# althonos/pyskani

Hardware: AMD Instinct MI355X
Metric: genome-pairs/sec (sketch+ANI) (higher is better)
Workload: dtype u64; 1 GPU; all-vs-all 10000 x 10000 synthetic ~5 Mb genomes on one GPU (100 families x 100; single-contig genomes, substitutions only), c=125 marker_c=1000 k=15; device-resident ASCII; hits=999867, genomes=10000, parallelism=references sharded over 1 GPU(s)

## Files before the change

### pyskani_amd/csrc/chain.hip

```cpp
#include "chain_stages.h"
#include "query_parts.h"
#include <hipcub/hipcub.hpp>
#include <cmath>
#include <algorithm>
#include <unordered_map>


SketchDesc make_desc(const psk_sketch* s, bool unindexed_ok) {
    SketchDesc d{};
    const bool ix = s->idx != nullptr;
    d.key = ix ? s->idx->km32 + s->idx_off : nullptr; d.pms = ix ? s->idx->pms + s->idx_off : nullptr;
    d.perm = ix ? s->idx->perm + s->idx_off : nullptr; d.bucket = ix ? s->idx->bucket + s->idx_boff : nullptr;
    d.bshift = ix ? s->idx_bshift : 0; d.n = (ix || (unindexed_ok && s->store)) ? (uint32_t)s->n_seeds : 0;
    d.pos = s->store ? s->store->seed_pos + s->seed_off : nullptr; d.meta = s->store ? s->store->seed_meta + s->seed_off : nullptr;
    d.kmer = s->store ? s->store->seed_kmer + s->seed_off : nullptr;
    d.seed_pos_base = s->store ? s->store->seed_pos : nullptr;
    d.contig_start = s->store ? s->store->contig_seed_start + s->contig_off : nullptr;
    d.total_len = s->total_len; d.n_contigs = (uint32_t)s->contig_len.size();
    uint64_t rows = 0;
    if (d.n) for (uint32_t len : s->contig_len) rows += (uint64_t)len / (FRAGMENT_LENGTH + 1) + 1;
    d.rows = (uint32_t)std::min<uint64_t>(rows, 0xFFFFFFFFu);
    s->len_quantiles(d.lenq);
    d.tab = (ix && s->ptab) ? (const ProbeLine*)s->ptab->base + s->ptab_off : nullptr; d.tab_lines = (ix && s->ptab) ? s->ptab_lines : 0;
    return d;
// ... 25 lines not shown
    const int lane = threadIdx.x & 63, wave = threadIdx.x >> 6;
    uint32_t running = 0;
    for (uint32_t base = 0; base < n_refs && running < B.rank_hi; base += 256) {
        const uint32_t r = base + threadIdx.x;
        const bool f = r < n_refs && row[r];
        const unsigned long long bal = __ballot(f);
        if (lane == 0) s_w[wave] = (uint32_t)__popcll(bal);
        __syncthreads();
        uint32_t before = 0;
        for (int w = 0; w < wave; w++) before += s_w[w];
        const uint32_t tot = s_w[0] + s_w[1] + s_w[2] + s_w[3];
        const uint32_t rank = running + before + (uint32_t)__popcll(bal & ((1ull << lane) - 1));
        if (f && rank >= B.rank_lo && rank < B.rank_hi) {
            const uint32_t j = rank - B.rank_lo, slot = B.pair_off + j;
            pairs[slot] = combine_desc(Q, rd[r]);
            sbase[slot] = B.item_off + j * Q.n; cbase[slot] = B.row_off + j * Q.rows;
            pair_qr[slot] = make_uint2(B.q, r);
        }
        running += tot;
        __syncthreads();
    }
    if (blockIdx.x == gridDim.x - 1 && threadIdx.x == 0) { sbase[n_pairs] = n_items; cbase[n_pairs] = n_rows; }
}

__global__ __launch_bounds__(256) void pass_canon_kernel(uint8_t* __restrict__ pass, uint32_t n_refs, const uint32_t* __restrict__ canon) {
    uint8_t* row = pass + (size_t)blockIdx.x * n_refs;
    for (uint32_t r = threadIdx.x; r < n_refs; r += blockDim.x) if (row[r] && canon[r] != r) { row[canon[r]] = 1; row[r] = 0; }
}
static_assert((1 << BSI_BLOG) == 256, "pass_count_kernel: one sweep of its 256 threads = one block of references");
__global__ __launch_bounds__(256) void pass_count_kernel(const uint8_t* __restrict__ pass, uint32_t n_refs, uint32_t* __restrict__ row_count, uint8_t* __restrict__ col_flag, uint32_t* __restrict__ row_blocks) {
    __shared__ uint32_t s_c[4], s_any;
    const uint8_t* row = pass + (size_t)blockIdx.x * n_refs;
    uint32_t c = 0, blocks = 0;
    if (threadIdx.x == 0) s_any = 0;
    __syncthreads();
    for (uint32_t r0 = 0; r0 < n_refs; r0 += 256) {
        const uint32_t r = r0 + threadIdx.x;
        const bool f = r < n_refs && row[r];
        if (f) { c++; col_flag[r] = 1; s_any = 1; }
        __syncthreads();
        blocks += s_any;
        __syncthreads();
        if (threadIdx.x == 0) s_any = 0;
        __syncthreads();
    }
#pragma unroll
    for (int o = 32; o > 0; o >>= 1) c += __shfl_xor(c, o);
    if ((threadIdx.x & 63) == 0) s_c[threadIdx.x >> 6] = c;
    __syncthreads();
    if (threadIdx.x == 0) { row_count[blockIdx.x] = s_c[0] + s_c[1] + s_c[2] + s_c[3]; row_blocks[blockIdx.x] = blocks; }
}

__global__ __launch_bounds__(256) void gsi_room_kernel(const uint32_t* __restrict__ sbase, uint32_t n_pairs, uint32_t* __restrict__ pstart) {
    const uint32_t p = blockIdx.x * blockDim.x + threadIdx.x;
    if (p <= n_pairs) { const uint32_t a = sbase[p]; pstart[p] = a + (a >> 3) + 8u * p; }
}
__global__ void gsi_total_kernel(const unsigned long long* __restrict__ poff, uint32_t n_pairs, unsigned long long* __restrict__ total64) { *total64 = poff[n_pairs]; }

struct HitPasses { __host__ __device__ bool operator()(const psk_hit& h) const { return h.ani > 0.1f; } };

__global__ __launch_bounds__(256) void work_rows_kernel(const ChunkOut* __restrict__ cout, const uint32_t* __restrict__ n_chunks, const uint32_t* __restrict__ cbase,
                                                        const uint32_t* __restrict__ row_pair, uint32_t n_rows, unsigned long long* __restrict__ out) {
    __shared__ unsigned long long s_c[4], s_l[4];
    unsigned long long c = 0, live = 0;
    for (uint32_t r = blockIdx.x * blockDim.x + threadIdx.x; r < n_rows; r += gridDim.x * blockDim.x) {
        const uint32_t p = row_pair[r];
        if (r - cbase[p] < n_chunks[p]) { c += cout[r].n_cand; live++; }
    }
#pragma unroll
    for (int o = 32; o > 0; o >>= 1) { c += __shfl_xor(c, o); live += __shfl_xor(live, o); }
    if ((threadIdx.x & 63) == 0) { s_c[threadIdx.x >> 6] = c; s_l[threadIdx.x >> 6] = live; }
    __syncthreads();
    if (threadIdx.x == 0) {
        c = s_c[0] + s_c[1] + s_c[2] + s_c[3]; live = s_l[0] + s_l[1] + s_l[2] + s_l[3];
        if (live) { atomicAdd(&out[0], c); atomicAdd(&out[1], live); }
    }
}

psk_status chain_layout(Lane* ctx, size_t n_pairs, size_t n_items, size_t n_rows, size_t n_bq, ChainBufs* L) {
    const size_t gi = (n_items + 255) / 256, gi_sum = std::max(gi, (n_pairs + 3) / 4);
    size_t o_pairs = 0, o_sbase = al256(o_pairs + sizeof(PairDesc) * n_pairs), o_cbase = al256(o_sbase + 4 * (n_pairs + 1)),
           o_pstart = al256(o_cbase + 4 * (n_pairs + 1)), o_lb = al256(o_pstart + 4 * (n_pairs + 1)),
           o_aoff = al256(o_lb + 8 * (n_items + 1)), o_nch = al256(o_aoff + 4 * (n_items + 1)),
           o_chunks = al256(o_nch + 4 * n_pairs), o_cout = al256(o_chunks + sizeof(uint2) * n_rows),
           o_misc = al256(o_cout + sizeof(ChunkOut) * n_rows), o_hits = o_misc + 256, o_sel = al256(o_hits + sizeof(psk_hit) * n_pairs),
           o_ovf = al256(o_sel + sizeof(psk_hit) * n_pairs), o_bsum = al256(o_ovf + 4 * n_rows),
           o_qr = al256(o_bsum + 8 * (gi_sum + 1)), o_bq = al256(o_qr + 8 * n_pairs), o_bp = al256(o_bq + sizeof(BatchQ) * (n_bq + 1)),
           o_rp = al256(o_bp + 4 * (gi + 1)), o_live = al256(o_rp + 4 * (n_rows + 1)), o_big = al256(o_live + 4 * (n_pairs + 1)),
           o_huge = al256(o_big + 4 * (n_pairs + 1)), o_end = o_huge + 4 * (n_pairs + 1);
    PSK_TRY(ctx->q_b.reserve(o_end));
    char* B = (char*)ctx->q_b.p;
    L->pairs = (PairDesc*)(B + o_pairs); L->sbase = (uint32_t*)(B + o_sbase); L->cbase = (uint32_t*)(B + o_cbase); L->pstart = (uint32_t*)(B + o_pstart);
    L->lbcnt = (uint2*)(B + o_lb); L->aoff = (uint32_t*)(B + o_aoff); L->nch = (uint32_t*)(B + o_nch); L->chunks = (uint2*)(B + o_chunks);
    L->cout = (ChunkOut*)(B + o_cout); L->hits = (psk_hit*)(B + o_hits); L->hits_sel = (psk_hit*)(B + o_sel); L->misc = (uint32_t*)(B + o_misc);
    L->ovf = (uint32_t*)(B + o_ovf); L->bsum = (unsigned long long*)(B + o_bsum); L->pair_qr = (uint2*)(B + o_qr); L->bq = (BatchQ*)(B + o_bq);
    L->blk_pair = (uint32_t*)(B + o_bp); L->row_pair = (uint32_t*)(B + o_rp); L->live = (uint32_t*)(B + o_live); L->big_list = (uint32_t*)(B + o_big); L->huge_list = (uint32_t*)(B + o_huge);
    L->gi = (uint32_t)gi; L->gi_sum = (uint32_t)gi_sum;
    L->total = (unsigned long long*)(L->misc + 16);
    return PSK_OK;
}

psk_status chain_run(Lane* ctx, const ChainBufs& L, uint32_t n_pairs, size_t n_items, size_t n_rows, const psk_params& prm,
                     const psk_query_opts* o, const SketchDesc* d_qd, const SketchDesc* d_rd, uint64_t cap, bool wide, const Switches& sw, bool probe_ok) {
    hipStream_t st = ctx->stream;
    const int force_serial = sw.chain_serial.get() != nullptr;
    const uint32_t gi = L.gi;
    hipLaunchKernelGGL(pair_table_kernel, dim3((uint32_t)(((size_t)gi + n_rows + 255) / 256)), dim3(256), 0, st, L.sbase, L.cbase, n_pairs, gi, (uint32_t)n_items, (uint32_t)n_rows, L.blk_pair, L.row_pair,
                       L.misc, L.lbcnt + n_items);
    ctx->t_begin(K_ANCHOR);
    if (wide) hipLaunchKernelGGL(anchor_count_kernel, dim3(gi), dim3(256), 0, st, L.pairs, L.sbase, n_pairs, (uint32_t)n_items, L.lbcnt, L.bsum, L.blk_pair);
    const uint32_t gi4 = (gi + JT - 1) / JT;
    uint32_t n_sum = gi;
    const int jp_force = sw.join_pairs.force();
    const bool gsi_join = !wide && (L.g_key || L.b_key) && L.d_pass && L.n_bq;
    const bool join_pairs = !wide && (gsi_join || (jp_force >= 0 ? jp_force == 1 : (n_pairs >= 16384 && n_items / n_pairs < 2048)));
    const bool gsl = gsi_join && L.gsi_slice;
    const bool gsi_one = gsi_join && !gsl && L.gsi_onepass && cap >= n_items + n_items / 8 + 8 * ((size_t)n_pairs + 1);
    bool probe_local = false;
    GsiJoinArgs GA{};
    GslArgs GL{};
    const uint32_t gsi_nw = (L.g_key && !L.gsi_slice) ? std::max(4u, (L.n_refs + 63u) / 64u) : 4u;
    const size_t gsi_lds_row = 8 * (size_t)gsi_nw + 4 * (size_t)((gsi_nw + 1u) & ~1u), gsi_lds_count = gsi_lds_row + 4 * (size_t)L.p_cap, gsi_lds_emit = gsi_lds_row + 4 * (size_t)L.p_cap * 9;
    if (gsi_join) {
        GA.bq = L.bq; GA.pass = L.d_pass; GA.n_refs = L.n_refs; GA.qd = d_qd; GA.g_key = L.g_key; GA.g_val = L.g_val; GA.g_bucket = L.g_bucket; GA.g_shift = L.g_shift;
        GA.b_key = L.b_key; GA.b_val = L.b_val; GA.b_bucket = L.b_bucket; GA.b_shift = L.b_shift; GA.b_nb1 = L.b_nb1; GA.b_blocks = L.b_blocks; GA.b_max = L.b_max;
        GA.pair_cnt = L.big_list; GA.pstart = L.pstart; GA.cap = (uint32_t)cap; GA.err = L.misc; GA.p_cap = L.p_cap; GA.nw_lds = gsi_nw;
        const uint32_t t_blocks = gsl ? L.g_blocks : L.b_blocks;
        const unsigned long long* t_base = gsl ? L.g_base : L.b_base;
        const uint32_t bcap = std::max(1u, std::min<uint32_t>(t_blocks, std::min<uint32_t>(GSI_PMAX, std::max(1u, L.p_cap))));
        uint32_t* d_btab = nullptr; uint32_t* d_bcnt = nullptr;
        if (t_blocks) {
            const size_t o_bc = al256(4 * (size_t)L.n_bq * bcap * GSL_BT_WORDS);
            PSK_TRY(ctx->q_k.reserve(o_bc + 4 * (size_t)L.n_bq + 256));
            d_btab = (uint32_t*)ctx->q_k.p; d_bcnt = (uint32_t*)((char*)ctx->q_k.p + o_bc);
            PSK_TRY(gsl_blocks_launch(L.bq, L.n_bq, L.d_pass, L.n_refs, t_blocks, t_base, d_btab, d_bcnt, bcap, st));
        }
        GA.blk_tab = d_btab; GA.blk_cnt = d_bcnt; GA.blk_cap = bcap;
        if (gsl) {
            GL.bq = L.bq; GL.n_entries = L.n_bq; GL.tab = L.gsl_tab; GL.n_tab = L.gsl_n_tab; GL.ebase = L.gsl_ebase; GL.pass = L.d_pass; GL.n_refs = L.n_refs; GL.qd = d_qd;
            GL.g_key = L.g_key; GL.g_val = L.g_val; GL.g_bucket = L.g_bucket; GL.g_shift = L.g_shift; GL.g_nb1 = L.g_nb1; GL.g_blocks = L.g_blocks; GL.g_base = L.g_base; GL.blk_tab = d_btab; GL.blk_cnt = d_bcnt; GL.blk_cap = bcap; GL.cnt = L.gsl_cnt; GL.rec = L.gsl_rec; GL.bm = L.gsl_bm; GL.un = L.gsl_un; GL.n_slices = L.gsl_n_slices;
            GL.pair_cnt = L.big_list; GL.pstart = L.pstart; GL.cap = (uint32_t)cap; GL.err = L.misc; GL.p_cap = L.p_cap; GL.chunks = L.chunks; GL.n_chunks = L.nch;
            PSK_HIP(hipMemsetAsync(L.big_list, 0, 4 * ((size_t)n_pairs + 1), st));
            PSK_TRY(gsl_count_launch(GL, st));
        }
        else if (!gsi_one) hipLaunchKernelGGL(gsi_join_kernel<false>, dim3(L.n_bq), dim3(64), gsi_lds_count, st, GA);
        probe_local = true;
    }
    else if (join_pairs) {
        size_t ts = 0;
        uint32_t* keys_in = L.big_list;
        uint32_t* vals_in = L.live;
        uint32_t* keys_out = (uint32_t*)L.hits_sel;
        uint32_t* order = keys_out + n_pairs;
        hipLaunchKernelGGL(pair_ref_keys_kernel, dim3((n_pairs + 255) / 256), dim3(256), 0, st, L.pair_qr, n_pairs, keys_in, vals_in);
        PSK_HIP(hipcub::DeviceRadixSort::SortPairs(nullptr, ts, keys_in, keys_out, vals_in, order, (int)n_pairs, 0, 32, st));
        PSK_TRY(ctx->q_g.reserve(ts + 256));
        PSK_HIP(hipcub::DeviceRadixSort::SortPairs(ctx->q_g.p, ts, keys_in, keys_out, vals_in, order, (int)n_pairs, 0, 32, st));
        const uint32_t nb = (n_pairs + 3) / 4;
        probe_local = probe_ok;
        if (probe_ok) hipLaunchKernelGGL(anchor_join_probe_kernel, dim3(nb), dim3(256), 0, st, L.pairs, L.sbase, order, n_pairs, L.lbcnt, L.bsum, L.misc + 5, L.aoff, L.big_list);
        else hipLaunchKernelGGL(anchor_join_pairs_kernel, dim3(nb), dim3(256), 0, st, L.pairs, L.sbase, order, n_pairs, L.lbcnt, L.bsum, L.misc + 5);
        n_sum = nb;
    }
    const int ep_force = sw.emit_pairs.force();
    const bool emit_pairs = !wide && !join_pairs && n_items >= 2 * ((size_t)n_pairs + 1) &&
                            (ep_force >= 0 ? ep_force == 1 : (n_pairs >= 1024 && n_items / n_pairs >= 1024 && n_items / n_pairs <= (1u << 17)));
    uint32_t* pair_cnt = L.live;
    if (emit_pairs) PSK_HIP(hipMemsetAsync(pair_cnt, 0, 4 * ((size_t)n_pairs + 1), st));
    const int xg_env = (int)sw.xcd_group.num(-1);
    const uint32_t xcd_group = xg_env >= 0 ? (uint32_t)xg_env : (n_pairs >= 64 ? (uint32_t)std::min<size_t>(4096, std::max<size_t>(1, 4 * (n_items / n_pairs) / (JT * 256))) : 0u);
    if (!wide && !join_pairs) { hipLaunchKernelGGL(anchor_join4_kernel, dim3(gi4), dim3(256), 0, st, L.pairs, L.sbase, n_pairs, (uint32_t)n_items, gi, L.lbcnt, L.bsum, L.misc + 5, L.blk_pair, emit_pairs ? pair_cnt : (uint32_t*)nullptr, xcd_group); n_sum = gi4; }
    ctx->t_end();
    size_t tmp = 0, tmp2 = 0;
    hipcub::TransformInputIterator<uint32_t, CountOf, const uint2*> cnt_it(L.lbcnt, CountOf());
    hipcub::TransformInputIterator<uint32_t, PackedCount, const uint2*> pcnt_it(L.lbcnt, PackedCount());
    PSK_HIP(hipcub::DeviceScan::ExclusiveSum(nullptr, tmp, cnt_it, L.aoff, (int)(n_items + 1), st));
    PSK_HIP(hipcub::DeviceReduce::Sum(nullptr, tmp2, L.bsum, L.total, (int)L.gi_sum, st));
    size_t tmp3 = 0;
    PSK_HIP(hipcub::DeviceSelect::If(nullptr, tmp3, L.hits, L.hits_sel, L.misc + 12, (int)n_pairs, HitPasses(), st));
    PSK_TRY(ctx->q_c.reserve(std::max(tmp, std::max(tmp2, tmp3))));
    unsigned long long* poff = (unsigned long long*)L.aoff;
    hipcub::TransformInputIterator<unsigned long long, Widen, const uint32_t*> pc_it(pair_cnt, Widen());
    if (gsi_one) {
        hipLaunchKernelGGL(gsi_room_kernel, dim3((n_pairs + 1 + 255) / 256), dim3(256), 0, st, (const uint32_t*)L.sbase, n_pairs, L.pstart);
        PSK_HIP(hipMemsetAsync(L.total, 0, 8, st));
    }
    else if (emit_pairs) {
        size_t tmp4 = 0;
        PSK_HIP(hipcub::DeviceScan::ExclusiveSum(nullptr, tmp4, pc_it, poff, (int)(n_pairs + 1), st));
        PSK_TRY(ctx->q_c.reserve(std::max(tmp4, std::max(tmp, std::max(tmp2, tmp3)))));
        PSK_HIP(hipcub::DeviceScan::ExclusiveSum(ctx->q_c.p, tmp4, pc_it, poff, (int)(n_pairs + 1), st));
        hipLaunchKernelGGL(pair_start64_kernel, dim3((n_pairs + 1 + 255) / 256), dim3(256), 0, st, poff, n_pairs, L.pstart, (uint32_t)cap, (const uint32_t*)(L.misc + 5));
    }
    else if (probe_local) {
        hipcub::TransformInputIterator<unsigned long long, Widen, const uint32_t*> pl_it(L.big_list, Widen());
        size_t tmp5 = 0;
        PSK_HIP(hipcub::DeviceScan::ExclusiveSum(nullptr, tmp5, pl_it, (unsigned long long*)nullptr, (int)(n_pairs + 1), st));
        const size_t o_poff = al256(tmp5 + 256);
        PSK_TRY(ctx->q_g.reserve(o_poff + 8 * ((size_t)n_pairs + 2) + 256));
        unsigned long long* pl_off64 = (unsigned long long*)((char*)ctx->q_g.p + o_poff);
        PSK_HIP(hipMemsetAsync(L.big_list + n_pairs, 0, 4, st));
        PSK_HIP(hipcub::DeviceScan::ExclusiveSum(ctx->q_g.p, tmp5, pl_it, pl_off64, (int)(n_pairs + 1), st));
        hipLaunchKernelGGL(pair_start64_kernel, dim3((n_pairs + 1 + 255) / 256), dim3(256), 0, st, (const unsigned long long*)pl_off64, n_pairs, L.pstart, (uint32_t)cap, (const uint32_t*)(L.misc + 5));
        if (gsi_join) hipLaunchKernelGGL(gsi_total_kernel, dim3(1), dim3(1), 0, st, (const unsigned long long*)pl_off64, n_pairs, L.total);
    }
    else if (wide) PSK_HIP(hipcub::DeviceScan::ExclusiveSum(ctx->q_c.p, tmp, cnt_it, L.aoff, (int)(n_items + 1), st));
    else PSK_HIP(hipcub::DeviceScan::ExclusiveSum(ctx->q_c.p, tmp, pcnt_it, L.aoff, (int)(n_items + 1), st));
    const bool small_sum = !gsi_join && n_sum <= 16384;
    if (!small_sum && !gsi_join) PSK_HIP(hipcub::DeviceReduce::Sum(ctx->q_c.p, tmp2, L.bsum, L.total, (int)n_sum, st));
    if ((!emit_pairs && !probe_local) || small_sum)
        hipLaunchKernelGGL(pair_start_kernel, dim3((emit_pairs || probe_local) ? 1u : (n_pairs + 1 + 255) / 256), dim3(256), 0, st, (emit_pairs || probe_local) ? (const uint32_t*)nullptr : L.aoff, L.sbase, n_pairs, L.pstart, (uint32_t)cap,
                           L.bsum, small_sum ? n_sum : 0u, L.total, (const uint32_t*)(L.misc + 5));
    hipLaunchKernelGGL(pair_guard_kernel, dim3((n_pairs + 1 + 255) / 256), dim3(256), 0, st, (const uint32_t*)(L.misc + 5), (const unsigned long long*)L.total, (unsigned long long)cap, L.pstart, n_pairs);
    const size_t na = ((size_t)cap + 64 + 63) & ~(size_t)63;
    PSK_TRY(ctx->q_d.reserve(4 * na * CHAIN_ANCHOR_WORDS));
    PSK_TRY(ctx->q_e.reserve(na * (8 + 4 * 7 + 1) + 512 + 4 * 2 * BIG_GMAX * (BIG_GROUPS + 64) + 4 * BIG_GROUPS));
    uint32_t* D = (uint32_t*)ctx->q_d.p;
    uint32_t* E4 = (uint32_t*)ctx->q_e.p;
    uint4* anc = (uint4*)D;
    uint32_t* a_nxt = D + 4 * na;
    ChainArgs A{};
    A.anc = anc;
    A.sc_ptr = D + 5 * na;
    A.sc_f = (int32_t*)E4; A.sc_root = E4 + na; A.sc_depth = E4 + 2 * na; A.sc_best = E4 + 3 * na;
    uint32_t* CAND = D + 6 * na;
    A.c_score.p = (int32_t*)CAND; A.c_q0.p = CAND + 1; A.c_q1.p = CAND + 2; A.c_r0.p = CAND + 3; A.c_r1.p = CAND + 4; A.c_n.p = CAND + 5; A.c_rc.p = CAND + 6; A.c_state.p = CAND + 7;
    A.chunks = L.chunks; A.n_chunks = L.nch; A.cbase = L.cbase; A.n_pairs = n_pairs; A.n_rows = (uint32_t)n_rows;
    A.row_pair = L.row_pair;
    A.pairs = L.pairs;
    A.out = L.cout; A.two_c = 2u * (uint32_t)prm.c; A.force_serial = force_serial; A.stats = L.misc + 1;
    A.band = std::max(1, std::min(MAX_CHAIN_BAND, BP_CHAIN_BAND / (int)prm.c));
    A.cap = (uint32_t)cap;
    const bool use_hops = gsi_join ? false : sw.chunk_hops.get() ? !sw.chunk_hops.off() : ((n_pairs < 1024 && n_items / n_pairs > 4096) || n_items / n_pairs > (1u << 20));
    const bool emit_heads = emit_pairs && !use_hops && !sw.emit_heads.off();
    const int hi_force = sw.hops_items.force();
    const bool hops_items = use_hops && !gsl && !emit_pairs && !join_pairs && n_items <= 0x7FFFFFFFull && (hi_force >= 0 ? hi_force == 1 : n_items / n_pairs > (1u << 20));
    ctx->t_begin(K_ANCHOR_EMIT);
    if (hops_items) {
        const size_t o_scr = al256(4 * (size_t)n_pairs * HOP_SLICES + 256);
        PSK_TRY(ctx->q_g.reserve(o_scr + sizeof(uint2) * n_rows + 256));
        uint32_t* slice_cnt = (uint32_t*)ctx->q_g.p;
        uint2* scratch_rows = (uint2*)((char*)ctx->q_g.p + o_scr);
        hipStream_t sd = nullptr;
        PSK_TRY(ctx->side_lane(&sd));
        PSK_HIP(hipEventRecord(ctx->side_fork, st));
        PSK_HIP(hipStreamWaitEvent(sd, ctx->side_fork, 0));
        hipLaunchKernelGGL(chunk_hops_items_kernel, dim3(n_pairs, HOP_SLICES), dim3(64), 0, sd, L.pstart, (const uint32_t*)L.aoff, L.pairs, L.sbase, L.cbase, n_pairs, slice_cnt, scratch_rows, L.misc);
        hipLaunchKernelGGL(chunk_hops_sliced_kernel, dim3(n_pairs, HOP_SLICES), dim3(64), 0, sd, L.pstart, a_nxt, anc, L.pairs, L.cbase, n_pairs, slice_cnt, 1, scratch_rows, L.chunks, L.nch, L.misc);
        PSK_HIP(hipEventRecord(ctx->side_join, sd));
    }
    if (gsl) { GL.anc = anc; PSK_TRY(gsl_heads_launch(GL, st)); PSK_TRY(gsl_emit_launch(GL, st)); }
    else if (gsi_join) { GA.anc = anc; GA.chunks = L.chunks; GA.n_chunks = L.nch; GA.onepass = gsi_one ? 1 : 0; GA.total = L.total; if (gsi_one) GA.pair_cnt = L.aoff;
                    hipLaunchKernelGGL(gsi_join_kernel<true>, dim3(L.n_bq), dim3(64), gsi_lds_emit, st, GA); }
    else if (wide) hipLaunchKernelGGL(anchor_emit_kernel, dim3(gi), dim3(256), 0, st, L.pairs, L.sbase, n_pairs, (uint32_t)n_items, L.lbcnt, L.aoff, anc, (uint32_t)cap, L.misc, L.blk_pair);
    else if (emit_pairs) hipLaunchKernelGGL(anchor_emit_pairs_kernel, dim3(n_pairs), dim3(EP_T), 0, st, L.pairs, L.sbase, n_pairs, L.lbcnt, poff, anc, (uint32_t)cap, L.misc,
                                            L.cbase, emit_heads ? L.chunks : (uint2*)nullptr, L.nch);
    else {
        const int ex_force = sw.emit_expand.force();
        const bool expand = ex_force >= 0 ? ex_force == 1 : n_items / n_pairs > (1u << 20);
        if (expand) hipLaunchKernelGGL(anchor_emit_expand_kernel, dim3(gi), dim3(256), 0, st, L.pairs, L.sbase, n_pairs, (uint32_t)n_items, L.lbcnt, L.aoff, anc, (uint32_t)cap, L.misc, L.blk_pair);
        else hipLaunchKernelGGL(anchor_emit_packed4_kernel, dim3(gi4), dim3(256), 0, st, L.pairs, L.sbase, n_pairs, (uint32_t)n_items, gi, L.lbcnt, L.aoff, anc, (uint32_t)cap, L.misc, L.blk_pair,
                                probe_local ? (const uint32_t*)L.pstart : (const uint32_t*)nullptr);
    }
    if (hops_items) PSK_HIP(hipStreamWaitEvent(st, ctx->side_join, 0));
    else if (use_hops) {
        if (n_items / n_pairs > (1u << 20)) {
            uint32_t* coarse = E4;
            hipLaunchKernelGGL(anchor_next_kernel<1>, dim3((uint32_t)((cap / 64 + 1 + 255) / 256)), dim3(256), 0, st, anc, L.pstart, n_pairs, (const uint32_t*)nullptr, coarse);
            hipLaunchKernelGGL(anchor_next_kernel<2>, dim3((uint32_t)((cap + 255) / 256)), dim3(256), 0, st, anc, L.pstart, n_pairs, (const uint32_t*)coarse, a_nxt);
        } else
        hipLaunchKernelGGL(anchor_next_kernel<0>, dim3((uint32_t)((cap + 255) / 256)), dim3(256), 0, st, anc, L.pstart, n_pairs, (const uint32_t*)nullptr, a_nxt);
        if (n_items / n_pairs > (1u << 20)) {
            const size_t o_scr = al256(4 * (size_t)n_pairs * HOP_SLICES + 256);
            PSK_TRY(ctx->q_g.reserve(o_scr + sizeof(uint2) * n_rows + 256));
            uint32_t* slice_cnt = (uint32_t*)ctx->q_g.p;
            uint2* scratch_rows = (uint2*)((char*)ctx->q_g.p + o_scr);
            for (int pass = 0; pass < 2; pass++)
                hipLaunchKernelGGL(chunk_hops_sliced_kernel, dim3(n_pairs, HOP_SLICES), dim3(64), 0, st, L.pstart, a_nxt, anc, L.pairs, L.cbase, n_pairs, slice_cnt, pass, scratch_rows, L.chunks, L.nch, L.misc);
        } else
        hipLaunchKernelGGL(chunk_hops_kernel, dim3(n_pairs), dim3(64), 0, st, L.pstart, a_nxt, L.cbase, n_pairs, L.chunks, L.nch, L.misc);
    } else if (!emit_heads && !gsi_join)
        hipLaunchKernelGGL(chunk_heads_kernel, dim3(n_pairs), dim3(64), 0, st, L.pstart, anc, L.cbase, n_pairs, L.chunks, L.nch, L.misc);
    ctx->t_end();
    ctx->t_begin(K_CHAIN_CHUNK);
    auto order_rows = [&]() -> psk_status {
        if (n_rows < 4096) return PSK_OK;
        size_t ts = 0;
        PSK_HIP(hipcub::DeviceRadixSort::SortPairsDescending(nullptr, ts, (const uint32_t*)nullptr, (uint32_t*)nullptr, (const uint32_t*)nullptr, (uint32_t*)nullptr, (int)n_rows, 0, 8, st));
        const size_t ob = al256(4 * n_rows);
        PSK_TRY(ctx->q_g.reserve(4 * ob + ts + 256));
        uint32_t* k_in = (uint32_t*)ctx->q_g.p; uint32_t* v_in = (uint32_t*)((char*)ctx->q_g.p + ob); uint32_t* k_out = (uint32_t*)((char*)ctx->q_g.p + 2 * ob); uint32_t* v_out = (uint32_t*)((char*)ctx->q_g.p + 3 * ob);
        hipLaunchKernelGGL(row_len_kernel, dim3((uint32_t)((n_rows + 255) / 256)), dim3(256), 0, st, L.chunks, L.nch, L.cbase, L.row_pair, (uint32_t)n_rows, k_in, v_in);
        PSK_HIP(hipcub::DeviceRadixSort::SortPairsDescending((char*)ctx->q_g.p + 4 * ob, ts, (const uint32_t*)k_in, k_out, (const uint32_t*)v_in, v_out, (int)n_rows, 0, 8, st));
        A.row_order = v_out;
        return PSK_OK;
    };
    {
        const char* le = sw.chain_lane.get();
        A.lane_dp = !force_serial && A.band <= LANE_N && !sw.chain_lane.off();
        if (A.lane_dp) {
            PSK_TRY(order_rows());
            uint32_t rpw = 64;
            while (rpw > 16 && n_rows / rpw < 512) rpw >>= 1;
            const int le_rows = (int)sw.chain_lane.num(0);
            if (le_rows >= 8) rpw = (uint32_t)std::min(64, le_rows);
            const uint32_t waves = (uint32_t)((n_rows + rpw - 1) / rpw);
            A.ovf_list = L.ovf; A.ovf_count = L.misc + 8;
            const bool quad = le && le[0] == 'q' ? true : (le_rows >= 8 ? false : n_rows < 32 * 1024);
            if (quad) {
                const uint32_t qw = (uint32_t)((n_rows + 15) / 16);
                hipLaunchKernelGGL(chain_quad_kernel, dim3((qw + LANE_WAVES - 1) / LANE_WAVES), dim3(64 * LANE_WAVES), 0, st, A);
            } else {
                const int xt_force = sw.lane_xtrees.force();
                const bool xtrees = xt_force >= 0 ? xt_force == 1 : n_items / n_pairs > (1u << 20);
                if (A.band <= 20 && xtrees) hipLaunchKernelGGL(chain_lane20x_kernel, dim3((waves + LANE_WAVES - 1) / LANE_WAVES), dim3(64 * LANE_WAVES), 0, st, A, rpw);
                else if (A.band <= 20) hipLaunchKernelGGL(chain_lane20_kernel, dim3((waves + LANE_WAVES - 1) / LANE_WAVES), dim3(64 * LANE_WAVES), 0, st, A, rpw);
                else hipLaunchKernelGGL(chain_lane_kernel, dim3((waves + LANE_WAVES - 1) / LANE_WAVES), dim3(64 * LANE_WAVES), 0, st, A, rpw);
            }
            const uint32_t lw = (uint32_t)std::min<size_t>((n_rows + CHAIN_WAVES - 1) / CHAIN_WAVES, 2048);
            hipLaunchKernelGGL(chain_chunk_list_kernel, dim3(lw), dim3(64 * CHAIN_WAVES), 0, st, A);
        }
    }
    const int wr_force = sw.chain_wave_reg.force();
    const bool wave_reg = !A.lane_dp && !force_serial && A.band < 128 && (wr_force >= 0 ? wr_force == 1 : n_rows <= 2048);
    if (wave_reg) {
        const dim3 g((uint32_t)((n_rows + CHAIN_WAVES - 1) / CHAIN_WAVES)), b(64 * CHAIN_WAVES);
        if (A.band < 64) hipLaunchKernelGGL(chain_wave_reg_kernel<1>, g, b, 0, st, A);
        else hipLaunchKernelGGL(chain_wave_reg_kernel<2>, g, b, 0, st, A);
    }
    const bool quad_deep = !wave_reg && !A.lane_dp && !force_serial && !sw.chain_quad_deep.off() && A.band <= 4 * QD && !sw.chain_lane.off();
    if (quad_deep) {
        A.ovf_list = L.ovf; A.ovf_count = L.misc + 8;
        A.lane_dp = 1;
        PSK_TRY(order_rows());
        const uint32_t qw = (uint32_t)((n_rows + 15) / 16);
        hipLaunchKernelGGL(chain_quad_deep_kernel, dim3((qw + LANE_WAVES - 1) / LANE_WAVES), dim3(64 * LANE_WAVES), 0, st, A);
        const uint32_t lw = (uint32_t)std::min<size_t>((n_rows + CHAIN_WAVES - 1) / CHAIN_WAVES, 2048);
        hipLaunchKernelGGL(chain_chunk_list_kernel, dim3(lw), dim3(64 * CHAIN_WAVES), 0, st, A);
    }
    if (!A.lane_dp && !wave_reg)
    hipLaunchKernelGGL(chain_chunk_kernel, dim3((uint32_t)((n_rows + CHAIN_WAVES - 1) / CHAIN_WAVES)), dim3(64 * CHAIN_WAVES), 0, st, A);
    ctx->t_end();
    SelArgs SA{};
    SA.chunks = L.chunks; SA.n_chunks = L.nch; SA.cbase = L.cbase; SA.n_pairs = n_pairs;
    SA.c_score = A.c_score; SA.c_q0 = A.c_q0; SA.c_q1 = A.c_q1; SA.c_r0 = A.c_r0; SA.c_r1 = A.c_r1; SA.c_n = A.c_n; SA.c_rc = A.c_rc; SA.c_state = A.c_state;
    SA.out = L.cout; SA.two_c = A.two_c; SA.force_serial = force_serial; SA.stats = L.misc + 1;
    const bool use_live = n_pairs > 4096;
    SA.live = use_live ? L.live : nullptr; SA.n_live = L.misc + 9; SA.big_list = L.big_list; SA.big_count = L.misc + 10;
    if (use_live) {
        hipcub::CountingInputIterator<uint32_t> ids(0);
        size_t tl = 0;
        PSK_HIP(hipcub::DeviceSelect::If(nullptr, tl, ids, L.live, L.misc + 9, (int)n_pairs, IsLivePair{L.nch}, st));
        PSK_TRY(ctx->q_c.reserve(std::max(tl, std::max(tmp, std::max(tmp2, tmp3)))));
        PSK_HIP(hipcub::DeviceSelect::If(ctx->q_c.p, tl, ids, L.live, L.misc + 9, (int)n_pairs, IsLivePair{L.nch}, st));
    }
    ctx->t_begin(K_SELECT);
    {
        SA.tiny_done = use_live && !force_serial && !sw.select_tiny.off() && n_rows / n_pairs < 16;
        SA.rest_list = (uint32_t*)L.hits_sel; SA.rest_count = L.misc + 13;
        if (SA.tiny_done) hipLaunchKernelGGL(select_tiny_kernel, dim3((n_pairs + 255) / 256), dim3(256), 0, st, SA);
    }
    hipLaunchKernelGGL(select_kernel, dim3(std::min<uint32_t>(n_pairs, 16384u)), dim3(64), 0, st, SA, L.huge_list, L.misc + 14);
    hipLaunchKernelGGL(select_mid_kernel, dim3(std::min<uint32_t>(n_pairs, 768u)), dim3(64), 0, st, SA, (const uint32_t*)L.huge_list, (const uint32_t*)(L.misc + 14));
    {
        if (!force_serial) {
            BigArgs BA{};
            BA.S = SA; BA.pstart = L.pstart;
            char* E = (char*)ctx->q_e.p;
            BA.key = (unsigned long long*)E; uint32_t* U = (uint32_t*)(E + 8 * na);
            BA.slot = U; BA.crow = U + na; BA.idx = U + 2 * na; BA.pm = U + 3 * na; BA.pm2 = U + 4 * na; BA.ord = U + 5 * na; BA.clist = U + 6 * na;
            BA.conf = (uint8_t*)(U + 7 * na);
            BA.parts = (uint32_t*)(E + (((size_t)na * (8 + 4 * 7 + 1) + 255) & ~(size_t)255));
            BA.huge_list = L.huge_list; BA.huge_count = L.misc + 11; BA.ctr = L.misc + 32; BA.huge_c = BA.parts + (size_t)2 * BIG_GMAX * (BIG_GROUPS + 64);
            const uint32_t solo = sw.big_solo.get() ? (uint32_t)std::max((int)sw.big_solo.num(0), CMAX) : BIG_SOLO;
            BA.solo = solo;
            hipLaunchKernelGGL(select_big_kernel, dim3(std::min<uint32_t>(n_pairs, 64u)), dim3(BIG_T), 0, st, BA);
            if (na / 3 > solo) {
                static std::mutex slots_mu;
                static std::unordered_map<int, uint32_t> slots_of;
                uint32_t slots;
                {
                    std::lock_guard<std::mutex> lk(slots_mu);
                    auto it = slots_of.find(ctx->device);
                    if (it == slots_of.end()) {
                        int per_cu = 0, cus = 0;
                        PSK_HIP(hipOccupancyMaxActiveBlocksPerMultiprocessor(&per_cu, select_huge_kernel, BIG_T, 0));
                        PSK_HIP(hipDeviceGetAttribute(&cus, hipDeviceAttributeMultiprocessorCount, ctx->device));
                        if (sw.huge_slots.get()) { per_cu = 1; cus = std::max(0, (int)sw.huge_slots.num(0)); }
                        it = slots_of.emplace(ctx->device, (uint32_t)std::max(0, per_cu) * (uint32_t)std::max(0, cus)).first;
                    }
                    slots = it->second;
                }
                uint32_t nb = BIG_GMAX;
                if ((double)(n_items / n_pairs) > sw.huge_min_seeds.num((double)(1ull << 20))) {
                    ctx->huge_acquire();
                    while (nb > 1 && nb > slots) nb >>= 1;
                } else {
                    const uint32_t rest = slots > BIG_GMAX ? slots - BIG_GMAX : 0;
                    while (nb > 1 && (size_t)nb * ctx->dev->max_lanes > rest) nb >>= 1;
                }
                if (nb < 8) nb = 1;
                hipLaunchKernelGGL(select_huge_kernel, dim3(nb), dim3(BIG_T), 0, st, BA);
            }
        }
    }
    hipLaunchKernelGGL(chunk_seeds_kernel, dim3((uint32_t)((n_rows + 255) / 256)), dim3(256), 0, st, A);
    ctx->t_end();
    ReduceArgs R{};
    R.chunks = L.cout; R.n_chunks = L.nch; R.cbase = L.cbase; R.pstart = L.pstart; R.pcnt = gsi_one ? L.aoff : nullptr; R.pairs = L.pairs; R.pair_qr = L.pair_qr;
    R.k = prm.k; R.median = o->median; R.robust = o->robust;
    R.min_af = o->min_aligned_frac > 0 ? o->min_aligned_frac : 0.15; R.hits = L.hits;
    if (o->median || o->robust) {
        PSK_TRY(ctx->q_f.reserve(sizeof(double) * (2 * n_rows + 1024 * (size_t)n_pairs + 1024)));
        R.big_vals = (double*)ctx->q_f.p;
    }
    ctx->t_begin(K_PAIR_REDUCE);
    R.live = use_live ? L.live : nullptr; R.n_live = L.misc + 9;
    if (use_live) hipLaunchKernelGGL(pair_empty_kernel, dim3((n_pairs + 255) / 256), dim3(256), 0, st, R, n_pairs);
    const bool no_small = sw.reduce_small.off();
    const bool no_wave = sw.reduce_wave.off();
    R.wave_done = !no_wave && !no_small && L.rows_pair_max > 64u && n_rows / n_pairs <= 64u * RW_PER;
    R.small_done = !no_small && (n_rows / n_pairs < 16 || R.wave_done);
    const bool no_tiny = sw.reduce_tiny.off();
    R.tiny_done = R.small_done && !no_tiny && !o->median && !o->robust && n_rows / n_pairs < 16;
// ... 144 lines not shown
```

### pyskani_amd/csrc/chain_dev.h

```cpp
#pragma once
#include "common.h"

struct MarkerSet { const uint64_t* p; uint32_t n; uint32_t pad; };

__device__ __forceinline__ void lds_wave_sync() {
    __builtin_amdgcn_fence(__ATOMIC_RELEASE, "workgroup");
    __builtin_amdgcn_wave_barrier();
    __builtin_amdgcn_fence(__ATOMIC_ACQUIRE, "workgroup");
}

struct LaneAnchor { uint32_t q, u, m; int32_t f; };
__device__ __forceinline__ uint32_t lane_diag(uint32_t qx, uint32_t rx, uint32_t sg) { return qx - ((rx ^ sg) - sg); }

struct LanePred { uint32_t q1, u, m; int32_t f1; };
__device__ __forceinline__ int32_t lane_eval2(uint32_t qx, uint32_t ux, uint32_t mx, const LanePred& y, int d) {
    const int32_t a = (int32_t)(qx - y.q1);
    const int32_t t = (int32_t)(ux - y.u), nt = (int32_t)(y.u - ux);
    const int32_t gap = t > nt ? t : nt;
    const int32_t b = a - t;
    const int32_t s1 = y.f1 - gap;
    const uint32_t z = y.m ^ mx;
    const uint32_t bad = (uint32_t)a | (uint32_t)(BP_CHAIN_BAND - 1 - a) | (uint32_t)b | (uint32_t)(MAX_GAP_LENGTH - gap) | (uint32_t)s1 | z | (0u - z);
    const uint32_t key = ((uint32_t)s1 << 7) + ((((uint32_t)ANCHOR_SCORE2 + 1u) << 7) | (127u - (uint32_t)d));
    return (int32_t)(key | (bad & 0x80000000u));
}
```

### pyskani_amd/csrc/chain_stages.h

```cpp
#pragma once
#include "common.h"
#include "chain_dev.h"
#include "slice_join.h"

struct PairDesc {
    const uint32_t* r_key; const uint64_t* r_pms;
    const uint32_t* q_key; const uint32_t* q_perm;
    const uint32_t* q_pos; const uint32_t* q_meta;
    const uint32_t* q_kmer;
    uint32_t q_nc, pad_;
    const uint32_t* q_seed_pos_base;
    const uint32_t* q_contig_start;
    uint64_t q_total_len, r_total_len;
    uint32_t r_n, q_n;
    const uint32_t* r_bucket; uint32_t r_bshift;
    uint32_t r_tab_lines; const ProbeLine* r_tab;
};


__device__ __forceinline__ uint32_t find_le(const uint32_t* __restrict__ base, uint32_t n, uint32_t x) {
    uint32_t lo = 0, hi = n - 1;
    while (lo < hi) { uint32_t mid = (lo + hi + 1) >> 1; if (base[mid] <= x) lo = mid; else hi = mid - 1; }
    return lo;
}

__device__ __forceinline__ uint32_t pair_from_hint(const uint32_t* __restrict__ base, uint32_t n, uint32_t x, uint32_t p) {
    while (p + 1 < n && base[p + 1] <= x) p++;
    return p;
}

struct CountOf { __host__ __device__ uint32_t operator()(const uint2& v) const { return v.y; } };

constexpr int JOIN_WIN = 256;

struct PackedCount { __host__ __device__ uint32_t operator()(const uint2& v) const { return v.y >> 24; } };

constexpr int JT = 4;

struct Widen { __host__ __device__ unsigned long long operator()(const uint32_t& v) const { return v; } };

constexpr int EP_W = 1;

constexpr int EP_T = 64 * EP_W;

constexpr int HEAD_WIN = 2048;

constexpr int HOP_WIN = 4096;

constexpr int HOP_SLICES = 32;

struct ChunkOut { uint32_t anchors, seeds, n_intervals, n_cand; uint32_t left, right; uint64_t cov_q; };

template <class T> struct Strided {
    T* p;
    __host__ __device__ __forceinline__ T& operator[](size_t i) const { return p[i * 8]; }
};

struct ChainArgs {
    const uint4* anc;
    const uint2* chunks; const uint32_t* n_chunks; const uint32_t* cbase; uint32_t n_pairs, n_rows;
    const uint32_t* row_pair;
    const uint32_t* row_order;
    const PairDesc* pairs;
    ChunkOut* out;
    int32_t* sc_f; uint32_t *sc_ptr, *sc_root, *sc_depth, *sc_best;
    Strided<int32_t> c_score; Strided<uint32_t> c_q0, c_q1, c_r0, c_r1, c_n, c_state, c_rc;
    uint32_t two_c; int band; int force_serial; int lane_dp;
    uint32_t cap;
    uint32_t* ovf_list; uint32_t* ovf_count;
    uint32_t* stats;
};

constexpr int RING = 128;

constexpr int RMAX = 256;

constexpr int CHAIN_WAVES = 4;

constexpr int LANE_N = 24;

constexpr int LANE_WAVES = 2;

constexpr int LANE_TREES = 4;

constexpr int LANE_XTREES = 12;

constexpr int QUAD_N = LANE_N / 4;

constexpr int QD = 21;

constexpr int QD_NEAR = 2;

constexpr int QD_RING = 128;

constexpr int CMAX = 1024;

struct SelArgs {
    const uint2* chunks; const uint32_t* n_chunks; const uint32_t* cbase; uint32_t n_pairs;
    Strided<int32_t> c_score; Strided<uint32_t> c_q0, c_q1, c_r0, c_r1, c_n, c_rc, c_state;
    ChunkOut* out; uint32_t two_c; int force_serial; uint32_t* stats;
    const uint32_t* live; const uint32_t* n_live;
    uint32_t* rest_list; uint32_t* rest_count;
    uint32_t* big_list; uint32_t* big_count;
    int tiny_done;
};

constexpr uint32_t TINY_ROWS = 4, TINY_CANDS = 8;

constexpr int CSMALL = 512;

struct BigArgs {
    SelArgs S; const uint32_t* pstart;
    unsigned long long* key;
    uint32_t *slot, *crow;
    uint32_t *idx, *pm, *pm2;
    uint32_t *ord, *clist;
    uint8_t* conf;
    uint32_t *huge_list, *huge_count;
    uint32_t* huge_c;
    uint32_t *ctr, *parts;
    uint32_t solo;
};

constexpr int BIG_T = 1024;

constexpr uint32_t BIG_TILE = 4096;

constexpr uint32_t BIG_SOLO = 32768;

#ifndef BIG_GMAX_N
#define BIG_GMAX_N 256
#endif
constexpr uint32_t BIG_GMAX = BIG_GMAX_N;

constexpr uint32_t BIG_GROUPS = 16;

struct ReduceArgs {
    const ChunkOut* chunks; const uint32_t* n_chunks; const uint32_t* cbase;
    const uint32_t* pstart; const PairDesc* pairs;
    const uint32_t* pcnt;
    const uint2* pair_qr;
    const uint32_t* live; const uint32_t* n_live;
// ... 14 lines not shown
struct IsLivePair { const uint32_t* nch; __host__ __device__ bool operator()(const uint32_t& p) const { return nch[p] != 0; } };

struct GsiJoinArgs {
    const BatchQ* bq; const uint8_t* pass; uint32_t n_refs; const SketchDesc* qd;
    const uint32_t* g_key; const unsigned long long* g_val; const uint32_t* g_bucket; int g_shift;
    const uint32_t* b_key; const unsigned long long* b_val; const uint32_t* b_bucket; int b_shift; uint32_t b_nb1, b_blocks, b_max;
    const uint32_t* blk_tab; const uint32_t* blk_cnt; uint32_t blk_cap;
    uint32_t nw_lds;
    uint32_t* pair_cnt; const uint32_t* pstart; uint4* anc; uint32_t cap; uint32_t* err;
    uint32_t p_cap;
    uint2* chunks; uint32_t* n_chunks;
    int onepass; unsigned long long* total;
};

#ifndef LANE_NEAR_N
#define LANE_NEAR_N 3
#endif
constexpr int LANE_NEAR = LANE_NEAR_N;

__global__ __launch_bounds__(256) void pair_table_kernel(const uint32_t* __restrict__ sbase, const uint32_t* __restrict__ cbase, uint32_t n,
                                                         uint32_t n_tiles, uint32_t n_items, uint32_t n_rows,
                                                         uint32_t* __restrict__ blk_pair, uint32_t* __restrict__ row_pair, uint32_t* __restrict__ misc, uint2* __restrict__ lb_tail);
__global__ __launch_bounds__(256) void anchor_count_kernel(const PairDesc* __restrict__ pairs, const uint32_t* __restrict__ sbase,
                                                           uint32_t n_pairs, uint32_t n_items,
                                                           uint2* __restrict__ lbcnt_out, unsigned long long* __restrict__ block_sum,
                                                           const uint32_t* __restrict__ blk_pair);
__global__ __launch_bounds__(256) void anchor_join4_kernel(const PairDesc* __restrict__ pairs, const uint32_t* __restrict__ sbase,
                                                           uint32_t n_pairs, uint32_t n_items, uint32_t n_tiles,
                                                           uint2* __restrict__ item_out, unsigned long long* __restrict__ block_sum,
                                                           uint32_t* __restrict__ need_wide, const uint32_t* __restrict__ blk_pair,
                                                           uint32_t* __restrict__ pair_cnt, uint32_t xcd_group);
__global__ __launch_bounds__(256) void anchor_join_pairs_kernel(const PairDesc* __restrict__ pairs, const uint32_t* __restrict__ sbase,
                                                                const uint32_t* __restrict__ order, uint32_t n_pairs,
                                                                uint2* __restrict__ item_out, unsigned long long* __restrict__ block_sum,
                                                                uint32_t* __restrict__ need_wide);
__global__ __launch_bounds__(256) void anchor_join_probe_kernel(const PairDesc* __restrict__ pairs, const uint32_t* __restrict__ sbase,
                                                                const uint32_t* __restrict__ order, uint32_t n_pairs,
                                                                uint2* __restrict__ item_out, unsigned long long* __restrict__ block_sum,
                                                                uint32_t* __restrict__ need_wide, uint32_t* __restrict__ aoff_local, uint32_t* __restrict__ pair_cnt);
__global__ __launch_bounds__(256) void anchor_emit_packed4_kernel(const PairDesc* __restrict__ pairs, const uint32_t* __restrict__ sbase,
                                                                  uint32_t n_pairs, uint32_t n_items, uint32_t n_tiles,
                                                                  const uint2* __restrict__ item, const uint32_t* __restrict__ aoff,
                                                                  uint4* __restrict__ anc, uint32_t cap, uint32_t* __restrict__ err,
                                                                  const uint32_t* __restrict__ blk_pair, const uint32_t* __restrict__ pstart_local);
__global__ __launch_bounds__(256) void anchor_emit_expand_kernel(const PairDesc* __restrict__ pairs, const uint32_t* __restrict__ sbase,
                                                                 uint32_t n_pairs, uint32_t n_items,
                                                                 const uint2* __restrict__ item, const uint32_t* __restrict__ aoff,
                                                                 uint4* __restrict__ anc, uint32_t cap, uint32_t* __restrict__ err,
                                                                 const uint32_t* __restrict__ blk_pair);
__global__ __launch_bounds__(256) void anchor_emit_kernel(const PairDesc* __restrict__ pairs, const uint32_t* __restrict__ sbase,
                                                          uint32_t n_pairs, uint32_t n_items,
                                                          const uint2* __restrict__ lbcnt,
                                                          const uint32_t* __restrict__ aoff,
                                                          uint4* __restrict__ anc, uint32_t cap, uint32_t* __restrict__ err,
                                                          const uint32_t* __restrict__ blk_pair);
__global__ __launch_bounds__(EP_T) __attribute__((amdgpu_waves_per_eu(5, 8))) void anchor_emit_pairs_kernel(const PairDesc* __restrict__ pairs, const uint32_t* __restrict__ sbase, uint32_t n_pairs,
                                                                const uint2* __restrict__ item, const unsigned long long* __restrict__ poff,
                                                                uint4* __restrict__ anc, uint32_t cap, uint32_t* __restrict__ err,
                                                                const uint32_t* __restrict__ cbase, uint2* __restrict__ chunks, uint32_t* __restrict__ n_chunks);
__global__ __launch_bounds__(256) void pair_start64_kernel(const unsigned long long* __restrict__ poff, uint32_t n_pairs, uint32_t* __restrict__ pstart, uint32_t cap,
                                                           const uint32_t* __restrict__ need_wide);
__global__ __launch_bounds__(256) void pair_guard_kernel(const uint32_t* __restrict__ need_wide, const unsigned long long* __restrict__ total64, unsigned long long cap,
                                                         uint32_t* __restrict__ pstart, uint32_t n_pairs);
__global__ __launch_bounds__(256) void pair_start_kernel(const uint32_t* __restrict__ aoff, const uint32_t* __restrict__ sbase, uint32_t n_pairs, uint32_t* __restrict__ pstart, uint32_t cap,
                                                         const unsigned long long* __restrict__ bsum, uint32_t n_sum, unsigned long long* __restrict__ total64,
                                                         const uint32_t* __restrict__ need_wide);
__global__ __launch_bounds__(64) void chunk_heads_kernel(const uint32_t* __restrict__ pstart, const uint4* __restrict__ anc,
                                                         const uint32_t* __restrict__ cbase, uint32_t n_pairs, uint2* __restrict__ chunks,
                                                         uint32_t* __restrict__ n_chunks, uint32_t* __restrict__ err);
template <int COARSE>
__global__ __launch_bounds__(256) void anchor_next_kernel(const uint4* __restrict__ anc,
                                                          const uint32_t* __restrict__ pstart, uint32_t n_pairs,
                                                          const uint32_t* __restrict__ coarse, uint32_t* __restrict__ nxt);
__global__ __launch_bounds__(64) void chunk_hops_kernel(const uint32_t* __restrict__ pstart, const uint32_t* __restrict__ nxt, const uint32_t* __restrict__ cbase,
                                                         uint32_t n_pairs, uint2* __restrict__ chunks, uint32_t* __restrict__ n_chunks,
                                                         uint32_t* __restrict__ err);
__global__ __launch_bounds__(64) void chunk_hops_sliced_kernel(const uint32_t* __restrict__ pstart, const uint32_t* __restrict__ nxt, const uint4* __restrict__ anc,
                                                                const PairDesc* __restrict__ pairs, const uint32_t* __restrict__ cbase, uint32_t n_pairs,
                                                                uint32_t* __restrict__ slice_cnt, int pass, uint2* __restrict__ scratch, uint2* __restrict__ chunks, uint32_t* __restrict__ n_chunks,
                                                                uint32_t* __restrict__ err);
__global__ __launch_bounds__(64) void chunk_hops_items_kernel(const uint32_t* __restrict__ pstart, const uint32_t* __restrict__ aoff,
                                                               const PairDesc* __restrict__ pairs, const uint32_t* __restrict__ sbase, const uint32_t* __restrict__ cbase,
                                                               uint32_t n_pairs, uint32_t* __restrict__ slice_cnt, uint2* __restrict__ scratch, uint32_t* __restrict__ err);
__global__ __launch_bounds__(64 * LANE_WAVES) __attribute__((amdgpu_waves_per_eu(3, 8))) void chain_lane20_kernel(ChainArgs A, uint32_t rows_per_wave);
__global__ __launch_bounds__(64 * LANE_WAVES) void chain_lane20x_kernel(ChainArgs A, uint32_t rows_per_wave);
__global__ __launch_bounds__(64 * LANE_WAVES) void chain_lane_kernel(ChainArgs A, uint32_t rows_per_wave);
__global__ __launch_bounds__(64 * LANE_WAVES) void chain_quad_kernel(ChainArgs A);
__global__ __launch_bounds__(64 * LANE_WAVES) void chain_quad_deep_kernel(ChainArgs A);
__global__ __launch_bounds__(64 * CHAIN_WAVES) void chain_chunk_kernel(ChainArgs A);
__global__ __launch_bounds__(64 * CHAIN_WAVES) void chain_chunk_list_kernel(ChainArgs A);
__global__ __launch_bounds__(256) void row_len_kernel(const uint2* __restrict__ chunks, const uint32_t* __restrict__ n_chunks, const uint32_t* __restrict__ cbase,
                                                      const uint32_t* __restrict__ row_pair, uint32_t n_rows, uint32_t* __restrict__ key, uint32_t* __restrict__ val);
template <int S>
__global__ __launch_bounds__(64 * CHAIN_WAVES) void chain_wave_reg_kernel(ChainArgs A);
__global__ __launch_bounds__(256) void select_tiny_kernel(SelArgs S);
__global__ __launch_bounds__(64) void select_kernel(SelArgs S, uint32_t* __restrict__ mid_list, uint32_t* __restrict__ mid_count);
__global__ __launch_bounds__(64) void select_mid_kernel(SelArgs S, const uint32_t* __restrict__ mid_list, const uint32_t* __restrict__ mid_count);
__global__ __launch_bounds__(BIG_T) void select_big_kernel(BigArgs B);
__global__ __launch_bounds__(BIG_T) void select_huge_kernel(BigArgs B);
__global__ __launch_bounds__(256) void chunk_seeds_kernel(ChainArgs A);
__global__ __launch_bounds__(256) void pair_empty_kernel(ReduceArgs R, uint32_t n_pairs);
__global__ __launch_bounds__(256) void pair_reduce_small_kernel(ReduceArgs R, uint32_t n_pairs);
__global__ __launch_bounds__(256) void pair_reduce_tiny_kernel(ReduceArgs R, uint32_t n_pairs);
__global__ __launch_bounds__(256) void pair_reduce_wave_kernel(ReduceArgs R, uint32_t n_pairs);
__global__ __launch_bounds__(256) void pair_reduce_kernel(ReduceArgs R, uint32_t n_pairs);
__global__ __launch_bounds__(256) void pair_reduce_large_kernel(ReduceArgs R, uint32_t n_pairs);
__global__ __launch_bounds__(256) void pair_ref_keys_kernel(const uint2* __restrict__ pair_qr, uint32_t n_pairs, uint32_t* __restrict__ keys, uint32_t* __restrict__ ids);
template <bool EMIT>
__global__ __launch_bounds__(64) void gsi_join_kernel(GsiJoinArgs A);
```

### pyskani_amd/csrc/common.h

```cpp
#pragma once
#include <hip/hip_runtime.h>
#include <cstdint>
#include <cstdio>
#include <cstdlib>
#include <cstring>
#include <ctime>
#include <sys/mman.h>
#include <algorithm>
#include <atomic>
#include <memory>
#include <mutex>
#include <shared_mutex>
#include <condition_variable>
#include <deque>
#include <string>
#include <unordered_map>
#include <vector>
#include "../../include/pyskani_amd.h"

struct EnvVal {
    const char* text;
    bool off() const { return text && text[0] == '0'; }
    int force() const { return text ? text[0] == '1' : -1; }
    double num(double dflt) const { return text ? atof(text) : dflt; }
// ... 372 lines not shown
    mutable std::shared_ptr<IndexStore> idx;
    mutable uint64_t idx_off = 0;
    mutable uint64_t idx_boff = 0;
    mutable uint32_t idx_bshift = 0;
    mutable std::shared_ptr<ProbeStore> ptab;
    mutable uint64_t ptab_off = 0;
    mutable uint32_t ptab_lines = 0;
};

struct psk_db {
    psk_ctx* ctx = nullptr;
    mutable std::shared_mutex rw;
    psk_params params{};
    std::vector<psk_sketch*> refs;
    std::deque<std::string> names;
    std::vector<uint32_t> name_slot;
    std::vector<uint32_t> canon;
    bool has_dups = false, canon_dirty = false;
    static uint32_t name_hash(const std::string& s) { uint32_t h = 2166136261u; for (unsigned char c : s) h = (h ^ c) * 16777619u; return h; }
    void note_added(uint32_t i) {
        canon_dirty = true;
        if (name_slot.size() < 2 * (size_t)(i + 1) + 2) {
            size_t cap = 64; while (cap < 4 * (size_t)(i + 1)) cap <<= 1;
            std::vector<uint32_t> grown(cap, 0);
            for (uint32_t v : name_slot) if (v) { size_t k = name_hash(names[v - 1]) & (cap - 1); while (grown[k]) k = (k + 1) & (cap - 1); grown[k] = v; }
            name_slot.swap(grown);
        }
        const size_t mask = name_slot.size() - 1;
        size_t k = name_hash(names[i]) & mask;
        while (name_slot[k] && names[name_slot[k] - 1] != names[i]) k = (k + 1) & mask;
        if (name_slot[k]) { has_dups = true; const uint32_t prev = name_slot[k] - 1; for (uint32_t j = 0; j < i; j++) if (canon[j] == prev) canon[j] = i; }
        name_slot[k] = i + 1;
        canon.push_back(i);
    }
    bool tables_dirty = true;
    PoolScratch d_marker_ptr, d_marker_n;
    bool inv_dirty = true;
    PoolScratch inv_key, inv_ref, inv_tmp, inv_bucket;
    uint64_t inv_n = 0; int inv_bits = 0;
    bool desc_dirty = true;
    uint64_t desc_indexed = 0; uint32_t desc_n = 0;
    PoolScratch d_refdesc, d_canon;
    std::vector<SketchDesc> h_refdesc;
    int gsi_state = 0;
    PoolScratch gsi_key, gsi_val, gsi_bucket;
    uint64_t gsi_n = 0; int gsi_shift = 0;
    int bsi_state = 0;
    PoolScratch bsi_key, bsi_val, bsi_bucket, bsi_base;
    uint64_t bsi_n = 0; int bsi_shift = 0; uint32_t bsi_nb1 = 0, bsi_blocks = 0;
    std::atomic<int> small_state{0};
};

struct ModelNode { int32_t feature; float threshold; int32_t left, right; float value; int32_t missing, is_leaf, menu; };
struct ModelDev { const ModelNode* nodes; const uint32_t* first; uint32_t n_trees; uint32_t n_features; float bias, shrinkage; };
struct psk_model {
    psk_ctx* ctx = nullptr;
    void* base = nullptr;
    ModelDev dev{};
    uint64_t n_nodes = 0;
    std::vector<int32_t> features;
    ~psk_model() { if (base) (void)hipFree(base); }
};
void learned_apply_launch(const psk_model* m, psk_hit* d_hits, const uint2* pair_qr, const SketchDesc* qd, const SketchDesc* rd,
                          uint32_t n_pairs, hipStream_t st);

struct ContigDesc {
    uint64_t byte_off;
    uint32_t len;
    uint32_t first_tile;
    uint32_t genome;
    uint32_t contig_index;
    uint32_t pad0, pad1;
};

struct SketchConsts {
    uint64_t thr, thr_marker;
    uint32_t kmask;
    int k, d, rshift;
    int delta;
};


constexpr int BSI_BLOG = 8;
constexpr uint32_t SQ_MAX_TILES = 64, SQ_MAX_DESC = 64;
constexpr uint32_t SQ_SEEDS = 3072;
constexpr uint32_t SQ_MARKERS = 2048;
constexpr uint32_t SQ_ROWS = 64;
constexpr uint32_t SQ_CANDS = 256;
constexpr uint32_t SQ_HITS_FIRST = 256;
constexpr uint32_t SQ_F_SEEDS = 1u, SQ_F_MARKERS = 2u, SQ_F_PAIR = 4u;
struct SmallQHead {
    uint32_t n_seeds, n_markers_raw, n_markers, n_short;
    uint32_t flags, n_hits;
    unsigned long long n_anchors;
    uint32_t coff[SQ_MAX_DESC + 1];
    uint32_t done;
    uint32_t pad1[128 - 9 - (SQ_MAX_DESC + 1)];
};
static_assert(sizeof(SmallQHead) == 512, "the status block is 512 bytes, the hits follow it");
struct SmallQSketch {
    const uint8_t* d_bases; const ContigDesc* d_desc; const uint32_t* d_tci; const uint4* d_tinfo; const uint32_t* d_cft;
    uint32_t n_desc, n_tiles;
    uint32_t *d_packed; uint64_t* d_mask; uint32_t *d_cnt, *d_toff, *d_tmc;
    uint32_t *seed_kmer, *seed_pos, *seed_meta; uint64_t* seed_pm; uint64_t* mstage;
    SmallQHead* head;
};
psk_status small_query_sketch_enqueue(Lane* ctx, const psk_params* p, const SmallQSketch& A, hipStream_t st);

__device__ __forceinline__ uint64_t mm_hash64(uint64_t key) {
    key = ~(key + (key << 21));
    key = key ^ key >> 24;
    key = (key + (key << 3)) + (key << 8);
    key = key ^ key >> 14;
    key = (key + (key << 2)) + (key << 4);
    key = key ^ key >> 28;
    key = key + (key << 31);
    return key;
}

__device__ __forceinline__ uint64_t mm_hash64_u32(uint32_t key) {
    const uint64_t P = (uint64_t)key * 0x200001u;
    uint32_t lo = (uint32_t)P, hi = (uint32_t)(P >> 32);
    lo ^= __builtin_amdgcn_alignbit(hi, lo, 24);
    hi ^= 0xFFFFFF00u;
    uint64_t r = (uint64_t)lo * 265u;
    hi = hi * 265u + (uint32_t)(r >> 32);
    uint64_t x = ((uint64_t)hi << 32) | (uint32_t)r;
    x ^= x >> 14;
    lo = (uint32_t)x; hi = (uint32_t)(x >> 32);
    r = (uint64_t)lo * 21u;
    hi = hi * 21u + (uint32_t)(r >> 32);
    x = ((uint64_t)hi << 32) | (uint32_t)r;
    x ^= x >> 28;
    lo = (uint32_t)x; hi = (uint32_t)(x >> 32);
    r = (uint64_t)lo * 0x80000001u;
    hi = (hi << 31) + (uint32_t)(r >> 32) + hi;
    return ((uint64_t)hi << 32) | (uint32_t)r;
}

psk_status sketch_batch_impl(Lane* ctx, const psk_params* p, const uint8_t* d_bases,
                             const uint64_t* contig_off, const uint64_t* contig_len,
                             const uint32_t* genome_first_contig, uint32_t n_genomes,
                             int want_seeds, psk_sketch** out, const uint32_t* d_packed_in = nullptr);
extern "C" void psk_pack2bit_host(const uint8_t* src, uint64_t n, uint32_t* dst, int mode);
psk_status ensure_index(Lane* ctx, const psk_sketch* const* refs, uint32_t n, bool lazy = false);
psk_status ensure_probe(Lane* ctx, const psk_sketch* const* refs, uint32_t n);
__device__ __forceinline__ uint32_t probe_line(uint32_t km, uint32_t lines) { return __umulhi(km * 2654435761u, lines); }
psk_status screen_impl(Lane* ctx, psk_db* db, const psk_sketch* query, double screen_val, int rescue_small,
                       uint8_t* pass, uint32_t* shared);
psk_status chain_pairs_impl(Lane* ctx, const psk_sketch* const* refs, const psk_sketch* const* queries, uint32_t n,
                            const psk_query_opts* o, psk_hit* out);
void* hit_block_alloc(size_t bytes);
bool hit_block_free(void* p);
void hit_block_trim();
template <class H>
struct HitListT {
    H* p = nullptr; size_t n = 0, cap = 0;
    HitListT() = default;
    HitListT(const HitListT&) = delete; HitListT& operator=(const HitListT&) = delete;
    ~HitListT() { drop(p); }
    static void drop(void* q) { if (q && !hit_block_free(q)) free(q); }
    bool reserve(size_t want) {
        if (want <= cap) return true;
        if (n && want < 2 * cap) want = 2 * cap;
        const size_t bytes = sizeof(H) * want;
        H* q = (H*)(bytes >= ((size_t)8 << 20) ? hit_block_alloc(bytes) : malloc(bytes));
// ... 28 lines not shown
```

### pyskani_amd/csrc/dp.hip

```cpp
#include "chain_stages.h"






__device__ uint32_t chain_chunk_serial(const ChainArgs& A, uint32_t s, uint32_t e) {
    for (uint32_t x = s; x < e; x++) {
        int32_t bs = ANCHOR_SCORE2; uint32_t bp = x;
        uint32_t qx = A.anc[x].x, rx = A.anc[x].y, mx = A.anc[x].z;
        for (uint32_t y = x; y-- > s && x - y <= (uint32_t)A.band;) {
            if (A.anc[y].z != mx) continue;
            int64_t dq = (int64_t)qx - (int64_t)A.anc[y].x;
            if (dq > BP_CHAIN_BAND) break;
            int64_t dr = (mx & 1) ? (int64_t)A.anc[y].y - (int64_t)rx : (int64_t)rx - (int64_t)A.anc[y].y;
            if (dq <= 0 || dr <= 0) continue;
            int64_t gap = dq > dr ? dq - dr : dr - dq;
            if (gap > MAX_GAP_LENGTH) continue;
            int32_t sc = A.sc_f[y] + ANCHOR_SCORE2 - (int32_t)gap;
            if (sc > bs) { bs = sc; bp = y; }
        }
        A.sc_f[x] = bs;
        if (bp == x) { A.sc_root[x] = x; A.sc_depth[x] = 1; }
        else { A.sc_root[x] = A.sc_root[bp]; A.sc_depth[x] = A.sc_depth[bp] + 1; }
        A.sc_best[x] = 0xFFFFFFFFu;
    }
    for (uint32_t x = s; x < e; x++) { uint32_t rt = A.sc_root[x]; uint32_t b = A.sc_best[rt]; if (b == 0xFFFFFFFFu || A.sc_f[x] > A.sc_f[b]) A.sc_best[rt] = x; }
    uint32_t nc = 0;
    for (uint32_t x = s; x < e; x++) {
        if (A.sc_root[x] != x) continue;
        uint32_t b = A.sc_best[x];
        if (A.sc_depth[b] < MIN_ANCHORS || A.sc_f[b] < MIN_SCORE2) continue;
        uint32_t ra = A.anc[x].y, rb = A.anc[b].y;
        A.c_score[s + nc] = A.sc_f[b]; A.c_q0[s + nc] = A.anc[x].x; A.c_q1[s + nc] = A.anc[b].x;
        A.c_r0[s + nc] = ra < rb ? ra : rb; A.c_r1[s + nc] = ra < rb ? rb : ra; A.c_n[s + nc] = A.sc_depth[b];
        A.c_rc[s + nc] = A.anc[x].z >> 1;
        nc++;
    }
    return nc;
}



template <int W, int XT>
__device__ __forceinline__ void chain_lane_body(const ChainArgs& A, const uint32_t rows_per_wave) {
    __shared__ uint32_t s_rd[LANE_WAVES][32][64];
    __shared__ unsigned long long s_xk[LANE_WAVES][XT ? XT : 1][XT ? 64 : 1];
    __shared__ uint32_t s_xr[LANE_WAVES][XT ? XT : 1][XT ? 64 : 1];
    const int wave = threadIdx.x >> 6, lane = threadIdx.x & 63;
    const uint32_t slot_i = (blockIdx.x * LANE_WAVES + wave) * rows_per_wave + lane;
    const uint32_t slot = A.row_order && (uint32_t)lane < rows_per_wave && slot_i < A.n_rows ? A.row_order[slot_i] : slot_i;
    uint32_t s = 0, e = 0;
    bool mine = false, real = false;
    const uint32_t pair = A.row_pair[slot < A.n_rows ? slot : A.n_rows - 1];
    if ((uint32_t)lane < rows_per_wave && slot_i < A.n_rows) {
        if (slot - A.cbase[pair] < A.n_chunks[pair]) {
            const uint2 se = A.chunks[slot];
            s = se.x; e = se.y;
            real = true;
            mine = e > s && e - s < 16384;
        }
    }
    constexpr int LD = XT ? 1 : 2;
    const uint32_t s_al = s & ~(4u * LD - 1u);
    const uint32_t len = mine ? e - s_al : 0;
    LanePred P[W];
#pragma unroll
    for (int i = 0; i < W; i++) { P[i].q1 = 0; P[i].u = 0; P[i].m = 0xFFFFFFFFu; P[i].f1 = -1; }
    unsigned long long bk[LANE_TREES];
    uint32_t sroot[LANE_TREES];
#pragma unroll
    for (int j = 0; j < LANE_TREES; j++) { bk[j] = 0; sroot[j] = 0xFFFFFFFFu; }
    uint32_t S = 0;
    bool ovf = false;
    uint32_t (*rd)[64] = s_rd[wave];
    const int band = A.band;
    constexpr bool prune = XT == 0;
    constexpr int NR = LANE_NEAR;
    uint32_t far_diag = 0;
    for (uint32_t tb = 0; __any(tb < len); tb += 4 * LD) {
      uint4 an[4 * LD];
#pragma unroll
      for (int i = 0; i < 4 * LD; i++) an[i] = make_uint4(0, 0, 0, 0);
      if (tb < len) {
#pragma unroll
          for (int i = 0; i < 4 * LD; i++) an[i] = A.anc[s_al + tb + i];
      }
#pragma unroll
      for (int h = 0; h < LD; h++) {
        const uint32_t t0 = tb + 4u * h, x0 = s_al + t0;
        const uint32_t qs[4] = {an[4 * h].x, an[4 * h + 1].x, an[4 * h + 2].x, an[4 * h + 3].x}, rs[4] = {an[4 * h].y, an[4 * h + 1].y, an[4 * h + 2].y, an[4 * h + 3].y},
                       ms[4] = {an[4 * h].z, an[4 * h + 1].z, an[4 * h + 2].z, an[4 * h + 3].z};
        LanePred nw[4];
        int32_t ftop[4] = {-1, -1, -1, -1};
        if (prune) {
            if ((t0 & 63u) == 0) {
                far_diag = 0;
#pragma unroll
                for (int i = NR - 3; i < W; i++) far_diag |= __builtin_amdgcn_alignbit(3u, 3u, 32u - (((P[i].u - (uint32_t)MAX_GAP_LENGTH) >> 10) & 31u));
            } else {
#pragma unroll
                for (int i = NR - 3; i <= NR; i++) far_diag |= __builtin_amdgcn_alignbit(3u, 3u, 32u - (((P[i].u - (uint32_t)MAX_GAP_LENGTH) >> 10) & 31u));
            }
            const uint32_t q0 = qs[0] + 1u;
            int32_t m = -1;
#pragma unroll
            for (int i = NR; i < W; i++) { const int32_t f = q0 - P[i].q1 <= (uint32_t)BP_CHAIN_BAND ? P[i].f1 : -1; m = f > m ? f : m; }
            ftop[0] = m;
#pragma unroll
            for (int u = 1; u < 4; u++) { const int32_t f = q0 - P[NR - u].q1 <= (uint32_t)BP_CHAIN_BAND ? P[NR - u].f1 : -1; m = f > m ? f : m; ftop[u] = m; }
        }
#pragma unroll
        for (int u = 0; u < 4; u++) {
            const uint32_t x = x0 + u, t = t0 + u;
            const bool act = x >= s && x < e && mine;
            const uint32_t qx = qs[u], rx = rs[u], mx = ms[u];
            const uint32_t ux = lane_diag(qx, rx, 0u - (mx & 1u));
            int32_t best = 0;
#pragma unroll
            for (int d = 1; d <= NR; d++) {
                if (d <= band) {
                    const int32_t k = d <= u ? lane_eval2(qx, ux, mx, nw[u - d], d) : lane_eval2(qx, ux, mx, P[d - 1 - u], d);
                    best = k > best ? k : best;
                }
            }
            if (!prune || __any(act && ftop[u] >= 0 && (best >> 7) < ftop[u] + 1 + ANCHOR_SCORE2 && ((far_diag >> ((ux >> 10) & 31u)) & 1u) && qx + 1u - P[NR - u].q1 <= (uint32_t)BP_CHAIN_BAND)) {
#pragma unroll
                for (int d = NR + 1; d <= W; d++) {
                    if (d <= band) {
                        const int32_t k = lane_eval2(qx, ux, mx, P[d - 1 - u], d);
                        best = k > best ? k : best;
                    }
                }
            }
            int32_t f = ANCHOR_SCORE2; uint32_t ridx = x - s, dep = 1;
            if (best > 0) {
                f = best >> 7;
                const uint32_t v = rd[(t - (127u - ((uint32_t)best & 127u))) & 31u][lane];
                ridx = v >> 14; dep = (v & 16383u) + 1;
            }
            rd[t & 31u][lane] = (ridx << 14) | dep;
            nw[u].q1 = qx + 1u; nw[u].u = ux; nw[u].m = act ? mx : 0xFFFFFFFFu; nw[u].f1 = act ? f - 1 : -1;
            if (act && f >= MIN_SCORE2) {
                const unsigned long long k64 = ((unsigned long long)(uint32_t)f << 28) | ((unsigned long long)(16383u - (x - s)) << 14) | dep;
                bool found = false;
#pragma unroll
                for (int j = 0; j < LANE_TREES; j++) {
                    const bool hit = sroot[j] == ridx;
                    found = found || hit;
                    if (hit && k64 > bk[j]) bk[j] = k64;
                }
                if (XT && !found && S > (uint32_t)LANE_TREES) {
                    const uint32_t nx = S - LANE_TREES < (uint32_t)XT ? S - LANE_TREES : (uint32_t)XT;
                    for (uint32_t j = 0; j < nx; j++)
                        if (s_xr[wave][j][lane] == ridx) { found = true; if (k64 > s_xk[wave][j][lane]) s_xk[wave][j][lane] = k64; break; }
                }
                if (!found) {
                    if (S >= (uint32_t)(LANE_TREES + XT)) ovf = true;
                    else if (XT && S >= (uint32_t)LANE_TREES) { s_xr[wave][S - LANE_TREES][lane] = ridx; s_xk[wave][S - LANE_TREES][lane] = k64; }
#pragma unroll
                    for (int j = 0; j < LANE_TREES; j++) if (S == (uint32_t)j) { sroot[j] = ridx; bk[j] = k64; }
                    S++;
                }
            }
        }
#pragma unroll
        for (int i = W - 1; i >= 4; i--) P[i] = P[i - 4];
        P[0] = nw[3]; P[1] = nw[2]; P[2] = nw[1]; P[3] = nw[0];
      }
    }
    if ((uint32_t)lane < rows_per_wave && slot < A.n_rows && real) {
        if (mine && !ovf) {
            uint32_t nc = 0, last = 0;
            for (uint32_t c = 0; c < S; c++) {
                uint32_t pick = 0xFFFFFFFFu; unsigned long long k = 0;
#pragma unroll
                for (int j = 0; j < LANE_TREES; j++)
                    if (sroot[j] != 0xFFFFFFFFu && (c == 0 || sroot[j] > last) && sroot[j] < pick) { pick = sroot[j]; k = bk[j]; }
                if (XT && S > (uint32_t)LANE_TREES)
                    for (uint32_t j = 0; j < S - LANE_TREES; j++) {
                        const uint32_t rt = s_xr[wave][j][lane];
                        if ((c == 0 || rt > last) && rt < pick) { pick = rt; k = s_xk[wave][j][lane]; }
                    }
                last = pick;
                const uint32_t xb = s + (16383u - (uint32_t)((k >> 14) & 16383u));
                const uint32_t q1 = A.anc[xb].x, rb = A.anc[xb].y;
                const uint32_t xr = s + pick, ra = A.anc[xr].y, o = s + nc;
                A.c_score[o] = (int32_t)(uint32_t)(k >> 28); A.c_q0[o] = A.anc[xr].x; A.c_q1[o] = q1;
                A.c_r0[o] = ra < rb ? ra : rb; A.c_r1[o] = ra < rb ? rb : ra;
                A.c_n[o] = (uint32_t)(k & 16383u); A.c_rc[o] = A.anc[xr].z >> 1;
                nc++;
            }
            ChunkOut o{};
            o.n_cand = nc; o.left = 0xFFFFFFFFu; o.right = 0;
            A.out[slot] = o;
        } else {
            A.ovf_list[atomicAdd(A.ovf_count, 1u)] = slot;
        }
    }
}

__global__ __launch_bounds__(64 * LANE_WAVES) __attribute__((amdgpu_waves_per_eu(3, 8))) void chain_lane20_kernel(ChainArgs A, uint32_t rows_per_wave) { chain_lane_body<20, 0>(A, rows_per_wave); }
__global__ __launch_bounds__(64 * LANE_WAVES) void chain_lane20x_kernel(ChainArgs A, uint32_t rows_per_wave) { chain_lane_body<20, LANE_XTREES>(A, rows_per_wave); }
__global__ __launch_bounds__(64 * LANE_WAVES) void chain_lane_kernel(ChainArgs A, uint32_t rows_per_wave) { chain_lane_body<LANE_N, 0>(A, rows_per_wave); }

__device__ __forceinline__ uint32_t lane_eval_d(uint32_t qx, uint32_t ux, uint32_t mx, const LaneAnchor& y, uint32_t d, int band) {
    const int32_t dq = (int32_t)(qx - y.q);
    const int32_t t = (int32_t)(ux - y.u), nt = (int32_t)(y.u - ux);
    const int32_t dr = dq - t;
    const int32_t gap = t > nt ? t : nt;
    const int32_t scp = y.f - gap;
    const uint32_t z = y.m ^ mx;
    const uint32_t bad = (uint32_t)(dq - 1) | (uint32_t)(BP_CHAIN_BAND - dq) | (uint32_t)(dr - 1) | (uint32_t)(MAX_GAP_LENGTH - gap) |
                         (uint32_t)(scp - 1) | z | (0u - z) | (uint32_t)(band - (int32_t)d);
    const uint32_t ok = (uint32_t)((int32_t)~bad >> 31);
    return ((((uint32_t)scp << 7) + (((uint32_t)ANCHOR_SCORE2 << 7) | 127u) - d)) & ok;
}

__global__ __launch_bounds__(64 * LANE_WAVES) void chain_quad_kernel(ChainArgs A) {
    __shared__ uint32_t s_rd[LANE_WAVES][32][16];
    const int wave = threadIdx.x >> 6, lane = threadIdx.x & 63, quad = lane >> 2;
    const uint32_t j = lane & 3;
    const uint32_t slot_i = (blockIdx.x * LANE_WAVES + wave) * 16 + quad;
    const uint32_t slot = A.row_order && slot_i < A.n_rows ? A.row_order[slot_i] : slot_i;
    uint32_t s = 0, e = 0;
    bool mine = false, real = false;
    const uint32_t pair = A.row_pair[slot < A.n_rows ? slot : A.n_rows - 1];
    if (slot < A.n_rows && slot - A.cbase[pair] < A.n_chunks[pair]) {
        const uint2 se = A.chunks[slot];
        s = se.x; e = se.y;
        real = true;
        mine = e > s && e - s < 16384;
    }
    const uint32_t s_al = s & ~3u;
    const uint32_t len = mine ? e - s_al : 0;
    uint32_t Wq[QUAD_N], Wr[QUAD_N], Wm[QUAD_N]; int32_t Wf[QUAD_N];
#pragma unroll
    for (int i = 0; i < QUAD_N; i++) { Wq[i] = 0; Wr[i] = 0; Wm[i] = 0xFFFFFFFFu; Wf[i] = 0; }
    unsigned long long bk[LANE_TREES];
    uint32_t sroot[LANE_TREES], bq[LANE_TREES], br[LANE_TREES];
#pragma unroll
    for (int k = 0; k < LANE_TREES; k++) { bk[k] = 0; sroot[k] = 0xFFFFFFFFu; bq[k] = br[k] = 0; }
    uint32_t S = 0;
    bool ovf = false;
    uint32_t (*rd)[16] = s_rd[wave];
    const int band = A.band;
    for (uint32_t t0 = 0; __any(t0 < len); t0 += 4) {
        const uint32_t x0 = s_al + t0;
        uint4 an0 = make_uint4(0, 0, 0, 0), an1 = an0, an2 = an0, an3 = an0;
        if (t0 < len) { an0 = A.anc[x0]; an1 = A.anc[x0 + 1]; an2 = A.anc[x0 + 2]; an3 = A.anc[x0 + 3]; }
        const uint32_t qs[4] = {an0.x, an1.x, an2.x, an3.x}, rs[4] = {an0.y, an1.y, an2.y, an3.y}, ms[4] = {an0.z, an1.z, an2.z, an3.z};
#pragma unroll
        for (int u = 0; u < 4; u++) {
            const uint32_t x = x0 + u, t = t0 + u;
            const bool act = x >= s && x < e && mine;
            const uint32_t qx = qs[u], rx = rs[u], mx = ms[u];
            const uint32_t ux = lane_diag(qx, rx, 0u - (mx & 1u));
            const uint32_t d0 = ((((uint32_t)u - j) - 1u) & 3u) + 1u;
            uint32_t best = 0;
#pragma unroll
            for (int i = 0; i < QUAD_N; i++) {
                LaneAnchor y; y.q = Wq[i]; y.u = Wr[i]; y.m = Wm[i]; y.f = Wf[i];
                const uint32_t k = lane_eval_d(qx, ux, mx, y, d0 + 4u * i, band);
                best = k > best ? k : best;
            }
            {
                uint32_t o = (uint32_t)__builtin_amdgcn_mov_dpp((int)best, 0xB1, 0xF, 0xF, true);
                best = o > best ? o : best;
                o = (uint32_t)__builtin_amdgcn_mov_dpp((int)best, 0x4E, 0xF, 0xF, true);
                best = o > best ? o : best;
            }
            int32_t f = ANCHOR_SCORE2; uint32_t ridx = x - s, dep = 1;
            if (best) {
                f = (int32_t)(best >> 7);
                const uint32_t v = rd[(t - (127u - (best & 127u))) & 31u][quad];
                ridx = v >> 14; dep = (v & 16383u) + 1;
            }
            rd[t & 31u][quad] = (ridx << 14) | dep;
            const bool own = j == (uint32_t)u;
#pragma unroll
            for (int i = QUAD_N - 1; i >= 1; i--) { Wq[i] = own ? Wq[i - 1] : Wq[i]; Wr[i] = own ? Wr[i - 1] : Wr[i]; Wm[i] = own ? Wm[i - 1] : Wm[i]; Wf[i] = own ? Wf[i - 1] : Wf[i]; }
            Wq[0] = own ? qx : Wq[0]; Wr[0] = own ? ux : Wr[0]; Wm[0] = own ? (act ? mx : 0xFFFFFFFFu) : Wm[0]; Wf[0] = own ? f : Wf[0];
            if (act && f >= MIN_SCORE2) {
                const unsigned long long k64 = ((unsigned long long)(uint32_t)f << 28) | ((unsigned long long)(16383u - (x - s)) << 14) | dep;
                bool found = false;
#pragma unroll
                for (int k = 0; k < LANE_TREES; k++) {
                    const bool hit = sroot[k] == ridx;
                    found = found || hit;
                    if (hit && k64 > bk[k]) { bk[k] = k64; bq[k] = qx; br[k] = rx; }
                }
                if (!found) {
                    if (S >= (uint32_t)LANE_TREES) ovf = true;
#pragma unroll
                    for (int k = 0; k < LANE_TREES; k++) if (S == (uint32_t)k) { sroot[k] = ridx; bk[k] = k64; bq[k] = qx; br[k] = rx; }
                    S++;
                }
            }
        }
    }
    if (j == 0 && slot < A.n_rows && real) {
        if (mine && !ovf) {
            uint32_t nc = 0, last = 0;
            for (uint32_t c = 0; c < S; c++) {
                uint32_t pick = 0xFFFFFFFFu; unsigned long long k = 0; uint32_t q1 = 0, rb = 0;
#pragma unroll
                for (int i = 0; i < LANE_TREES; i++)
                    if (sroot[i] != 0xFFFFFFFFu && (c == 0 || sroot[i] > last) && sroot[i] < pick) { pick = sroot[i]; k = bk[i]; q1 = bq[i]; rb = br[i]; }
                last = pick;
                const uint32_t xr = s + pick, ra = A.anc[xr].y, o = s + nc;
                A.c_score[o] = (int32_t)(uint32_t)(k >> 28); A.c_q0[o] = A.anc[xr].x; A.c_q1[o] = q1;
                A.c_r0[o] = ra < rb ? ra : rb; A.c_r1[o] = ra < rb ? rb : ra;
                A.c_n[o] = (uint32_t)(k & 16383u); A.c_rc[o] = A.anc[xr].z >> 1;
                nc++;
            }
            ChunkOut o{};
            o.n_cand = nc; o.left = 0xFFFFFFFFu; o.right = 0;
            A.out[slot] = o;
        } else {
            A.ovf_list[atomicAdd(A.ovf_count, 1u)] = slot;
        }
    }
}

__device__ __forceinline__ int32_t quad_eval(uint32_t qx, uint32_t ux, uint32_t mx, uint32_t yq1, uint32_t yu, uint32_t ym, int32_t yf1, int32_t dpj, int32_t bj) {
    const int32_t a = (int32_t)(qx - yq1);
    const int32_t t = (int32_t)(ux - yu), nt = (int32_t)(yu - ux);
    const int32_t gap = t > nt ? t : nt;
    const int32_t b = a - t;
    const int32_t s1 = yf1 - gap;
    const uint32_t z = ym ^ mx;
    const uint32_t bad = (uint32_t)a | (uint32_t)(BP_CHAIN_BAND - 1 - a) | (uint32_t)b | (uint32_t)(MAX_GAP_LENGTH - gap) | (uint32_t)s1 | z | (0u - z) | (uint32_t)(bj - dpj);
    const uint32_t key = ((uint32_t)s1 << 7) + (((((uint32_t)ANCHOR_SCORE2 + 1u) << 7) | 127u) - (uint32_t)dpj);
    return (int32_t)(key | (bad & 0x80000000u));
}
__global__ __launch_bounds__(64 * LANE_WAVES) void chain_quad_deep_kernel(ChainArgs A) {
    __shared__ uint32_t s_rd[LANE_WAVES][QD_RING][16];
    const int wave = threadIdx.x >> 6, lane = threadIdx.x & 63, quad = lane >> 2;
    const int32_t j = lane & 3;
    const uint32_t slot_i = (blockIdx.x * LANE_WAVES + wave) * 16 + quad;
    const uint32_t slot = A.row_order && slot_i < A.n_rows ? A.row_order[slot_i] : slot_i;
    uint32_t s = 0, e = 0;
    bool mine = false, real = false;
    const uint32_t pair = A.row_pair[slot < A.n_rows ? slot : A.n_rows - 1];
    if (slot < A.n_rows && slot - A.cbase[pair] < A.n_chunks[pair]) {
        const uint2 se = A.chunks[slot];
        s = se.x; e = se.y;
        real = true;
        mine = e > s && e - s < 16384;
    }
    const uint32_t s_al = s & ~3u;
    const uint32_t len = mine ? e - s_al : 0;
    uint32_t Wq[QD], Wu[QD], Wm[QD]; int32_t Wf[QD];
#pragma unroll
    for (int i = 0; i < QD; i++) { Wq[i] = 0; Wu[i] = 0; Wm[i] = 0xFFFFFFFFu; Wf[i] = -1; }
    static_assert(LANE_TREES == 4, "one tree slot per lane of the quad");
    unsigned long long my_bk = 0;
    uint32_t my_root = 0xFFFFFFFFu, my_bq = 0, my_br = 0;
    uint32_t S = 0;
    bool ovf = false;
    uint32_t (*rd)[16] = s_rd[wave];
    const int32_t bj = A.band + j;
    uint32_t far_diag = 0;
    for (uint32_t t0 = 0; __any(t0 < len); t0 += 4) {
        const uint32_t x0 = s_al + t0;
        uint4 an0 = make_uint4(0, 0, 0, 0), an1 = an0, an2 = an0, an3 = an0;
        if (t0 < len) { an0 = A.anc[x0]; an1 = A.anc[x0 + 1]; an2 = A.anc[x0 + 2]; an3 = A.anc[x0 + 3]; }
        const uint32_t qs[4] = {an0.x, an1.x, an2.x, an3.x}, rs[4] = {an0.y, an1.y, an2.y, an3.y}, ms[4] = {an0.z, an1.z, an2.z, an3.z};
        uint32_t nq = 0, nu = 0, nm = 0xFFFFFFFFu; int32_t nf = -1;
        int32_t far_top = -1;
        {
            if ((t0 & 63u) == 0) {
                far_diag = 0;
#pragma unroll
                for (int i = QD_NEAR; i < QD; i++) far_diag |= __builtin_amdgcn_alignbit(3u, 3u, 32u - (((Wu[i] - (uint32_t)MAX_GAP_LENGTH) >> 10) & 31u));
            } else far_diag |= __builtin_amdgcn_alignbit(3u, 3u, 32u - (((Wu[QD_NEAR] - (uint32_t)MAX_GAP_LENGTH) >> 10) & 31u));
#pragma unroll
            for (int i = QD_NEAR; i < QD; i++) far_top = Wf[i] > far_top ? Wf[i] : far_top;
            int32_t o = __builtin_amdgcn_mov_dpp(far_top, 0xB1, 0xF, 0xF, true); far_top = o > far_top ? o : far_top;
            o = __builtin_amdgcn_mov_dpp(far_top, 0x4E, 0xF, 0xF, true); far_top = o > far_top ? o : far_top;
        }
        uint32_t fd = far_diag;
        fd |= (uint32_t)__builtin_amdgcn_mov_dpp((int)fd, 0xB1, 0xF, 0xF, true); fd |= (uint32_t)__builtin_amdgcn_mov_dpp((int)fd, 0x4E, 0xF, 0xF, true);
#pragma unroll
        for (int u = 0; u < 4; u++) {
            const uint32_t x = x0 + u, t = t0 + u;
            const bool act = x >= s && x < e && mine;
            const uint32_t qx = qs[u], rx = rs[u], mx = ms[u];
            const uint32_t ux = lane_diag(qx, rx, 0u - (mx & 1u));
            int32_t best = 0;
#pragma unroll
            for (int i = 0; i < QD_NEAR; i++) {
                const int32_t k = quad_eval(qx, ux, mx, Wq[i], Wu[i], Wm[i], Wf[i], u + 4 * (i + 1), bj);
                best = k > best ? k : best;
            }
            {
                const bool late = u > j;
                const int32_t k = quad_eval(qx, ux, mx, late ? nq : Wq[QD - 1], late ? nu : Wu[QD - 1], late ? nm : Wm[QD - 1], late ? nf : Wf[QD - 1], late ? u : u + 4 * QD, bj);
                best = k > best ? k : best;
            }
            bool far;
            {
                int32_t nb = best;
                int32_t o = __builtin_amdgcn_mov_dpp(nb, 0xB1, 0xF, 0xF, true); nb = o > nb ? o : nb;
                o = __builtin_amdgcn_mov_dpp(nb, 0x4E, 0xF, 0xF, true); nb = o > nb ? o : nb;
                far = __any(act && far_top >= 0 && (nb >> 7) < far_top + 1 + ANCHOR_SCORE2 && ((fd >> ((ux >> 10) & 31u)) & 1u) && qx + 1u - Wq[QD_NEAR] <= (uint32_t)BP_CHAIN_BAND);
            }
            if (far) {
#pragma unroll
                for (int i = QD_NEAR; i < QD - 1; i++) {
                    const int32_t k = quad_eval(qx, ux, mx, Wq[i], Wu[i], Wm[i], Wf[i], u + 4 * (i + 1), bj);
                    best = k > best ? k : best;
                }
            }
            if (best > 0) best += j;
            {
                int32_t o = __builtin_amdgcn_mov_dpp(best, 0xB1, 0xF, 0xF, true);
                best = o > best ? o : best;
                o = __builtin_amdgcn_mov_dpp(best, 0x4E, 0xF, 0xF, true);
                best = o > best ? o : best;
            }
            int32_t f = ANCHOR_SCORE2; uint32_t ridx = x - s, dep = 1;
            if (best > 0) {
                f = best >> 7;
                const uint32_t v = rd[(t - (127u - ((uint32_t)best & 127u))) & (uint32_t)(QD_RING - 1)][quad];
                ridx = v >> 14; dep = (v & 16383u) + 1;
            }
            rd[t & (uint32_t)(QD_RING - 1)][quad] = (ridx << 14) | dep;
            if (j == u) { nq = qx + 1u; nu = ux; nm = act ? mx : 0xFFFFFFFFu; nf = act ? f - 1 : -1; }
            if (act && f >= MIN_SCORE2) {
                const unsigned long long k64 = ((unsigned long long)(uint32_t)f << 28) | ((unsigned long long)(16383u - (x - s)) << 14) | dep;
                const bool hit = my_root == ridx;
                if (hit && k64 > my_bk) { my_bk = k64; my_bq = qx; my_br = rx; }
                int fnd = hit ? 1 : 0;
                fnd |= __builtin_amdgcn_mov_dpp(fnd, 0xB1, 0xF, 0xF, true); fnd |= __builtin_amdgcn_mov_dpp(fnd, 0x4E, 0xF, 0xF, true);
                if (!fnd) {
                    if (S >= (uint32_t)LANE_TREES) ovf = true;
                    if (S == (uint32_t)j) { my_root = ridx; my_bk = k64; my_bq = qx; my_br = rx; }
                    S++;
                }
            }
        }
#pragma unroll
        for (int i = QD - 1; i >= 1; i--) { Wq[i] = Wq[i - 1]; Wu[i] = Wu[i - 1]; Wm[i] = Wm[i - 1]; Wf[i] = Wf[i - 1]; }
        Wq[0] = nq; Wu[0] = nu; Wm[0] = nm; Wf[0] = nf;
    }
    unsigned long long bk[LANE_TREES];
    uint32_t sroot[LANE_TREES], bq[LANE_TREES], br[LANE_TREES];
#pragma unroll
    for (int k = 0; k < LANE_TREES; k++) {
        const int src = (lane & ~3) + k;
        sroot[k] = (uint32_t)__shfl((int)my_root, src); bq[k] = (uint32_t)__shfl((int)my_bq, src); br[k] = (uint32_t)__shfl((int)my_br, src);
        bk[k] = ((unsigned long long)(uint32_t)__shfl((int)(uint32_t)(my_bk >> 32), src) << 32) | (uint32_t)__shfl((int)(uint32_t)my_bk, src);
    }
    if (j == 0 && slot < A.n_rows && real) {
        if (mine && !ovf) {
            uint32_t nc = 0, last = 0;
            for (uint32_t c = 0; c < S; c++) {
                uint32_t pick = 0xFFFFFFFFu; unsigned long long k = 0; uint32_t q1 = 0, rb = 0;
#pragma unroll
                for (int i = 0; i < LANE_TREES; i++)
                    if (sroot[i] != 0xFFFFFFFFu && (c == 0 || sroot[i] > last) && sroot[i] < pick) { pick = sroot[i]; k = bk[i]; q1 = bq[i]; rb = br[i]; }
                last = pick;
                const uint32_t xr = s + pick, ra = A.anc[xr].y, o = s + nc;
                A.c_score[o] = (int32_t)(uint32_t)(k >> 28); A.c_q0[o] = A.anc[xr].x; A.c_q1[o] = q1;
                A.c_r0[o] = ra < rb ? ra : rb; A.c_r1[o] = ra < rb ? rb : ra;
                A.c_n[o] = (uint32_t)(k & 16383u); A.c_rc[o] = A.anc[xr].z >> 1;
                nc++;
            }
            ChunkOut o{};
            o.n_cand = nc; o.left = 0xFFFFFFFFu; o.right = 0;
            A.out[slot] = o;
        } else {
            A.ovf_list[atomicAdd(A.ovf_count, 1u)] = slot;
        }
    }
}

__device__ __forceinline__ uint32_t wave_max_u32(uint32_t v) {
    uint32_t o = (uint32_t)__builtin_amdgcn_mov_dpp((int)v, 0xB1, 0xF, 0xF, true); v = o > v ? o : v;
    o = (uint32_t)__builtin_amdgcn_mov_dpp((int)v, 0x4E, 0xF, 0xF, true); v = o > v ? o : v;
    o = (uint32_t)__builtin_amdgcn_mov_dpp((int)v, 0x124, 0xF, 0xF, true); v = o > v ? o : v;
    o = (uint32_t)__builtin_amdgcn_mov_dpp((int)v, 0x128, 0xF, 0xF, true); v = o > v ? o : v;
    const uint32_t a = __builtin_amdgcn_readlane(v, 0), b = __builtin_amdgcn_readlane(v, 16), c = __builtin_amdgcn_readlane(v, 32), d = __builtin_amdgcn_readlane(v, 48);
    const uint32_t ab = a > b ? a : b, cd = c > d ? c : d;
    return ab > cd ? ab : cd;
}

struct ChainWaveLds {
    union {
        uint32_t ring[6][RING];
        uint32_t cand[7][64];
    };
    unsigned long long best[RMAX];
};
static_assert(sizeof(uint32_t) * 7 * 64 <= sizeof(uint32_t) * 6 * RING, "candidate staging fits the ring");

__device__ void chain_row_candidates(const ChainArgs& A, uint32_t s, uint32_t e, ChunkOut* op, ChainWaveLds& L, int lane, uint32_t R, bool fast);

__device__ void chain_chunk_row(const ChainArgs& A, uint32_t slot, ChainWaveLds& L, int lane) {
    const uint2 se = A.chunks[slot];
    const uint32_t s = se.x, e = se.y, n = e - s;
    ChunkOut* op = &A.out[slot];
    uint32_t (*ring)[RING] = L.ring;
    unsigned long long* s_best_w = L.best;
    bool fast = !A.force_serial && n < 16384;
    uint32_t R = 0;
    if (fast) {
        for (uint32_t base = s; base < e && fast; base += 64) {
            const uint32_t idx = base + lane;
            const bool have = idx < e;
            const uint4 my_a = have ? A.anc[idx] : make_uint4(0, 0, 0, 0);
            const uint32_t my_qp = my_a.x, my_rp = my_a.y, my_rm = my_a.z;
            const uint32_t cnt = e - base < 64 ? e - base : 64;
            for (uint32_t j = 0; j < cnt; j++) {
                const uint32_t x = base + j;
                const uint32_t qx = __builtin_amdgcn_readlane(my_qp, j), rx = __builtin_amdgcn_readlane(my_rp, j),
                               mx = __builtin_amdgcn_readlane(my_rm, j);
                const uint32_t avail = x - s;
                uint32_t key = 0;
                int sweeps = 1;
                if (avail > 64 && A.band > 64 && qx - ring[0][(x - 65) & (RING - 1)] <= (uint32_t)BP_CHAIN_BAND) sweeps = 2;
                for (int sw = 0; sw < sweeps; sw++) {
                    const uint32_t dist = lane + 1 + 64 * sw;
                    if (dist <= avail && dist <= (uint32_t)A.band) {
                        const uint32_t sl = (x - dist) & (RING - 1);
                        const uint32_t qy = ring[0][sl], ry = ring[1][sl], my = ring[2][sl];
                        const int32_t fy = (int32_t)ring[3][sl];
                        const int32_t dq = (int32_t)(qx - qy);
                        const int32_t dr = (mx & 1) ? (int32_t)(ry - rx) : (int32_t)(rx - ry);
                        const int32_t gap = dq > dr ? dq - dr : dr - dq;
                        const int32_t sc = fy + ANCHOR_SCORE2 - gap;
                        if (my == mx && dq > 0 && dq <= BP_CHAIN_BAND && dr > 0 && gap <= MAX_GAP_LENGTH && sc > ANCHOR_SCORE2) {
                            uint32_t k2 = ((uint32_t)sc << 7) | (127u - dist);
                            key = k2 > key ? k2 : key;
                        }
                    }
                }
                uint32_t best = wave_max_u32(key);
                int32_t f = ANCHOR_SCORE2; uint32_t rid, dep;
                if (best) {
                    f = (int32_t)(best >> 7);
                    const uint32_t sl = (x - (127u - (best & 127u))) & (RING - 1);
                    rid = ring[4][sl]; dep = ring[5][sl] + 1;
                } else {
                    rid = R++; dep = 1;
                    if (rid >= RMAX) { fast = false; break; }
                    if (lane == 0) s_best_w[rid] = (unsigned long long)avail << 49;
                }
                if (lane == 0) {
                    const uint32_t sl = x & (RING - 1);
                    ring[0][sl] = qx; ring[1][sl] = rx; ring[2][sl] = mx; ring[3][sl] = (uint32_t)f; ring[4][sl] = rid; ring[5][sl] = dep;
                    const unsigned long long old = s_best_w[rid];
                    const unsigned long long k64 = (old & ~((1ull << 49) - 1)) | ((unsigned long long)(uint32_t)f << 28) | ((unsigned long long)(16383u - avail) << 14) | dep;
                    if (k64 > old) s_best_w[rid] = k64;
                }
                lds_wave_sync();
            }
        }
    }
    chain_row_candidates(A, s, e, op, L, lane, R, fast);
}

__device__ void chain_row_candidates(const ChainArgs& A, uint32_t s, uint32_t e, ChunkOut* op, ChainWaveLds& L, int lane, uint32_t R, bool fast) {
    unsigned long long* s_best_w = L.best; uint32_t (*s_cand_w)[64] = L.cand;
    uint32_t C = 0;
    if (fast) {
        for (uint32_t r0 = 0; r0 < R && fast; r0 += 64) {
            const uint32_t r = r0 + lane;
            bool qual = false; uint32_t f = 0, lx = 0, dep = 0, rootx = 0;
            if (r < R) {
                unsigned long long bk = s_best_w[r];
                rootx = (uint32_t)(bk >> 49); bk &= (1ull << 49) - 1;
                f = (uint32_t)(bk >> 28); lx = 16383u - (uint32_t)((bk >> 14) & 16383u); dep = (uint32_t)(bk & 16383u);
                qual = dep >= MIN_ANCHORS && (int32_t)f >= MIN_SCORE2;
            }
            unsigned long long bal = __ballot(qual);
            uint32_t ci = C + __popcll(bal & ((1ull << lane) - 1));
            C += __popcll(bal);
            if (C > 64) { fast = false; break; }
            if (qual) {
                uint32_t xr = s + rootx, xb = s + lx;
                uint32_t ra = A.anc[xr].y, rb = A.anc[xb].y;
                s_cand_w[0][ci] = f; s_cand_w[1][ci] = A.anc[xr].x; s_cand_w[2][ci] = A.anc[xb].x;
                s_cand_w[3][ci] = ra < rb ? ra : rb; s_cand_w[4][ci] = ra < rb ? rb : ra; s_cand_w[5][ci] = dep;
                s_cand_w[6][ci] = A.anc[xr].z >> 1;
            }
        }
    }
    if (!fast) {
        if (lane == 0) {
            C = chain_chunk_serial(A, s, e);
            atomicAdd(&A.stats[1], 1u);
        }
    } else {
        lds_wave_sync();
        if ((uint32_t)lane < C) {
            A.c_score[s + lane] = (int32_t)s_cand_w[0][lane]; A.c_q0[s + lane] = s_cand_w[1][lane]; A.c_q1[s + lane] = s_cand_w[2][lane];
            A.c_r0[s + lane] = s_cand_w[3][lane]; A.c_r1[s + lane] = s_cand_w[4][lane]; A.c_n[s + lane] = s_cand_w[5][lane];
            A.c_rc[s + lane] = s_cand_w[6][lane];
        }
    }
    if (lane == 0) {
        ChunkOut o{};
        o.n_cand = C; o.left = 0xFFFFFFFFu; o.right = 0;
        *op = o;
    }
}

__global__ __launch_bounds__(64 * CHAIN_WAVES) void chain_chunk_kernel(ChainArgs A) {
    __shared__ ChainWaveLds s_lds[CHAIN_WAVES];
    const int wave = threadIdx.x >> 6, lane = threadIdx.x & 63;
    const uint32_t slot = blockIdx.x * CHAIN_WAVES + wave;
    const uint32_t pair = A.row_pair[slot < A.n_rows ? slot : A.n_rows - 1];
    if (slot >= A.n_rows) return;
    if (slot - A.cbase[pair] >= A.n_chunks[pair]) return;
    chain_chunk_row(A, slot, s_lds[wave], lane);
}

__global__ __launch_bounds__(64 * CHAIN_WAVES) void chain_chunk_list_kernel(ChainArgs A) {
    __shared__ ChainWaveLds s_lds[CHAIN_WAVES];
    const int wave = threadIdx.x >> 6, lane = threadIdx.x & 63;
    const uint32_t n_list = *A.ovf_count, n_waves = gridDim.x * CHAIN_WAVES;
    for (uint32_t k = blockIdx.x * CHAIN_WAVES + wave; k < n_list; k += n_waves) {
        chain_chunk_row(A, A.ovf_list[k], s_lds[wave], lane);
        lds_wave_sync();
    }
}

__global__ __launch_bounds__(256) void row_len_kernel(const uint2* __restrict__ chunks, const uint32_t* __restrict__ n_chunks, const uint32_t* __restrict__ cbase,
                                                      const uint32_t* __restrict__ row_pair, uint32_t n_rows, uint32_t* __restrict__ key, uint32_t* __restrict__ val) {
    const uint32_t r = blockIdx.x * 256u + threadIdx.x;
    if (r >= n_rows) return;
    const uint32_t p = row_pair[r];
    uint32_t len = 0;
    if (r - cbase[p] < n_chunks[p]) { const uint2 se = chunks[r]; len = se.y - se.x; len = (len + 7u) >> 3; len = len < 255u ? len : 255u; }
    key[r] = len; val[r] = r;
}

__device__ __forceinline__ void write_lane6(uint32_t lane, uint32_t& v0, uint32_t a0, uint32_t& v1, uint32_t a1, uint32_t& v2, uint32_t a2, uint32_t& v3, uint32_t a3,
                                            uint32_t& v4, uint32_t a4, uint32_t& v5, uint32_t a5) {
    uint32_t keep;
    asm volatile("s_mov_b32 %6, m0\n\ts_mov_b32 m0, %7\n\ts_nop 0\n\tv_writelane_b32 %0, %8, m0\n\tv_writelane_b32 %1, %9, m0\n\tv_writelane_b32 %2, %10, m0\n\t"
                 "v_writelane_b32 %3, %11, m0\n\tv_writelane_b32 %4, %12, m0\n\tv_writelane_b32 %5, %13, m0\n\ts_mov_b32 m0, %6"
                 : "+v"(v0), "+v"(v1), "+v"(v2), "+v"(v3), "+v"(v4), "+v"(v5), "=&s"(keep)
                 : "s"(lane), "s"(a0), "s"(a1), "s"(a2), "s"(a3), "s"(a4), "s"(a5));
}
struct RegWin { uint32_t q1, u, m; int32_t f1; uint32_t id, dp; };
__device__ __forceinline__ uint32_t wave_max_scalar(uint32_t v) {
    uint32_t o = (uint32_t)__builtin_amdgcn_mov_dpp((int)v, 0xB1, 0xF, 0xF, true); v = o > v ? o : v;
    o = (uint32_t)__builtin_amdgcn_mov_dpp((int)v, 0x4E, 0xF, 0xF, true); v = o > v ? o : v;
    o = (uint32_t)__builtin_amdgcn_mov_dpp((int)v, 0x124, 0xF, 0xF, true); v = o > v ? o : v;
    o = (uint32_t)__builtin_amdgcn_mov_dpp((int)v, 0x128, 0xF, 0xF, true); v = o > v ? o : v;
    asm volatile("s_nop 1\n\tv_max_u32_dpp %0, %0, %0 row_bcast:15 row_mask:0xa bank_mask:0xf\n\ts_nop 1\n\t"
                 "v_max_u32_dpp %0, %0, %0 row_bcast:31 row_mask:0xc bank_mask:0xf\n\ts_nop 1" : "+v"(v));
    return __builtin_amdgcn_readlane(v, 63);
}

template <int S, int T>
__device__ __forceinline__ void chain_reg_block(const ChainArgs& A, ChainWaveLds& L, uint32_t* s_root, const int lane, const uint32_t s, const uint32_t e, const uint32_t base,
                                                const uint32_t band, RegWin& w0, RegWin& w1, uint32_t& R, bool& over) {
    constexpr uint32_t WMASK = 64u * S - 1u;
    RegWin& wt = T ? w1 : w0;
    const uint32_t idx = base + lane;
    const uint4 my_a = idx < e ? A.anc[idx] : make_uint4(0, 0, 0, 0);
    const uint32_t cnt = e - base < 64 ? e - base : 64;
    for (uint32_t j = 0; j < cnt; j++) {
        const uint32_t qx = __builtin_amdgcn_readlane(my_a.x, j), rx = __builtin_amdgcn_readlane(my_a.y, j), mx = __builtin_amdgcn_readlane(my_a.z, j);
        const uint32_t avail = base + j - s;
        const uint32_t ux = lane_diag(qx, rx, 0u - (mx & 1u));
        const uint32_t d0 = (avail - (uint32_t)lane) & WMASK;
        int32_t key = lane_eval2(qx, ux, mx, LanePred{w0.q1, w0.u, w0.m, w0.f1}, (int)d0) | (int32_t)(((band - d0) | (d0 - 1u)) & 0x80000000u);
        key = key > 0 ? key : 0;
        if (S > 1) {
            const uint32_t d1 = (d0 - 64u) & WMASK;
            const int32_t k1 = lane_eval2(qx, ux, mx, LanePred{w1.q1, w1.u, w1.m, w1.f1}, (int)d1) | (int32_t)(((band - d1) | (d1 - 1u)) & 0x80000000u);
            key = k1 > key ? k1 : key;
        }
        const uint32_t best = wave_max_scalar((uint32_t)key);
        int32_t f = ANCHOR_SCORE2; uint32_t rid, dep;
        if (best) {
            f = (int32_t)(best >> 7);
            const uint32_t ps = (avail - (127u - (best & 127u))) & WMASK;
            rid = __builtin_amdgcn_readlane(w0.id, ps & 63u); dep = __builtin_amdgcn_readlane(w0.dp, ps & 63u);
            if (S > 1) {
                const uint32_t rid1 = __builtin_amdgcn_readlane(w1.id, ps & 63u), dep1 = __builtin_amdgcn_readlane(w1.dp, ps & 63u);
                if (ps >> 6) { rid = rid1; dep = dep1; }
            }
            dep++;
        } else {
            rid = R++; dep = 1;
            if (rid >= RMAX) { over = true; rid = 0; }
            else if (lane == 0) s_root[rid] = avail;
        }
        uint32_t f1 = (uint32_t)wt.f1;
        write_lane6(j, wt.q1, qx + 1u, wt.u, ux, wt.m, mx, f1, (uint32_t)(f - 1), wt.id, rid, wt.dp, dep);
        wt.f1 = (int32_t)f1;
    }
    if (!over && (uint32_t)lane < cnt)
        atomicMax(&L.best[wt.id], ((unsigned long long)(uint32_t)(wt.f1 + 1) << 28) | ((unsigned long long)(16383u - (base - s + (uint32_t)lane)) << 14) | wt.dp);
}

template <int S>
__device__ void chain_chunk_row_reg(const ChainArgs& A, uint32_t slot, ChainWaveLds& L, int lane) {
    static_assert(S == 1 || S == 2, "one or two window slots per lane");
    const uint2 se = A.chunks[slot];
    const uint32_t s = se.x, e = se.y, n = e - s;
    ChunkOut* op = &A.out[slot];
    bool fast = !A.force_serial && n < 16384;
    uint32_t R = 0;
    RegWin w0{0, 0, 0xFFFFFFFFu, 0, 0, 0}, w1 = w0;
    uint32_t* s_root = &L.ring[0][0];
    static_assert(RMAX <= 6 * RING, "root table fits the ring's space");
    const uint32_t band = (uint32_t)A.band;
    if (fast) {
#pragma unroll
        for (int u = 0; u < RMAX / 64; u++) L.best[lane + 64 * u] = 0;
        lds_wave_sync();
        bool over = false;
        for (uint32_t base = s; base < e && !over; base += 64u * S) {
            chain_reg_block<S, 0>(A, L, s_root, lane, s, e, base, band, w0, w1, R, over);
            if (S > 1 && base + 64u < e && !over) chain_reg_block<S, 1>(A, L, s_root, lane, s, e, base + 64u, band, w0, w1, R, over);
        }
        fast = !over;
    }
    if (fast) {
        lds_wave_sync();
#pragma unroll
        for (int u = 0; u < RMAX / 64; u++) if ((uint32_t)lane + 64u * u < R) L.best[lane + 64 * u] |= (unsigned long long)s_root[lane + 64 * u] << 49;
        lds_wave_sync();
    }
    chain_row_candidates(A, s, e, op, L, lane, R, fast);
}

template <int S>
__global__ __launch_bounds__(64 * CHAIN_WAVES) void chain_wave_reg_kernel(ChainArgs A) {
    __shared__ ChainWaveLds s_lds[CHAIN_WAVES];
    const int wave = __builtin_amdgcn_readfirstlane(threadIdx.x >> 6), lane = threadIdx.x & 63;
    const uint32_t slot = blockIdx.x * CHAIN_WAVES + wave;
    const uint32_t pair = A.row_pair[slot < A.n_rows ? slot : A.n_rows - 1];
    if (slot >= A.n_rows) return;
    if (slot - A.cbase[pair] >= A.n_chunks[pair]) return;
    chain_chunk_row_reg<S>(A, slot, s_lds[wave], lane);
}


template __global__ void chain_wave_reg_kernel<1>(ChainArgs A);
template __global__ void chain_wave_reg_kernel<2>(ChainArgs A);
```

### pyskani_amd/csrc/query_parts.h

```cpp
#pragma once
#include "chain_stages.h"
#include <deque>
#include <vector>
#include <cstring>

static inline size_t al256(size_t x) { return (x + 255) & ~(size_t)255; }

struct SwitchVal {
    char text[24]; bool set;
    const char* get() const { return set ? text : nullptr; }
    bool off() const { return EnvVal{get()}.off(); }
    int force() const { return EnvVal{get()}.force(); }
    double num(double dflt) const { return EnvVal{get()}.num(dflt); }
};
#define PSK_SWITCHES(X) \
    X(chain_serial, "PSK_CHAIN_SERIAL") \
    X(join_pairs, "PSK_JOIN_PAIRS") \
    X(emit_pairs, "PSK_EMIT_PAIRS") \
    X(xcd_group, "PSK_XCD_GROUP") \
    X(chunk_hops, "PSK_CHUNK_HOPS") \
    X(emit_heads, "PSK_EMIT_HEADS") \
    X(hops_items, "PSK_HOPS_ITEMS") \
    X(emit_expand, "PSK_EMIT_EXPAND") \
    X(chain_lane, "PSK_CHAIN_LANE") \
    X(lane_xtrees, "PSK_LANE_XTREES") \
    X(chain_quad_deep, "PSK_CHAIN_QUAD_DEEP") \
    X(chain_wave_reg, "PSK_CHAIN_WAVE_REG") \
    X(select_tiny, "PSK_SELECT_TINY") \
    X(big_solo, "PSK_BIG_SOLO") \
    X(huge_slots, "PSK_HUGE_SLOTS") \
    X(huge_min_seeds, "PSK_HUGE_MIN_SEEDS") \
    X(reduce_small, "PSK_REDUCE_SMALL") \
    X(reduce_wave, "PSK_REDUCE_WAVE") \
    X(reduce_tiny, "PSK_REDUCE_TINY") \
    X(join, "PSK_JOIN") \
    X(round_queries, "PSK_ROUND_QUERIES") \
    X(screen, "PSK_SCREEN") \
    X(prefilter, "PSK_PREFILTER") \
    X(gsi_join, "PSK_GSI_JOIN") \
    X(gsl_max_blocks, "PSK_GSL_MAX_BLOCKS") \
    X(probe, "PSK_PROBE") \
    X(gsi_slice, "PSK_GSI_SLICE") \
    X(bsi_small, "PSK_BSI_SMALL") \
    X(batch_items_log2, "PSK_BATCH_ITEMS_LOG2") \
    X(batch_pairs_log2, "PSK_BATCH_PAIRS_LOG2") \
    X(gsi_onepass, "PSK_GSI_ONEPASS") \
    X(pipeline, "PSK_PIPELINE") \
    X(screen_global, "PSK_SCREEN_GLOBAL") \
    X(screen_wave, "PSK_SCREEN_WAVE")
struct Switches {
#define X(field, name) SwitchVal field;
    PSK_SWITCHES(X)
#undef X
    static Switches read();
    bool join_wide() const { const char* e = join.get(); return e && !strcmp(e, "wide"); }
};

struct ScreenStaging { std::deque<std::vector<MarkerSet>> hq; std::deque<std::vector<uint32_t>> qoff; };
psk_status upload_marker_table(Lane* ctx, psk_db* db);
psk_status build_inverted(Lane* ctx, psk_db* db);
psk_status screen_many_device(Lane* ctx, psk_db* db, const psk_sketch* const* queries, uint32_t nq, double screen_val, int rescue_small, uint8_t* d_pass, ScreenStaging& keep, const Switches& sw);

SketchDesc make_desc(const psk_sketch* s, bool unindexed_ok = false);
__global__ __launch_bounds__(256) void pair_build_rows_kernel(const BatchQ* __restrict__ bq, const uint8_t* __restrict__ pass, uint32_t n_refs,
                                                              const SketchDesc* __restrict__ qd, const SketchDesc* __restrict__ rd,
                                                              PairDesc* __restrict__ pairs, uint32_t* __restrict__ sbase, uint32_t* __restrict__ cbase,
                                                              uint2* __restrict__ pair_qr, uint32_t n_pairs, uint32_t n_items, uint32_t n_rows);
__global__ __launch_bounds__(256) void pass_canon_kernel(uint8_t* __restrict__ pass, uint32_t n_refs, const uint32_t* __restrict__ canon);
__global__ __launch_bounds__(256) void pass_count_kernel(const uint8_t* __restrict__ pass, uint32_t n_refs, uint32_t* __restrict__ row_count, uint8_t* __restrict__ col_flag, uint32_t* __restrict__ row_blocks);
constexpr size_t CHAIN_ANCHOR_WORDS = 14;
struct ChainBufs {
    PairDesc* pairs; uint32_t *sbase, *cbase, *pstart; uint2* lbcnt; uint32_t* aoff; uint32_t* nch; uint2* chunks; ChunkOut* cout;
    psk_hit* hits; psk_hit* hits_sel; uint32_t* misc; uint32_t* ovf; unsigned long long* bsum; uint2* pair_qr; BatchQ* bq;
    uint32_t *blk_pair, *row_pair, *live, *big_list, *huge_list;
    uint32_t gi, gi_sum;
    unsigned long long* total;
    uint32_t rows_pair_max = 0xFFFFFFFFu;
    const uint32_t* g_key = nullptr; const unsigned long long* g_val = nullptr; const uint32_t* g_bucket = nullptr; int g_shift = 0;
    uint32_t g_nb1 = 0, g_blocks = 0; const unsigned long long* g_base = nullptr;
    const uint32_t* b_key = nullptr; const unsigned long long* b_val = nullptr; const uint32_t* b_bucket = nullptr; int b_shift = 0; uint32_t b_nb1 = 0, b_blocks = 0, b_max = 0; const unsigned long long* b_base = nullptr;
    const uint8_t* d_pass = nullptr; uint32_t n_refs = 0, n_bq = 0, p_cap = 0;
    bool gsi_slice = false; const uint2* gsl_tab = nullptr; uint32_t gsl_n_tab = 0; const uint2* gsl_ebase = nullptr; uint32_t *gsl_cnt = nullptr, *gsl_bm = nullptr, *gsl_un = nullptr, gsl_n_slices = 0; uint4* gsl_rec = nullptr;
    bool gsi_onepass = false;
};
psk_status chain_layout(Lane* ctx, size_t n_pairs, size_t n_items, size_t n_rows, size_t n_bq, ChainBufs* L);
psk_status chain_run(Lane* ctx, const ChainBufs& L, uint32_t n_pairs, size_t n_items, size_t n_rows, const psk_params& prm,
                     const psk_query_opts* o, const SketchDesc* d_qd, const SketchDesc* d_rd, uint64_t cap, bool wide, const Switches& sw, bool probe_ok = false);
uint64_t anchor_cap_for(Lane* ctx, size_t n_items, bool sparse = false, bool gb_scale = false);
struct ChainTail { uint32_t misc[16]; unsigned long long total64, visited, cands, rows; };
psk_status chain_check(const ChainTail& T, uint32_t n_pairs, uint64_t* cap, bool* wide, bool* retry);
struct HostPair { const psk_sketch* r; const psk_sketch* q; };
psk_status chain_batch(Lane* ctx, const HostPair* hp, uint32_t n_pairs, const psk_query_opts* o, psk_hit* out, const Switches& sw);

uint64_t index_stamp(const psk_db* db);
psk_status refresh_ref_descs(Lane* ctx, psk_db* db);

psk_status build_gsi(Lane* ctx, psk_db* db);
psk_status build_bsi(Lane* ctx, psk_db* db);
```

### pyskani_amd/csrc/seed_index.hip

```cpp
#include "query_parts.h"
#include <hipcub/hipcub.hpp>
#include <algorithm>

struct GsiSeg { const uint32_t* kmer; const uint64_t* pm; uint32_t n, off; };
__global__ __launch_bounds__(256) void gsi_gather_kernel(const GsiSeg* __restrict__ segs, uint32_t* __restrict__ key, unsigned long long* __restrict__ val) {
    const GsiSeg sg = segs[blockIdx.y];
    const unsigned long long ref = (unsigned long long)blockIdx.y << 48;
    for (uint32_t i = blockIdx.x * blockDim.x + threadIdx.x; i < sg.n; i += gridDim.x * blockDim.x) {
        const unsigned long long pm = sg.pm[i];
        const uint32_t meta = (uint32_t)pm;
        key[sg.off + i] = sg.kmer[i];
        val[sg.off + i] = ref | ((unsigned long long)(meta >> 1) << 33) | ((pm >> 32) << 1) | (meta & 1u);
    }
}
__global__ __launch_bounds__(256) void gsi_bucket_kernel(const uint32_t* __restrict__ key, uint32_t n, int shift, uint32_t nb, uint32_t* __restrict__ bucket) {
    const uint32_t i = blockIdx.x * 256u + threadIdx.x;
    if (i >= n) return;
    const uint32_t b = key[i] >> shift;
    const uint32_t from = i ? (key[i - 1] >> shift) + 1u : 0u;
    for (uint32_t x = from; x <= b; x++) bucket[x] = i;
    if (i == n - 1) for (uint32_t x = b + 1; x <= nb; x++) bucket[x] = n;
}
psk_status build_gsi(Lane* ctx, psk_db* db) {
    if (db->gsi_state) return PSK_OK;
    static const bool off = env_val("PSK_GSI").off();
    hipStream_t st = ctx->stream;
    const uint32_t n = (uint32_t)db->refs.size();
    db->gsi_state = 2;
    if (off || n == 0 || n > 65536u || db->params.k > 16) return PSK_OK;
    std::vector<GsiSeg> segs(n);
    uint64_t N = 0; uint32_t maxn = 0;
    for (uint32_t i = 0; i < n; i++) {
        const psk_sketch* r = db->refs[i];
        if (!r->has_seeds || r->contig_len.size() > 32768u || r->params.k != db->params.k || r->params.c != db->params.c) return PSK_OK;
        const uint32_t ns = r->store ? (uint32_t)r->n_seeds : 0u;
        segs[i] = GsiSeg{ns ? r->store->seed_kmer + r->seed_off : nullptr, ns ? r->store->seed_pm + r->seed_off : nullptr, ns, (uint32_t)N};
        N += ns; maxn = std::max(maxn, ns);
        if (N >= 0x7FFFFF00ull) return PSK_OK;
    }
    if (N == 0) return PSK_OK;
    const int kbits = 2 * db->params.k;
    int bits = 4; while (bits < 26 && (8ull << bits) < N) bits++;
    if (bits > kbits) bits = kbits;
    const uint32_t nb = 1u << bits;
    size_t ts = 0;
    PSK_HIP(hipcub::DeviceRadixSort::SortPairs(nullptr, ts, (const uint32_t*)nullptr, (uint32_t*)nullptr, (const unsigned long long*)nullptr, (unsigned long long*)nullptr, (int)N, 0, kbits, st));
    PoolScratch tmp;
    const size_t o_k = 0, o_v = al256(4 * (size_t)N), o_t = al256(o_v + 8 * (size_t)N), o_s = al256(o_t + ts), o_end = o_s + sizeof(GsiSeg) * (size_t)n;
    psk_status rc = tmp.reserve(ctx->dev, o_end + 256);
    if (rc == PSK_OK) rc = db->gsi_key.reserve(ctx->dev, 4 * (size_t)N + 256);
    if (rc == PSK_OK) rc = db->gsi_val.reserve(ctx->dev, 8 * (size_t)N + 256);
    if (rc == PSK_OK) rc = db->gsi_bucket.reserve(ctx->dev, 4 * ((size_t)nb + 2));
    if (rc != PSK_OK) { db->gsi_key.release(); db->gsi_val.release(); db->gsi_bucket.release(); return rc == PSK_ENOMEM ? PSK_OK : rc; }
    char* T = (char*)tmp.p;
    auto fail = [&](hipError_t e, const char* what) -> psk_status {
        (void)hipStreamSynchronize(st);
        db->gsi_key.release(); db->gsi_val.release(); db->gsi_bucket.release();
        psk_set_error("%s: %s", what, hipGetErrorString(e));
        return PSK_OK;
    };
    hipError_t e = hipMemcpyAsync(T + o_s, segs.data(), sizeof(GsiSeg) * (size_t)n, hipMemcpyHostToDevice, st);
    if (e != hipSuccess) return fail(e, "gsi: upload");
    hipLaunchKernelGGL(gsi_gather_kernel, dim3(std::max(1u, std::min(64u, (maxn + 4095u) / 4096u)), n), dim3(256), 0, st, (const GsiSeg*)(T + o_s), (uint32_t*)(T + o_k), (unsigned long long*)(T + o_v));
    e = hipcub::DeviceRadixSort::SortPairs(T + o_t, ts, (const uint32_t*)(T + o_k), (uint32_t*)db->gsi_key.p, (const unsigned long long*)(T + o_v), (unsigned long long*)db->gsi_val.p, (int)N, 0, kbits, st);
    if (e != hipSuccess) return fail(e, "gsi: sort");
    hipLaunchKernelGGL(gsi_bucket_kernel, dim3((uint32_t)((N + 255) / 256)), dim3(256), 0, st, (const uint32_t*)db->gsi_key.p, (uint32_t)N, kbits - bits, nb, (uint32_t*)db->gsi_bucket.p);
    e = hipStreamSynchronize(st);
    if (e != hipSuccess) return fail(e, "gsi: build");
    db->gsi_n = N; db->gsi_shift = kbits - bits;
    db->gsi_state = 1;
    return PSK_OK;
}

__global__ __launch_bounds__(256) void bsi_bucket_kernel(const uint32_t* __restrict__ key, uint32_t n, int shift, uint32_t nb, uint32_t* __restrict__ bucket, uint32_t base) {
    const uint32_t i = blockIdx.x * 256u + threadIdx.x;
    if (n == 0) { for (uint32_t x = i; x <= nb; x += gridDim.x * 256u) bucket[x] = base; return; }
    if (i >= n) return;
    const uint32_t b = key[i] >> shift;
    const uint32_t from = i ? (key[i - 1] >> shift) + 1u : 0u;
    for (uint32_t x = from; x <= b; x++) bucket[x] = base + i;
    if (i == n - 1) for (uint32_t x = b + 1; x <= nb; x++) bucket[x] = base + n;
}
psk_status build_bsi(Lane* ctx, psk_db* db) {
    if (db->bsi_state) return PSK_OK;
    static const bool off = env_val("PSK_GSI").off();
    hipStream_t st = ctx->stream;
    const uint32_t n = (uint32_t)db->refs.size();
    db->bsi_state = 2;
    if (off || n == 0 || db->params.k > 16) return PSK_OK;
    const uint32_t n_blocks = (n + (1u << BSI_BLOG) - 1) >> BSI_BLOG;
    std::vector<GsiSeg> segs(n);
    std::vector<uint64_t> base(n_blocks + 1, 0);
    uint64_t N = 0, max_block = 0; uint32_t maxn = 0;
    for (uint32_t b = 0; b < n_blocks; b++) {
        const uint32_t r0 = b << BSI_BLOG, r1 = std::min<uint32_t>(n, (b + 1) << BSI_BLOG);
        uint64_t in_block = 0;
        for (uint32_t i = r0; i < r1; i++) {
            const psk_sketch* r = db->refs[i];
            if (!r->has_seeds || r->contig_len.size() > 32768u || r->params.k != db->params.k || r->params.c != db->params.c) return PSK_OK;
            const uint32_t ns = r->store ? (uint32_t)r->n_seeds : 0u;
            if (in_block + ns >= 0x7FFFFF00ull) return PSK_OK;
            segs[i] = GsiSeg{ns ? r->store->seed_kmer + r->seed_off : nullptr, ns ? r->store->seed_pm + r->seed_off : nullptr, ns, (uint32_t)in_block};
            in_block += ns; maxn = std::max(maxn, ns);
        }
        base[b] = N; N += in_block; max_block = std::max(max_block, in_block);
    }
    base[n_blocks] = N;
    if (N == 0) return PSK_OK;
    const int kbits = 2 * db->params.k;
    int bits = 4; while (bits < 24 && (8ull << bits) < max_block) bits++;
    if (bits > kbits) bits = kbits;
    const uint32_t nb = 1u << bits;
    size_t ts = 0;
    PSK_HIP(hipcub::DeviceRadixSort::SortPairs(nullptr, ts, (const uint32_t*)nullptr, (uint32_t*)nullptr, (const unsigned long long*)nullptr, (unsigned long long*)nullptr, (int)max_block, 0, kbits, st));
    PoolScratch tmp;
    const size_t o_k = 0, o_v = al256(4 * (size_t)max_block), o_t = al256(o_v + 8 * (size_t)max_block), o_s = al256(o_t + ts), o_end = o_s + sizeof(GsiSeg) * (size_t)n;
    psk_status rc = tmp.reserve(ctx->dev, o_end + 256);
    if (rc == PSK_OK) rc = db->bsi_key.reserve(ctx->dev, 4 * (size_t)N + 256);
    if (rc == PSK_OK) rc = db->bsi_val.reserve(ctx->dev, 8 * (size_t)N + 256);
    if (rc == PSK_OK) rc = db->bsi_bucket.reserve(ctx->dev, 4 * ((size_t)n_blocks * (nb + 1) + 2));
    if (rc == PSK_OK) rc = db->bsi_base.reserve(ctx->dev, 8 * ((size_t)n_blocks + 1) + 256);
    auto drop = [&]() { db->bsi_key.release(); db->bsi_val.release(); db->bsi_bucket.release(); db->bsi_base.release(); };
    if (rc != PSK_OK) { drop(); if (rc == PSK_ENOMEM) return PSK_OK; return rc; }
    char* T = (char*)tmp.p;
    auto fail = [&](hipError_t e, const char* what) -> psk_status {
        (void)hipStreamSynchronize(st);
        drop();
        psk_set_error("%s: %s", what, hipGetErrorString(e));
        return PSK_OK;
    };
    hipError_t e = hipMemcpyAsync(T + o_s, segs.data(), sizeof(GsiSeg) * (size_t)n, hipMemcpyHostToDevice, st);
    if (e == hipSuccess) e = hipMemcpyAsync(db->bsi_base.p, base.data(), 8 * ((size_t)n_blocks + 1), hipMemcpyHostToDevice, st);
    if (e != hipSuccess) return fail(e, "bsi: upload");
    for (uint32_t b = 0; b < n_blocks; b++) {
        const uint32_t r0 = b << BSI_BLOG, r1 = std::min<uint32_t>(n, (b + 1) << BSI_BLOG);
        const size_t o = (size_t)base[b]; const uint32_t cnt = (uint32_t)(base[b + 1] - base[b]);
        if (cnt) {
            hipLaunchKernelGGL(gsi_gather_kernel, dim3(std::max(1u, std::min(64u, (maxn + 4095u) / 4096u)), r1 - r0), dim3(256), 0, st, (const GsiSeg*)(T + o_s) + r0, (uint32_t*)(T + o_k), (unsigned long long*)(T + o_v));
            size_t ts_b = ts;
            e = hipcub::DeviceRadixSort::SortPairs(T + o_t, ts_b, (const uint32_t*)(T + o_k), (uint32_t*)db->bsi_key.p + o, (const unsigned long long*)(T + o_v), (unsigned long long*)db->bsi_val.p + o, (int)cnt, 0, kbits, st);
            if (e != hipSuccess) return fail(e, "bsi: sort");
        }
        hipLaunchKernelGGL(bsi_bucket_kernel, dim3(std::max(1u, (cnt + 255u) / 256u)), dim3(256), 0, st, (const uint32_t*)db->bsi_key.p + o, cnt, kbits - bits, nb, (uint32_t*)db->bsi_bucket.p + (size_t)b * (nb + 1), 0u);
    }
    e = hipStreamSynchronize(st);
    if (e != hipSuccess) return fail(e, "bsi: build");
    db->bsi_n = N; db->bsi_shift = kbits - bits; db->bsi_nb1 = nb + 1; db->bsi_blocks = n_blocks;
    db->bsi_state = 1;
    return PSK_OK;
}

psk_status small_query_prepare(Lane* ctx, psk_db* db, std::shared_lock<std::shared_mutex>& sh, bool* ok) {
    *ok = false;
    const int state = db->small_state.load(std::memory_order_acquire);
    if (state == 1) { *ok = true; return PSK_OK; }
    if (state == 2) return PSK_OK;
    const uint32_t n = (uint32_t)db->refs.size();
    if (n == 0 || n > SQ_MAX_REFS) return PSK_OK;
    for (const psk_sketch* r : db->refs)
        if (!r->has_seeds || !r->store || r->params.k != db->params.k || r->params.c != db->params.c) { db->small_state = 2; return PSK_OK; }
    sh.unlock();
    psk_status rc = PSK_OK;
    {
        std::unique_lock<std::shared_mutex> ex(db->rw);
        if (db->refs.size() == n && db->small_state.load() == 0) {
            auto build = [&]() -> psk_status {
                PSK_TRY(upload_marker_table(ctx, db));
                PSK_TRY(build_inverted(ctx, db));
                if (db->has_dups && db->canon_dirty) {
                    PSK_TRY(db->d_canon.reserve(ctx->dev, 4 * (size_t)n));
                    PSK_HIP(hipMemcpyAsync(db->d_canon.p, db->canon.data(), 4 * (size_t)n, hipMemcpyHostToDevice, ctx->stream));
                    db->canon_dirty = false;
                }
                std::vector<const psk_sketch*> all_refs(db->refs.begin(), db->refs.end());
                PSK_TRY(ensure_index(ctx, all_refs.data(), (uint32_t)all_refs.size()));
                PSK_TRY(refresh_ref_descs(ctx, db));
                PSK_HIP(hipStreamSynchronize(ctx->stream));
                PSK_TRY(build_gsi(ctx, db));
                return PSK_OK;
            };
            rc = build();
            if (rc == PSK_OK) db->small_state.store(1, std::memory_order_release);
// ... 8 lines not shown
```

### pyskani_amd/csrc/select.hip

```cpp
#include "chain_stages.h"



__device__ __forceinline__ void sel_commit(const SelArgs& S, uint32_t row, uint32_t q0, uint32_t q1, uint32_t n) {
    ChunkOut* o = &S.out[row];
    atomicAdd(&o->anchors, n); atomicAdd(&o->n_intervals, 1u);
    atomicMin(&o->left, q0); atomicMax(&o->right, q1);
    atomicAdd((unsigned long long*)&o->cov_q, (unsigned long long)(q1 - q0) + 1 + S.two_c);
}

__device__ void select_serial(const SelArgs& S, uint32_t row0, uint32_t nrows) {
    for (uint32_t r = 0; r < nrows; r++) { uint32_t s = S.chunks[row0 + r].x, nc = S.out[row0 + r].n_cand; for (uint32_t i = 0; i < nc; i++) S.c_state[s + i] = 0; }
    for (;;) {
        int32_t best = -1; uint32_t brow = 0, bslot = 0;
        for (uint32_t r = 0; r < nrows; r++) {
            uint32_t s = S.chunks[row0 + r].x, nc = S.out[row0 + r].n_cand;
            for (uint32_t i = 0; i < nc; i++) if (S.c_state[s + i] == 0 && S.c_score[s + i] > best) { best = S.c_score[s + i]; brow = r; bslot = s + i; }
        }
        if (best < 0) break;
        bool ok = true;
        for (uint32_t r = 0; r < nrows && ok; r++) {
            uint32_t s = S.chunks[row0 + r].x, nc = S.out[row0 + r].n_cand;
            for (uint32_t i = 0; i < nc && ok; i++) if (S.c_state[s + i] == 1) {
                uint32_t j = s + i;
// ... 489 lines not shown
    SEL_STAMP();
#ifdef SEL_TRACE
    if (tid == 0 && G > 1) printf("SEL_TRACE pair %u C %u ncf %u G %u us: list %.0f sort %.0f max %.0f commit %.0f greedy %.0f\n", p, C, ncf, G, (t_ph[1] - t_ph[0]) * 0.01, (t_ph[2] - t_ph[1]) * 0.01, (t_ph[3] - t_ph[2]) * 0.01, (t_ph[4] - t_ph[3]) * 0.01, (t_ph[5] - t_ph[4]) * 0.01);
#endif
    if (tid == 0) atomicAdd(&S.stats[3], 1u);
}

__global__ __launch_bounds__(BIG_T) void select_big_kernel(BigArgs B) {
    __shared__ __attribute__((aligned(16))) unsigned char s_raw[12 * BIG_TILE];
    __shared__ uint32_t s_scan[BIG_T / 64 + 1];
    if (B.S.force_serial) return;
    const uint32_t n = *B.S.big_count;
    for (uint32_t k = blockIdx.x; k < n; k += gridDim.x) {
        const uint32_t p = B.S.big_list[k];
        const uint32_t n_cand = big_count_candidates(B.S, p, s_scan);
        if (n_cand > B.solo) { if (threadIdx.x == 0) { const uint32_t at = atomicAdd(B.huge_count, 1u); B.huge_list[at] = p; if (at < BIG_GROUPS) B.huge_c[at] = n_cand; } continue; }
        BigGrp g{1, 0, 0, nullptr, B.parts, B.parts + BIG_GMAX};
        g.part_a = B.parts + (size_t)(BIG_GROUPS + blockIdx.x) * 2 * BIG_GMAX; g.part_b = g.part_a + BIG_GMAX;
        select_big_pair(B, p, g, s_raw, s_scan);
        __syncthreads();
    }
}

__global__ __launch_bounds__(BIG_T) void select_huge_kernel(BigArgs B) {
    __shared__ __attribute__((aligned(16))) unsigned char s_raw[12 * BIG_TILE];
    __shared__ uint32_t s_scan[BIG_T / 64 + 1];
    const uint32_t n = *B.huge_count;
    if (n == 0) return;
    const uint32_t NB = gridDim.x;
    if (n <= BIG_GROUPS && NB >= 8 && NB >= 2 * n) {
        const uint32_t l = (blockIdx.x & 7u) * (NB >> 3) + (blockIdx.x >> 3);
        unsigned long long total = 0;
        for (uint32_t k = 0; k < n; k++) total += B.huge_c[k];
        uint32_t start = 0, gid = 0, G = 1; unsigned long long cum = 0;
        for (uint32_t k = 0; k < n; k++) {
            cum += B.huge_c[k];
            uint32_t end = k + 1 == n ? NB : (uint32_t)((unsigned long long)NB * cum / (total ? total : 1ull));
            if (end < start + 1u) end = start + 1u;
            if (end > NB - (n - 1u - k)) end = NB - (n - 1u - k);
            if (l >= start && l < end) { gid = k; G = end - start; break; }
            start = end;
        }
        BigGrp g{G, l - start, 0, B.ctr + gid, B.parts + (size_t)gid * 2 * BIG_GMAX, B.parts + (size_t)gid * 2 * BIG_GMAX + BIG_GMAX};
        select_big_pair(B, B.huge_list[gid], g, s_raw, s_scan);
        return;
    }
    uint32_t groups = 1; while (groups < n && groups < BIG_GROUPS && groups < NB) groups <<= 1;
    const uint32_t G = NB / groups;
    uint32_t gid, gr;
    if (NB < 8) { gid = blockIdx.x / G; gr = blockIdx.x % G; }
    else {
        const uint32_t xcd = blockIdx.x & 7, sl = blockIdx.x >> 3, per_xcd = NB >> 3;
        if (groups >= 8) { const uint32_t gpx = groups >> 3; gid = xcd * gpx + sl / G; gr = sl % G; }
        else { gid = xcd % groups; gr = (xcd / groups) * per_xcd + sl; }
    }
    BigGrp g{G, gr, 0, B.ctr + gid, B.parts + (size_t)gid * 2 * BIG_GMAX, B.parts + (size_t)gid * 2 * BIG_GMAX + BIG_GMAX};
    for (uint32_t k = gid; k < n; k += groups) {
        select_big_pair(B, B.huge_list[k], g, s_raw, s_scan);
        __syncthreads();
    }
}

__device__ uint32_t seeds_between(const PairDesc& P, uint32_t qc, uint32_t lo, uint32_t hi) {
    const uint32_t* __restrict__ pos = P.q_seed_pos_base;
    uint32_t a = P.q_contig_start[qc], b = P.q_contig_start[qc + 1];
    uint32_t l = a, r = b;
    while (l < r) { uint32_t m = (l + r) >> 1; if (pos[m] < lo) l = m + 1; else r = m; }
    uint32_t first = l; r = b;
    if (first + 256u < b && pos[first + 256u] > hi) r = first + 256u;
    while (l < r) { uint32_t m = (l + r) >> 1; if (pos[m] <= hi) l = m + 1; else r = m; }
    return l - first;
}

__global__ __launch_bounds__(256) void chunk_seeds_kernel(ChainArgs A) {
    uint32_t row = blockIdx.x * blockDim.x + threadIdx.x;
    const uint32_t pair = A.row_pair[row < A.n_rows ? row : A.n_rows - 1];
    if (row >= A.n_rows) return;
    if (row - A.cbase[pair] >= A.n_chunks[pair]) return;
    ChunkOut* o = &A.out[row];
    if (!o->n_intervals) return;
    const uint2 ch0 = A.chunks[row];
    if (ch0.x > ch0.y || ch0.y > A.cap) return;
    const uint32_t nc = A.pairs[pair].q_nc;
    const uint32_t qc = nc == 1u ? 0u : A.anc[ch0.x].w;
    if (qc < nc) o->seeds = seeds_between(A.pairs[pair], qc, o->left, o->right);
}
```

### pyskani_amd/csrc/slice_join.h

```cpp
#pragma once
#include "common.h"

struct BatchQ { uint32_t q, rank_lo, rank_hi, pair_off, item_off, row_off; };
constexpr uint32_t GSI_PMAX = 256;

#ifndef GSL_SEEDS_N
#define GSL_SEEDS_N 256
#endif
constexpr uint32_t GSL_SEEDS = GSL_SEEDS_N;
constexpr uint32_t GSL_WORDS = GSL_SEEDS / 32;
constexpr uint32_t GSL_BT_WORDS = 12;
struct GslArgs {
    const BatchQ* bq; uint32_t n_entries;
    const uint2* tab; uint32_t n_tab;
    const uint2* ebase;
    uint32_t* un; uint32_t n_slices;
    const uint8_t* pass; uint32_t n_refs; const SketchDesc* qd;
    const uint32_t* g_key; const unsigned long long* g_val; const uint32_t* g_bucket; int g_shift;
    const unsigned long long* g_base;
    uint32_t g_nb1, g_blocks;
    uint32_t* blk_tab; uint32_t* blk_cnt; uint32_t blk_cap;
    uint32_t* cnt;
    uint4* rec;
    uint32_t* bm;
    uint32_t* pair_cnt;
    const uint32_t* pstart; uint4* anc; uint32_t cap; uint32_t* err;
    uint32_t p_cap;
    uint2* chunks; uint32_t* n_chunks;
};

void gsl_make_tab(const BatchQ* bq, size_t n_entries, const uint32_t* q_seeds , std::vector<uint2>& tab, std::vector<uint2>& ebase, uint64_t* n_records, uint64_t* n_slices);
psk_status gsl_blocks_launch(const BatchQ* bq, uint32_t n_entries, const uint8_t* pass, uint32_t n_refs, uint32_t g_blocks, const unsigned long long* g_base,
                             uint32_t* blk_tab, uint32_t* blk_cnt, uint32_t blk_cap, hipStream_t st);
psk_status gsl_count_launch(const GslArgs& A, hipStream_t st);
psk_status gsl_heads_launch(const GslArgs& A, hipStream_t st);
psk_status gsl_emit_launch(const GslArgs& A, hipStream_t st);
```

### pyskani_amd/csrc/slice_join.hip

```cpp
#include "slice_join.h"
#include "chain_dev.h"

void gsl_make_tab(const BatchQ* bq, size_t n_entries, const uint32_t* q_seeds, std::vector<uint2>& tab, std::vector<uint2>& ebase, uint64_t* n_records, uint64_t* n_slices) {
    tab.clear(); ebase.resize(n_entries);
    uint64_t rec = 0, nsl_all = 0; uint32_t max_sl = 0;
    for (size_t e = 0; e < n_entries; e++) {
        const uint32_t nsl = (q_seeds[e] + GSL_SEEDS - 1) / GSL_SEEDS;
        ebase[e] = make_uint2((uint32_t)rec, (uint32_t)nsl_all);
        rec += (uint64_t)nsl * (bq[e].rank_hi - bq[e].rank_lo);
        nsl_all += nsl;
        max_sl = std::max(max_sl, nsl);
    }
    *n_records = rec; *n_slices = nsl_all;
    (void)max_sl;
    for (size_t e = 0; e < n_entries; e++) for (uint32_t sl = 0; sl < (q_seeds[e] + GSL_SEEDS - 1) / GSL_SEEDS; sl++) tab.push_back(make_uint2((uint32_t)e, sl));
}

#ifndef GSL_LINE_N
#define GSL_LINE_N 4
#endif
constexpr uint32_t GSL_LW = GSL_LINE_N, GSL_LM = GSL_LW - 1u, GSL_LS = GSL_LW == 8 ? 3u : GSL_LW == 4 ? 2u : 1u;
static_assert(GSL_LW == 8 || GSL_LW == 4 || GSL_LW == 2, "a staged line holds eight, four or two anchors");
static size_t gsl_walk_lds(const GslArgs& A, bool emit) {
    const size_t nw = (A.n_refs + 63) / 64;
    (void)nw;
    return (emit ? (16 * GSL_LW + 8 + 8) * (size_t)A.p_cap + 8 * 64 : 0) + 64 + 4 * (size_t)A.p_cap + (emit ? 0 : 4 * (size_t)GSL_WORDS * (A.p_cap + 1));
}

template <bool EMIT>
__global__ __launch_bounds__(64) void gsl_walk_kernel(GslArgs A) {
    extern __shared__ uint4 s_gsl[];
    const int lane = threadIdx.x;
    const uint2 te = A.tab[blockIdx.x];
    if (te.x == 0xFFFFFFFFu) return;
    if (EMIT && (A.err[5] || *(const unsigned long long*)(A.err + 16) > A.cap)) return;
    const BatchQ B = A.bq[te.x];
    const SketchDesc Q = A.qd[B.q];
    const uint32_t sb = te.y * GSL_SEEDS;
    if (sb >= Q.n) return;
    const uint32_t se = Q.n - sb > GSL_SEEDS ? sb + GSL_SEEDS : Q.n;
    const uint32_t P = B.rank_hi - B.rank_lo, pc = A.p_cap;
    const uint2 eb = A.ebase[te.x];
    const uint32_t rec0 = eb.x + te.y * P;
    uint4* s_line = s_gsl;
    unsigned long long* s_lim = (unsigned long long*)(s_gsl + (EMIT ? GSL_LW * pc : 0u));
    uint2* s_cs = (uint2*)(s_lim + (EMIT ? pc : 0u));
    uint2* s_fl = s_cs + (EMIT ? pc : 0u);
    uint2* s_bp = s_fl + (EMIT ? 64u : 0u);
    uint32_t* s_cur = (uint32_t*)(s_bp + 8u);
    uint32_t* s_rows = s_cur;
    uint32_t* s_bm = s_cur + pc;
    {
        if (EMIT) for (uint32_t j = lane; j < P; j += 64) { const uint4 v = A.rec[rec0 + j]; s_cs[j] = make_uint2(v.x, v.x); s_rows[j] = v.y; s_lim[j] = ((unsigned long long)v.w << 32) | v.z; }
        else {
            for (uint32_t j = lane; j < P; j += 64) s_cur[j] = 0;
            for (uint32_t x = lane; x < GSL_WORDS * (pc + 1u); x += 64) s_bm[x] = 0;
        }
    }
    uint32_t unw = 0;
    if (EMIT && lane < (int)GSL_WORDS) unw = A.un[(size_t)(eb.y + te.y) * GSL_WORDS + lane];
    lds_wave_sync();
    constexpr uint32_t GSL_AHEAD = 4;
    unsigned long long visited = 0;
    const uint32_t n_blk = A.blk_cnt[te.x];
    const uint32_t* __restrict__ brow = A.blk_tab + (size_t)te.x * A.blk_cap * GSL_BT_WORDS;
#pragma unroll 1
    for (uint32_t bi = 0; bi < n_blk; bi++, brow += GSL_BT_WORDS) {
    {
    const uint32_t blk = brow[8];
    const unsigned long long x_base = ((unsigned long long)brow[11] << 32) | brow[10];
    const uint32_t* __restrict__ x_key = A.g_key + x_base; const unsigned long long* __restrict__ x_val = A.g_val + x_base;
    {
        lds_wave_sync();
        if (lane < 8) {
            uint32_t run = brow[9];
#pragma unroll
            for (int u = 0; u < 7; u++) { const uint32_t w = brow[u]; if (u < lane) run += (uint32_t)__popc(w); }
            s_bp[lane] = make_uint2(brow[lane], run);
        }
        lds_wave_sync();
    }
    const uint32_t* __restrict__ bkt = A.g_bucket + (size_t)blk * A.g_nb1;
    uint32_t km1 = sb + (uint32_t)lane < se ? Q.kmer[sb + lane] : 0u, km2 = sb + 64u + (uint32_t)lane < se ? Q.kmer[sb + 64u + lane] : 0u;
    uint32_t lo1 = 0, hi1 = 0;
    if (sb + (uint32_t)lane < se) { const uint32_t b = km1 >> A.g_shift; lo1 = bkt[b]; hi1 = bkt[b + 1]; }
    for (uint32_t c0 = sb; c0 < se; c0 += 64) {
        const uint32_t i = c0 + (uint32_t)lane;
        const uint32_t km = km1, lo = lo1, hi = hi1;
        km1 = km2; lo1 = 0; hi1 = 0;
        if (i + 64u < se) { const uint32_t b = km1 >> A.g_shift; lo1 = bkt[b]; hi1 = bkt[b + 1]; }
        km2 = i + 128u < se ? Q.kmer[i + 128u] : 0u;
        uint32_t qp = 0, qm = 0;
        if (EMIT && i < se) { qp = Q.pos[i]; qm = Q.meta[i]; }
        const uint32_t nst = (hi - lo + 63u) >> 6;
        if (!EMIT) visited += hi - lo;
        uint32_t pre = nst;
#pragma unroll
        for (int o = 1; o < 64; o <<= 1) { const uint32_t y = __shfl_up(pre, o); if (lane >= o) pre += y; }
        const uint32_t T = (uint32_t)__builtin_amdgcn_readlane((int)pre, 63);
        pre -= nst;
        uint32_t ns[GSL_AHEAD], nx[GSL_AHEAD], nh[GSL_AHEAD], nk[GSL_AHEAD]; unsigned long long nv[GSL_AHEAD];
#define GSL_FETCH(t, u) do { \
            ns[u] = 0; nx[u] = 0; nh[u] = 0; nk[u] = 0xFFFFFFFFu; nv[u] = 0ull; \
            if ((t) < T) { \
                const unsigned long long own = __ballot(nst != 0 && pre <= (t)); \
                ns[u] = 63u - (uint32_t)__clzll((long long)own); \
                nx[u] = (uint32_t)__builtin_amdgcn_readlane((int)lo, (int)ns[u]) + 64u * ((t) - (uint32_t)__builtin_amdgcn_readlane((int)pre, (int)ns[u])); \
                nh[u] = (uint32_t)__builtin_amdgcn_readlane((int)hi, (int)ns[u]); \
                if (nx[u] + (uint32_t)lane < nh[u]) { nk[u] = x_key[nx[u] + lane]; nv[u] = x_val[nx[u] + lane]; } \
            } } while (0)
#pragma unroll
        for (uint32_t u = 0; u < GSL_AHEAD; u++) GSL_FETCH(u, u);
        for (uint32_t t0 = 0; t0 < T; t0 += GSL_AHEAD) {
            uint32_t cs[GSL_AHEAD], cx[GSL_AHEAD], ch[GSL_AHEAD], ck[GSL_AHEAD]; unsigned long long cv[GSL_AHEAD];
#pragma unroll
            for (uint32_t u = 0; u < GSL_AHEAD; u++) { cs[u] = ns[u]; cx[u] = nx[u]; ch[u] = nh[u]; ck[u] = nk[u]; cv[u] = nv[u]; }
#pragma unroll
            for (uint32_t u = 0; u < GSL_AHEAD; u++) GSL_FETCH(t0 + GSL_AHEAD + u, u);
            uint32_t slots[GSL_AHEAD]; uint2 bps[GSL_AHEAD];
#pragma unroll
            for (uint32_t u = 0; u < GSL_AHEAD; u++) bps[u] = s_bp[(uint32_t)(cv[u] >> 53) & 7u];
#pragma unroll
            for (uint32_t u = 0; u < GSL_AHEAD; u++) {
                const uint32_t skm = (uint32_t)__builtin_amdgcn_readlane((int)km, (int)cs[u]);
                const uint32_t b = (uint32_t)(cv[u] >> 48) & 31u, rk = bps[u].y + (uint32_t)__popc(bps[u].x & ~(~0u << b)) - B.rank_lo;
                const bool ok = cx[u] + (uint32_t)lane < ch[u] && ck[u] == skm && ((bps[u].x >> b) & 1u) && rk < P;
                slots[u] = ok ? rk : 0xFFFFFFFFu;
            }
#pragma unroll
            for (uint32_t u = 0; u < GSL_AHEAD; u++) {
                if (t0 + u >= T) break;
                const uint32_t s = cs[u]; const unsigned long long v = cv[u];
                const uint32_t slot = slots[u];
                const bool valid = slot != 0xFFFFFFFFu;
                if (!__any(valid)) continue;
                const uint32_t jl = c0 - sb + s;
                if (!EMIT) {
                    if (valid) { atomicAdd(&s_cur[slot], 1u); atomicOr(&s_bm[(jl >> 5) * (pc + 1u) + slot], 1u << (jl & 31u)); }
                    continue;
                }
                const uint32_t sqp = (uint32_t)__builtin_amdgcn_readlane((int)qp, (int)s), sqm = (uint32_t)__builtin_amdgcn_readlane((int)qm, (int)s);
                const uint32_t rmeta = (uint32_t)((((v >> 33) & 0x7FFFull) << 1) | (v & 1ull));
                const uint4 av = make_uint4(sqp, (uint32_t)(v >> 1), (rmeta & ~1u) | ((rmeta ^ sqm) & 1u), sqm >> 1);
                const uint32_t prev = (uint32_t)__builtin_amdgcn_update_dpp(-1, (int)slot, 0x138 , 0xf, 0xf, false);
                const bool same = valid && prev == slot;
                const bool dup = __ballot(same) != 0;
                const uint2 cs = s_cs[valid ? slot : 0u];
                const uint32_t base = cs.x;
                if (((uint32_t)__builtin_amdgcn_readlane((int)unw, (int)(jl >> 5)) >> (jl & 31u)) & 1u) {
                    if (valid && !same) {
                        const unsigned long long key1 = (((unsigned long long)(sqm >> 1) << 32) | sqp) + 1ull;
                        if (key1 > s_lim[slot]) {
                            const uint32_t row = s_rows[slot], idxc = base < A.cap ? base : A.cap;
                            if (row < Q.rows) {
                                uint2* r = A.chunks + ((size_t)B.row_off + (size_t)slot * Q.rows + row);
                                r->x = idxc;
                                if (row > 0) r[-1].y = idxc;
                            } else atomicOr(A.err, 1u);
                            s_rows[slot] = row + 1u; s_lim[slot] = key1 + FRAGMENT_LENGTH;
                        }
                    }
                }
                if (!dup) {
                    const uint32_t t3 = base & GSL_LM;
                    if (valid) { s_cs[slot].x = base + 1u; s_line[t3 * pc + slot] = av; }
                    const bool fl = valid && t3 == GSL_LM;
                    const unsigned long long fm = __ballot(fl);
                    if (fm) {
                        if (fl) {
                            const uint32_t st0 = cs.y, lb = base & ~GSL_LM, ft = lb >= st0 ? 0u : st0 - lb;
                            s_fl[__popcll(fm & ((1ull << lane) - 1ull))] = make_uint2(slot | (ft << 16), lb);
                        }
                        lds_wave_sync();
                        const uint32_t nf = (uint32_t)__popcll(fm), t = (uint32_t)lane & GSL_LM;
                        for (uint32_t g0 = 0; g0 < nf; g0 += 64u / GSL_LW) {
                            const uint32_t r2 = g0 + ((uint32_t)lane >> GSL_LS);
                            if (r2 < nf) { const uint2 f = s_fl[r2]; if (t >= (f.x >> 16)) A.anc[f.y + t] = s_line[t * pc + (f.x & 0xFFFFu)]; }
                        }
                    }
                    continue;
                }
                const uint32_t st0 = cs.y;
                const uint32_t next = (uint32_t)__builtin_amdgcn_update_dpp(-1, (int)slot, 0x130 , 0xf, 0xf, false);
                const bool last = valid && next != slot;
                const unsigned long long starts = __ballot(valid && !same);
                const unsigned long long upto = starts & (lane == 63 ? ~0ull : ((2ull << lane) - 1ull));
                const uint32_t jj = valid ? (uint32_t)lane - (63u - (uint32_t)__clzll((long long)upto)) : 0u;
                const unsigned long long ends = __ballot(last);
                const uint32_t tail = valid ? (uint32_t)__ffsll((long long)(ends >> lane)) - 1u : 0u;
                const uint32_t d = base + jj, e = d + tail, lastline = e >> GSL_LS;
                if (valid && jj == 0 && (base >> GSL_LS) != lastline && e < A.cap) {
                    const uint32_t f0 = (base & ~GSL_LM) > st0 ? (base & ~GSL_LM) : st0;
                    for (uint32_t t = f0; t < base; t++) A.anc[t] = s_line[(t & GSL_LM) * pc + slot];
                }
                lds_wave_sync();
                if (valid) {
                    if ((d >> GSL_LS) == lastline) s_line[(d & GSL_LM) * pc + slot] = av;
                    else if (e < A.cap) A.anc[d] = av;
                }
                lds_wave_sync();
                if (last) {
                    if (e >= A.cap) atomicOr(A.err, 2u);
                    else if ((e & GSL_LM) == GSL_LM) {
                        const uint32_t f0 = (e & ~GSL_LM) > st0 ? (e & ~GSL_LM) : st0;
                        for (uint32_t t = f0; t <= e; t++) A.anc[t] = s_line[(t & GSL_LM) * pc + slot];
                    }
                    s_cs[slot].x = e + 1u;
                }
                lds_wave_sync();
            }
        }
#undef GSL_FETCH
    }
    }
    }
    lds_wave_sync();
    if (!EMIT) {
#pragma unroll
        for (int o = 32; o > 0; o >>= 1) visited += __shfl_xor(visited, o);
        if (lane == 0 && visited) atomicAdd((unsigned long long*)(A.err + 18), visited);
        for (uint32_t j = lane; j < P; j += 64) {
            const uint32_t c = s_cur[j];
            A.cnt[rec0 + j] = c;
            if (c) atomicAdd(&A.pair_cnt[B.pair_off + j], c);
        }
        for (uint32_t x = lane; x < P * GSL_WORDS; x += 64) { const uint32_t j = x / GSL_WORDS, w = x % GSL_WORDS; A.bm[(size_t)(rec0 + j) * GSL_WORDS + w] = s_bm[w * (pc + 1u) + j]; }
    } else {
        for (uint32_t j = lane; j < P; j += 64) {
            const uint32_t c = s_cs[j].x, st0 = s_cs[j].y;
            if (c > st0 && (c & GSL_LM) && c <= A.cap) {
                const uint32_t f0 = ((c - 1u) & ~GSL_LM) > st0 ? ((c - 1u) & ~GSL_LM) : st0;
                for (uint32_t t = f0; t < c; t++) A.anc[t] = s_line[(t & GSL_LM) * pc + j];
            }
        }
    }
}

constexpr uint32_t GSL_HK = GSL_SEEDS / 64;
__global__ __launch_bounds__(64) void gsl_heads_kernel(GslArgs A) {
    __shared__ unsigned long long s_key[GSL_SEEDS];
    __shared__ uint32_t s_bm[64 * (GSL_WORDS + 1)];
    __shared__ uint32_t s_un[GSL_WORDS];
    const int lane = threadIdx.x;
    const uint32_t e = blockIdx.x;
    const BatchQ B = A.bq[e];
// ... 137 lines not shown
```

Measured before the change: 190.6 million genome-pairs/s.

## Pack chain anchors into 8 bytes with per-row query base offsets

On the slice-join path, anchors are now stored as 8-byte packed records instead of 16 bytes. Each one holds a 16-bit query position relative to its row start, the reference position, and the contig/strand meta. The per-row query base and query contig move to a new row_q0 array, and every chaining DP kernel is templated on PK so it unpacks anchors and adds q0 back when writing chain output. This halves anchor traffic in the emit stage, the LDS line buffers and the chaining reads, and shrinks LDS use in the emit kernel. In exchange it adds unpack arithmetic, doubles the number of compiled kernel variants, and depends on the relative-offset computation being correct for rows that continue across fragments.

Result: faster. 199.5 million genome-pairs/s (median of 6 runs) (+4.7%).

```diff
diff --git a/pyskani_amd/csrc/chain.hip b/pyskani_amd/csrc/chain.hip
--- a/pyskani_amd/csrc/chain.hip
+++ b/pyskani_amd/csrc/chain.hip
@@ -131,7 +131,7 @@
     size_t o_pairs = 0, o_sbase = al256(o_pairs + sizeof(PairDesc) * n_pairs), o_cbase = al256(o_sbase + 4 * (n_pairs + 1)),
            o_pstart = al256(o_cbase + 4 * (n_pairs + 1)), o_lb = al256(o_pstart + 4 * (n_pairs + 1)),
            o_aoff = al256(o_lb + 8 * (n_items + 1)), o_nch = al256(o_aoff + 4 * (n_items + 1)),
-           o_chunks = al256(o_nch + 4 * n_pairs), o_cout = al256(o_chunks + sizeof(uint2) * n_rows),
+           o_chunks = al256(o_nch + 4 * n_pairs), o_rq0 = al256(o_chunks + sizeof(uint2) * n_rows), o_cout = al256(o_rq0 + sizeof(uint2) * n_rows),
            o_misc = al256(o_cout + sizeof(ChunkOut) * n_rows), o_hits = o_misc + 256, o_sel = al256(o_hits + sizeof(psk_hit) * n_pairs),
            o_ovf = al256(o_sel + sizeof(psk_hit) * n_pairs), o_bsum = al256(o_ovf + 4 * n_rows),
            o_qr = al256(o_bsum + 8 * (gi_sum + 1)), o_bq = al256(o_qr + 8 * n_pairs), o_bp = al256(o_bq + sizeof(BatchQ) * (n_bq + 1)),
@@ -140,7 +140,7 @@
     PSK_TRY(ctx->q_b.reserve(o_end));
     char* B = (char*)ctx->q_b.p;
     L->pairs = (PairDesc*)(B + o_pairs); L->sbase = (uint32_t*)(B + o_sbase); L->cbase = (uint32_t*)(B + o_cbase); L->pstart = (uint32_t*)(B + o_pstart);
-    L->lbcnt = (uint2*)(B + o_lb); L->aoff = (uint32_t*)(B + o_aoff); L->nch = (uint32_t*)(B + o_nch); L->chunks = (uint2*)(B + o_chunks);
+    L->lbcnt = (uint2*)(B + o_lb); L->aoff = (uint32_t*)(B + o_aoff); L->nch = (uint32_t*)(B + o_nch); L->chunks = (uint2*)(B + o_chunks); L->row_q0 = (uint2*)(B + o_rq0);
     L->cout = (ChunkOut*)(B + o_cout); L->hits = (psk_hit*)(B + o_hits); L->hits_sel = (psk_hit*)(B + o_sel); L->misc = (uint32_t*)(B + o_misc);
     L->ovf = (uint32_t*)(B + o_ovf); L->bsum = (unsigned long long*)(B + o_bsum); L->pair_qr = (uint2*)(B + o_qr); L->bq = (BatchQ*)(B + o_bq);
     L->blk_pair = (uint32_t*)(B + o_bp); L->row_pair = (uint32_t*)(B + o_rp); L->live = (uint32_t*)(B + o_live); L->big_list = (uint32_t*)(B + o_big); L->huge_list = (uint32_t*)(B + o_huge);
@@ -188,7 +188,7 @@
         if (gsl) {
             GL.bq = L.bq; GL.n_entries = L.n_bq; GL.tab = L.gsl_tab; GL.n_tab = L.gsl_n_tab; GL.ebase = L.gsl_ebase; GL.pass = L.d_pass; GL.n_refs = L.n_refs; GL.qd = d_qd;
             GL.g_key = L.g_key; GL.g_val = L.g_val; GL.g_bucket = L.g_bucket; GL.g_shift = L.g_shift; GL.g_nb1 = L.g_nb1; GL.g_blocks = L.g_blocks; GL.g_base = L.g_base; GL.blk_tab = d_btab; GL.blk_cnt = d_bcnt; GL.blk_cap = bcap; GL.cnt = L.gsl_cnt; GL.rec = L.gsl_rec; GL.bm = L.gsl_bm; GL.un = L.gsl_un; GL.n_slices = L.gsl_n_slices;
-            GL.pair_cnt = L.big_list; GL.pstart = L.pstart; GL.cap = (uint32_t)cap; GL.err = L.misc; GL.p_cap = L.p_cap; GL.chunks = L.chunks; GL.n_chunks = L.nch;
+            GL.pair_cnt = L.big_list; GL.pstart = L.pstart; GL.cap = (uint32_t)cap; GL.err = L.misc; GL.p_cap = L.p_cap; GL.chunks = L.chunks; GL.n_chunks = L.nch; GL.row_q0 = L.row_q0;
             PSK_HIP(hipMemsetAsync(L.big_list, 0, 4 * ((size_t)n_pairs + 1), st));
             PSK_TRY(gsl_count_launch(GL, st));
         }
@@ -270,6 +270,7 @@
     uint32_t* a_nxt = D + 4 * na;
     ChainArgs A{};
     A.anc = anc;
+    A.row_q0 = gsl ? L.row_q0 : nullptr;
     A.sc_ptr = D + 5 * na;
     A.sc_f = (int32_t*)E4; A.sc_root = E4 + na; A.sc_depth = E4 + 2 * na; A.sc_best = E4 + 3 * na;
     uint32_t* CAND = D + 6 * na;
@@ -298,7 +299,7 @@
         hipLaunchKernelGGL(chunk_hops_sliced_kernel, dim3(n_pairs, HOP_SLICES), dim3(64), 0, sd, L.pstart, a_nxt, anc, L.pairs, L.cbase, n_pairs, slice_cnt, 1, scratch_rows, L.chunks, L.nch, L.misc);
         PSK_HIP(hipEventRecord(ctx->side_join, sd));
     }
-    if (gsl) { GL.anc = anc; PSK_TRY(gsl_heads_launch(GL, st)); PSK_TRY(gsl_emit_launch(GL, st)); }
+    if (gsl) { GL.anc = (uint2*)anc; PSK_TRY(gsl_heads_launch(GL, st)); PSK_TRY(gsl_emit_launch(GL, st)); }
     else if (gsi_join) { GA.anc = anc; GA.chunks = L.chunks; GA.n_chunks = L.nch; GA.onepass = gsi_one ? 1 : 0; GA.total = L.total; if (gsi_one) GA.pair_cnt = L.aoff;
                     hipLaunchKernelGGL(gsi_join_kernel<true>, dim3(L.n_bq), dim3(64), gsi_lds_emit, st, GA); }
     else if (wide) hipLaunchKernelGGL(anchor_emit_kernel, dim3(gi), dim3(256), 0, st, L.pairs, L.sbase, n_pairs, (uint32_t)n_items, L.lbcnt, L.aoff, anc, (uint32_t)cap, L.misc, L.blk_pair);
@@ -358,24 +359,24 @@
             const bool quad = le && le[0] == 'q' ? true : (le_rows >= 8 ? false : n_rows < 32 * 1024);
             if (quad) {
                 const uint32_t qw = (uint32_t)((n_rows + 15) / 16);
-                hipLaunchKernelGGL(chain_quad_kernel, dim3((qw + LANE_WAVES - 1) / LANE_WAVES), dim3(64 * LANE_WAVES), 0, st, A);
+                hipLaunchKernelGGL(gsl ? chain_quad_kernel<true> : chain_quad_kernel<false>, dim3((qw + LANE_WAVES - 1) / LANE_WAVES), dim3(64 * LANE_WAVES), 0, st, A);
             } else {
                 const int xt_force = sw.lane_xtrees.force();
                 const bool xtrees = xt_force >= 0 ? xt_force == 1 : n_items / n_pairs > (1u << 20);
-                if (A.band <= 20 && xtrees) hipLaunchKernelGGL(chain_lane20x_kernel, dim3((waves + LANE_WAVES - 1) / LANE_WAVES), dim3(64 * LANE_WAVES), 0, st, A, rpw);
-                else if (A.band <= 20) hipLaunchKernelGGL(chain_lane20_kernel, dim3((waves + LANE_WAVES - 1) / LANE_WAVES), dim3(64 * LANE_WAVES), 0, st, A, rpw);
-                else hipLaunchKernelGGL(chain_lane_kernel, dim3((waves + LANE_WAVES - 1) / LANE_WAVES), dim3(64 * LANE_WAVES), 0, st, A, rpw);
+                const auto lane_k = A.band <= 20 && xtrees ? (gsl ? chain_lane20x_kernel<true> : chain_lane20x_kernel<false>)
+                                  : A.band <= 20 ? (gsl ? chain_lane20_kernel<true> : chain_lane20_kernel<false>) : (gsl ? chain_lane_kernel<true> : chain_lane_kernel<false>);
+                hipLaunchKernelGGL(lane_k, dim3((waves + LANE_WAVES - 1) / LANE_WAVES), dim3(64 * LANE_WAVES), 0, st, A, rpw);
             }
             const uint32_t lw = (uint32_t)std::min<size_t>((n_rows + CHAIN_WAVES - 1) / CHAIN_WAVES, 2048);
-            hipLaunchKernelGGL(chain_chunk_list_kernel, dim3(lw), dim3(64 * CHAIN_WAVES), 0, st, A);
+            hipLaunchKernelGGL(gsl ? chain_chunk_list_kernel<true> : chain_chunk_list_kernel<false>, dim3(lw), dim3(64 * CHAIN_WAVES), 0, st, A);
         }
     }
     const int wr_force = sw.chain_wave_reg.force();
     const bool wave_reg = !A.lane_dp && !force_serial && A.band < 128 && (wr_force >= 0 ? wr_force == 1 : n_rows <= 2048);
     if (wave_reg) {
         const dim3 g((uint32_t)((n_rows + CHAIN_WAVES - 1) / CHAIN_WAVES)), b(64 * CHAIN_WAVES);
-        if (A.band < 64) hipLaunchKernelGGL(chain_wave_reg_kernel<1>, g, b, 0, st, A);
-        else hipLaunchKernelGGL(chain_wave_reg_kernel<2>, g, b, 0, st, A);
+        const auto reg_k = A.band < 64 ? (gsl ? chain_wave_reg_kernel<1, true> : chain_wave_reg_kernel<1, false>) : (gsl ? chain_wave_reg_kernel<2, true> : chain_wave_reg_kernel<2, false>);
+        hipLaunchKernelGGL(reg_k, g, b, 0, st, A);
     }
     const bool quad_deep = !wave_reg && !A.lane_dp && !force_serial && !sw.chain_quad_deep.off() && A.band <= 4 * QD && !sw.chain_lane.off();
     if (quad_deep) {
@@ -383,12 +384,12 @@
         A.lane_dp = 1;
         PSK_TRY(order_rows());
         const uint32_t qw = (uint32_t)((n_rows + 15) / 16);
-        hipLaunchKernelGGL(chain_quad_deep_kernel, dim3((qw + LANE_WAVES - 1) / LANE_WAVES), dim3(64 * LANE_WAVES), 0, st, A);
+        hipLaunchKernelGGL(gsl ? chain_quad_deep_kernel<true> : chain_quad_deep_kernel<false>, dim3((qw + LANE_WAVES - 1) / LANE_WAVES), dim3(64 * LANE_WAVES), 0, st, A);
         const uint32_t lw = (uint32_t)std::min<size_t>((n_rows + CHAIN_WAVES - 1) / CHAIN_WAVES, 2048);
-        hipLaunchKernelGGL(chain_chunk_list_kernel, dim3(lw), dim3(64 * CHAIN_WAVES), 0, st, A);
+        hipLaunchKernelGGL(gsl ? chain_chunk_list_kernel<true> : chain_chunk_list_kernel<false>, dim3(lw), dim3(64 * CHAIN_WAVES), 0, st, A);
     }
     if (!A.lane_dp && !wave_reg)
-    hipLaunchKernelGGL(chain_chunk_kernel, dim3((uint32_t)((n_rows + CHAIN_WAVES - 1) / CHAIN_WAVES)), dim3(64 * CHAIN_WAVES), 0, st, A);
+    hipLaunchKernelGGL(gsl ? chain_chunk_kernel<true> : chain_chunk_kernel<false>, dim3((uint32_t)((n_rows + CHAIN_WAVES - 1) / CHAIN_WAVES)), dim3(64 * CHAIN_WAVES), 0, st, A);
     ctx->t_end();
     SelArgs SA{};
     SA.chunks = L.chunks; SA.n_chunks = L.nch; SA.cbase = L.cbase; SA.n_pairs = n_pairs;
diff --git a/pyskani_amd/csrc/chain_dev.h b/pyskani_amd/csrc/chain_dev.h
--- a/pyskani_amd/csrc/chain_dev.h
+++ b/pyskani_amd/csrc/chain_dev.h
@@ -8,6 +8,31 @@
     __builtin_amdgcn_wave_barrier();
     __builtin_amdgcn_fence(__ATOMIC_ACQUIRE, "workgroup");
 }
+
+static_assert(FRAGMENT_LENGTH < (1u << 16), "q_rel fills the low 16 bits of a packed anchor");
+static_assert(GSI_CONTIG_BITS + 1 <= 16, "ref contig << 1 | strand fills the high 16 bits of a packed anchor");
+__device__ __forceinline__ uint2 pk_anchor(uint32_t q_rel, uint32_t r, uint32_t m) { return make_uint2((q_rel & 0xFFFFu) | (m << 16), r); }
+__device__ __forceinline__ uint4 pk_unpack(uint2 a) { return make_uint4(a.x & 0xFFFFu, a.y, a.x >> 16, 0u); }
+template <bool PK> struct AncRd {
+    const void* a;
+    __device__ __forceinline__ uint4 operator[](size_t i) const { return PK ? pk_unpack(((const uint2*)a)[i]) : ((const uint4*)a)[i]; }
+    static constexpr int W4 = PK ? 2 : 4;
+    __device__ __forceinline__ void load4w(size_t i, uint4 (&w)[W4]) const {
+        const uint4* p = PK ? (const uint4*)((const uint2*)a + i) : (const uint4*)a + i;
+#pragma unroll
+        for (int k = 0; k < W4; k++) w[k] = p[k];
+    }
+    static __device__ __forceinline__ void unpack4(const uint4 (&w)[W4], uint4 (&o)[4]) {
+        if (PK) {
+#pragma unroll
+            for (int k = 0; k < 2; k++) { o[2 * k] = pk_unpack(make_uint2(w[k].x, w[k].y)); o[2 * k + 1] = pk_unpack(make_uint2(w[k].z, w[k].w)); }
+        } else {
+#pragma unroll
+            for (int k = 0; k < 4; k++) o[k] = w[k % W4];
+        }
+    }
+    __device__ __forceinline__ void load4(size_t i, uint4 (&o)[4]) const { uint4 w[W4]; load4w(i, w); unpack4(w, o); }
+};
 
 struct LaneAnchor { uint32_t q, u, m; int32_t f; };
 __device__ __forceinline__ uint32_t lane_diag(uint32_t qx, uint32_t rx, uint32_t sg) { return qx - ((rx ^ sg) - sg); }
diff --git a/pyskani_amd/csrc/chain_stages.h b/pyskani_amd/csrc/chain_stages.h
--- a/pyskani_amd/csrc/chain_stages.h
+++ b/pyskani_amd/csrc/chain_stages.h
@@ -58,6 +58,7 @@
 
 struct ChainArgs {
     const uint4* anc;
+    const uint2* row_q0;
     const uint2* chunks; const uint32_t* n_chunks; const uint32_t* cbase; uint32_t n_pairs, n_rows;
     const uint32_t* row_pair;
     const uint32_t* row_order;
@@ -238,16 +239,16 @@
 __global__ __launch_bounds__(64) void chunk_hops_items_kernel(const uint32_t* __restrict__ pstart, const uint32_t* __restrict__ aoff,
                                                                const PairDesc* __restrict__ pairs, const uint32_t* __restrict__ sbase, const uint32_t* __restrict__ cbase,
                                                                uint32_t n_pairs, uint32_t* __restrict__ slice_cnt, uint2* __restrict__ scratch, uint32_t* __restrict__ err);
-__global__ __launch_bounds__(64 * LANE_WAVES) __attribute__((amdgpu_waves_per_eu(3, 8))) void chain_lane20_kernel(ChainArgs A, uint32_t rows_per_wave);
-__global__ __launch_bounds__(64 * LANE_WAVES) void chain_lane20x_kernel(ChainArgs A, uint32_t rows_per_wave);
-__global__ __launch_bounds__(64 * LANE_WAVES) void chain_lane_kernel(ChainArgs A, uint32_t rows_per_wave);
-__global__ __launch_bounds__(64 * LANE_WAVES) void chain_quad_kernel(ChainArgs A);
-__global__ __launch_bounds__(64 * LANE_WAVES) void chain_quad_deep_kernel(ChainArgs A);
-__global__ __launch_bounds__(64 * CHAIN_WAVES) void chain_chunk_kernel(ChainArgs A);
-__global__ __launch_bounds__(64 * CHAIN_WAVES) void chain_chunk_list_kernel(ChainArgs A);
+template <bool PK> __global__ __launch_bounds__(64 * LANE_WAVES) __attribute__((amdgpu_waves_per_eu(3, 8))) void chain_lane20_kernel(ChainArgs A, uint32_t rows_per_wave);
+template <bool PK> __global__ __launch_bounds__(64 * LANE_WAVES) void chain_lane20x_kernel(ChainArgs A, uint32_t rows_per_wave);
+template <bool PK> __global__ __launch_bounds__(64 * LANE_WAVES) void chain_lane_kernel(ChainArgs A, uint32_t rows_per_wave);
+template <bool PK> __global__ __launch_bounds__(64 * LANE_WAVES) void chain_quad_kernel(ChainArgs A);
+template <bool PK> __global__ __launch_bounds__(64 * LANE_WAVES) void chain_quad_deep_kernel(ChainArgs A);
+template <bool PK> __global__ __launch_bounds__(64 * CHAIN_WAVES) void chain_chunk_kernel(ChainArgs A);
+template <bool PK> __global__ __launch_bounds__(64 * CHAIN_WAVES) void chain_chunk_list_kernel(ChainArgs A);
 __global__ __launch_bounds__(256) void row_len_kernel(const uint2* __restrict__ chunks, const uint32_t* __restrict__ n_chunks, const uint32_t* __restrict__ cbase,
                                                       const uint32_t* __restrict__ row_pair, uint32_t n_rows, uint32_t* __restrict__ key, uint32_t* __restrict__ val);
-template <int S>
+template <int S, bool PK>
 __global__ __launch_bounds__(64 * CHAIN_WAVES) void chain_wave_reg_kernel(ChainArgs A);
 __global__ __launch_bounds__(256) void select_tiny_kernel(SelArgs S);
 __global__ __launch_bounds__(64) void select_kernel(SelArgs S, uint32_t* __restrict__ mid_list, uint32_t* __restrict__ mid_count);
diff --git a/pyskani_amd/csrc/common.h b/pyskani_amd/csrc/common.h
--- a/pyskani_amd/csrc/common.h
+++ b/pyskani_amd/csrc/common.h
@@ -478,6 +478,7 @@
 
 
 constexpr int BSI_BLOG = 8;
+constexpr uint32_t GSI_CONTIG_BITS = 15;
 constexpr uint32_t SQ_MAX_TILES = 64, SQ_MAX_DESC = 64;
 constexpr uint32_t SQ_SEEDS = 3072;
 constexpr uint32_t SQ_MARKERS = 2048;
diff --git a/pyskani_amd/csrc/dp.hip b/pyskani_amd/csrc/dp.hip
--- a/pyskani_amd/csrc/dp.hip
+++ b/pyskani_amd/csrc/dp.hip
@@ -5,15 +5,17 @@
 
 
 
-__device__ uint32_t chain_chunk_serial(const ChainArgs& A, uint32_t s, uint32_t e) {
+template <bool PK>
+__device__ uint32_t chain_chunk_serial(const ChainArgs& A, uint32_t s, uint32_t e, uint32_t q0) {
+    const AncRd<PK> an{A.anc};
     for (uint32_t x = s; x < e; x++) {
         int32_t bs = ANCHOR_SCORE2; uint32_t bp = x;
-        uint32_t qx = A.anc[x].x, rx = A.anc[x].y, mx = A.anc[x].z;
+        uint32_t qx = an[x].x, rx = an[x].y, mx = an[x].z;
         for (uint32_t y = x; y-- > s && x - y <= (uint32_t)A.band;) {
-            if (A.anc[y].z != mx) continue;
-            int64_t dq = (int64_t)qx - (int64_t)A.anc[y].x;
+            if (an[y].z != mx) continue;
+            int64_t dq = (int64_t)qx - (int64_t)an[y].x;
             if (dq > BP_CHAIN_BAND) break;
-            int64_t dr = (mx & 1) ? (int64_t)A.anc[y].y - (int64_t)rx : (int64_t)rx - (int64_t)A.anc[y].y;
+            int64_t dr = (mx & 1) ? (int64_t)an[y].y - (int64_t)rx : (int64_t)rx - (int64_t)an[y].y;
             if (dq <= 0 || dr <= 0) continue;
             int64_t gap = dq > dr ? dq - dr : dr - dq;
             if (gap > MAX_GAP_LENGTH) continue;
@@ -31,10 +33,10 @@
         if (A.sc_root[x] != x) continue;
         uint32_t b = A.sc_best[x];
         if (A.sc_depth[b] < MIN_ANCHORS || A.sc_f[b] < MIN_SCORE2) continue;
-        uint32_t ra = A.anc[x].y, rb = A.anc[b].y;
-        A.c_score[s + nc] = A.sc_f[b]; A.c_q0[s + nc] = A.anc[x].x; A.c_q1[s + nc] = A.anc[b].x;
+        uint32_t ra = an[x].y, rb = an[b].y;
+        A.c_score[s + nc] = A.sc_f[b]; A.c_q0[s + nc] = an[x].x + q0; A.c_q1[s + nc] = an[b].x + q0;
         A.c_r0[s + nc] = ra < rb ? ra : rb; A.c_r1[s + nc] = ra < rb ? rb : ra; A.c_n[s + nc] = A.sc_depth[b];
-        A.c_rc[s + nc] = A.anc[x].z >> 1;
+        A.c_rc[s + nc] = an[x].z >> 1;
         nc++;
     }
     return nc;
@@ -42,7 +44,11 @@
 
 
 
-template <int W, int XT>
+#ifndef LANE_PK_LD
+#define LANE_PK_LD 4
+#endif
+static_assert(LANE_PK_LD == 2 || LANE_PK_LD == 4, "eight or sixteen 8-byte anchors per load");
+template <int W, int XT, bool PK>
 __device__ __forceinline__ void chain_lane_body(const ChainArgs& A, const uint32_t rows_per_wave) {
     __shared__ uint32_t s_rd[LANE_WAVES][32][64];
     __shared__ unsigned long long s_xk[LANE_WAVES][XT ? XT : 1][XT ? 64 : 1];
@@ -61,7 +67,8 @@
             mine = e > s && e - s < 16384;
         }
     }
-    constexpr int LD = XT ? 1 : 2;
+    constexpr int LD = XT ? 1 : PK ? LANE_PK_LD : 2;
+    const AncRd<PK> anc{A.anc};
     const uint32_t s_al = s & ~(4u * LD - 1u);
     const uint32_t len = mine ? e - s_al : 0;
     LanePred P[W];
@@ -79,18 +86,19 @@
     constexpr int NR = LANE_NEAR;
     uint32_t far_diag = 0;
     for (uint32_t tb = 0; __any(tb < len); tb += 4 * LD) {
-      uint4 an[4 * LD];
-#pragma unroll
-      for (int i = 0; i < 4 * LD; i++) an[i] = make_uint4(0, 0, 0, 0);
+      uint4 aw[LD][AncRd<PK>::W4];
+#pragma unroll
+      for (int h = 0; h < LD; h++) for (int i = 0; i < AncRd<PK>::W4; i++) aw[h][i] = make_uint4(0, 0, 0, 0);
       if (tb < len) {
 #pragma unroll
-          for (int i = 0; i < 4 * LD; i++) an[i] = A.anc[s_al + tb + i];
+          for (int h = 0; h < LD; h++) anc.load4w(s_al + tb + 4u * h, aw[h]);
       }
 #pragma unroll
       for (int h = 0; h < LD; h++) {
+        uint4 an4[4];
+        AncRd<PK>::unpack4(aw[h], an4);
         const uint32_t t0 = tb + 4u * h, x0 = s_al + t0;
-        const uint32_t qs[4] = {an[4 * h].x, an[4 * h + 1].x, an[4 * h + 2].x, an[4 * h + 3].x}, rs[4] = {an[4 * h].y, an[4 * h + 1].y, an[4 * h + 2].y, an[4 * h + 3].y},
-                       ms[4] = {an[4 * h].z, an[4 * h + 1].z, an[4 * h + 2].z, an[4 * h + 3].z};
+        const uint32_t qs[4] = {an4[0].x, an4[1].x, an4[2].x, an4[3].x}, rs[4] = {an4[0].y, an4[1].y, an4[2].y, an4[3].y}, ms[4] = {an4[0].z, an4[1].z, an4[2].z, an4[3].z};
         LanePred nw[4];
         int32_t ftop[4] = {-1, -1, -1, -1};
         if (prune) {
@@ -172,6 +180,7 @@
     if ((uint32_t)lane < rows_per_wave && slot < A.n_rows && real) {
         if (mine && !ovf) {
             uint32_t nc = 0, last = 0;
+            const uint32_t q0 = PK ? A.row_q0[slot].x : 0u;
             for (uint32_t c = 0; c < S; c++) {
                 uint32_t pick = 0xFFFFFFFFu; unsigned long long k = 0;
 #pragma unroll
@@ -184,11 +193,12 @@
                     }
                 last = pick;
                 const uint32_t xb = s + (16383u - (uint32_t)((k >> 14) & 16383u));
-                const uint32_t q1 = A.anc[xb].x, rb = A.anc[xb].y;
-                const uint32_t xr = s + pick, ra = A.anc[xr].y, o = s + nc;
-                A.c_score[o] = (int32_t)(uint32_t)(k >> 28); A.c_q0[o] = A.anc[xr].x; A.c_q1[o] = q1;
+                const uint4 ab = anc[xb], ar = anc[s + pick];
+                const uint32_t q1 = ab.x + q0, rb = ab.y;
+                const uint32_t ra = ar.y, o = s + nc;
+                A.c_score[o] = (int32_t)(uint32_t)(k >> 28); A.c_q0[o] = ar.x + q0; A.c_q1[o] = q1;
                 A.c_r0[o] = ra < rb ? ra : rb; A.c_r1[o] = ra < rb ? rb : ra;
-                A.c_n[o] = (uint32_t)(k & 16383u); A.c_rc[o] = A.anc[xr].z >> 1;
+                A.c_n[o] = (uint32_t)(k & 16383u); A.c_rc[o] = ar.z >> 1;
                 nc++;
             }
             ChunkOut o{};
@@ -200,9 +210,12 @@
     }
 }
 
-__global__ __launch_bounds__(64 * LANE_WAVES) __attribute__((amdgpu_waves_per_eu(3, 8))) void chain_lane20_kernel(ChainArgs A, uint32_t rows_per_wave) { chain_lane_body<20, 0>(A, rows_per_wave); }
-__global__ __launch_bounds__(64 * LANE_WAVES) void chain_lane20x_kernel(ChainArgs A, uint32_t rows_per_wave) { chain_lane_body<20, LANE_XTREES>(A, rows_per_wave); }
-__global__ __launch_bounds__(64 * LANE_WAVES) void chain_lane_kernel(ChainArgs A, uint32_t rows_per_wave) { chain_lane_body<LANE_N, 0>(A, rows_per_wave); }
+template <bool PK>
+__global__ __launch_bounds__(64 * LANE_WAVES) __attribute__((amdgpu_waves_per_eu(3, 8))) void chain_lane20_kernel(ChainArgs A, uint32_t rows_per_wave) { chain_lane_body<20, 0, PK>(A, rows_per_wave); }
+template <bool PK>
+__global__ __launch_bounds__(64 * LANE_WAVES) void chain_lane20x_kernel(ChainArgs A, uint32_t rows_per_wave) { chain_lane_body<20, LANE_XTREES, PK>(A, rows_per_wave); }
+template <bool PK>
+__global__ __launch_bounds__(64 * LANE_WAVES) void chain_lane_kernel(ChainArgs A, uint32_t rows_per_wave) { chain_lane_body<LANE_N, 0, PK>(A, rows_per_wave); }
 
 __device__ __forceinline__ uint32_t lane_eval_d(uint32_t qx, uint32_t ux, uint32_t mx, const LaneAnchor& y, uint32_t d, int band) {
     const int32_t dq = (int32_t)(qx - y.q);
@@ -217,7 +230,9 @@
     return ((((uint32_t)scp << 7) + (((uint32_t)ANCHOR_SCORE2 << 7) | 127u) - d)) & ok;
 }
 
+template <bool PK>
 __global__ __launch_bounds__(64 * LANE_WAVES) void chain_quad_kernel(ChainArgs A) {
+    const AncRd<PK> anc{A.anc};
     __shared__ uint32_t s_rd[LANE_WAVES][32][16];
     const int wave = threadIdx.x >> 6, lane = threadIdx.x & 63, quad = lane >> 2;
     const uint32_t j = lane & 3;
@@ -247,9 +262,9 @@
     const int band = A.band;
     for (uint32_t t0 = 0; __any(t0 < len); t0 += 4) {
         const uint32_t x0 = s_al + t0;
-        uint4 an0 = make_uint4(0, 0, 0, 0), an1 = an0, an2 = an0, an3 = an0;
-        if (t0 < len) { an0 = A.anc[x0]; an1 = A.anc[x0 + 1]; an2 = A.anc[x0 + 2]; an3 = A.anc[x0 + 3]; }
-        const uint32_t qs[4] = {an0.x, an1.x, an2.x, an3.x}, rs[4] = {an0.y, an1.y, an2.y, an3.y}, ms[4] = {an0.z, an1.z, an2.z, an3.z};
+        uint4 an[4] = {make_uint4(0, 0, 0, 0), make_uint4(0, 0, 0, 0), make_uint4(0, 0, 0, 0), make_uint4(0, 0, 0, 0)};
+        if (t0 < len) anc.load4(x0, an);
+        const uint32_t qs[4] = {an[0].x, an[1].x, an[2].x, an[3].x}, rs[4] = {an[0].y, an[1].y, an[2].y, an[3].y}, ms[4] = {an[0].z, an[1].z, an[2].z, an[3].z};
 #pragma unroll
         for (int u = 0; u < 4; u++) {
             const uint32_t x = x0 + u, t = t0 + u;
@@ -302,16 +317,18 @@
     if (j == 0 && slot < A.n_rows && real) {
         if (mine && !ovf) {
             uint32_t nc = 0, last = 0;
+            const uint32_t q0 = PK ? A.row_q0[slot].x : 0u;
             for (uint32_t c = 0; c < S; c++) {
                 uint32_t pick = 0xFFFFFFFFu; unsigned long long k = 0; uint32_t q1 = 0, rb = 0;
 #pragma unroll
                 for (int i = 0; i < LANE_TREES; i++)
                     if (sroot[i] != 0xFFFFFFFFu && (c == 0 || sroot[i] > last) && sroot[i] < pick) { pick = sroot[i]; k = bk[i]; q1 = bq[i]; rb = br[i]; }
                 last = pick;
-                const uint32_t xr = s + pick, ra = A.anc[xr].y, o = s + nc;
-                A.c_score[o] = (int32_t)(uint32_t)(k >> 28); A.c_q0[o] = A.anc[xr].x; A.c_q1[o] = q1;
+                const uint4 ar = anc[s + pick];
+                const uint32_t ra = ar.y, o = s + nc;
+                A.c_score[o] = (int32_t)(uint32_t)(k >> 28); A.c_q0[o] = ar.x + q0; A.c_q1[o] = q1 + q0;
                 A.c_r0[o] = ra < rb ? ra : rb; A.c_r1[o] = ra < rb ? rb : ra;
-                A.c_n[o] = (uint32_t)(k & 16383u); A.c_rc[o] = A.anc[xr].z >> 1;
+                A.c_n[o] = (uint32_t)(k & 16383u); A.c_rc[o] = ar.z >> 1;
                 nc++;
             }
             ChunkOut o{};
@@ -334,7 +351,9 @@
     const uint32_t key = ((uint32_t)s1 << 7) + (((((uint32_t)ANCHOR_SCORE2 + 1u) << 7) | 127u) - (uint32_t)dpj);
     return (int32_t)(key | (bad & 0x80000000u));
 }
+template <bool PK>
 __global__ __launch_bounds__(64 * LANE_WAVES) void chain_quad_deep_kernel(ChainArgs A) {
+    const AncRd<PK> anc{A.anc};
     __shared__ uint32_t s_rd[LANE_WAVES][QD_RING][16];
     const int wave = threadIdx.x >> 6, lane = threadIdx.x & 63, quad = lane >> 2;
     const int32_t j = lane & 3;
@@ -364,9 +383,9 @@
     uint32_t far_diag = 0;
     for (uint32_t t0 = 0; __any(t0 < len); t0 += 4) {
         const uint32_t x0 = s_al + t0;
-        uint4 an0 = make_uint4(0, 0, 0, 0), an1 = an0, an2 = an0, an3 = an0;
-        if (t0 < len) { an0 = A.anc[x0]; an1 = A.anc[x0 + 1]; an2 = A.anc[x0 + 2]; an3 = A.anc[x0 + 3]; }
-        const uint32_t qs[4] = {an0.x, an1.x, an2.x, an3.x}, rs[4] = {an0.y, an1.y, an2.y, an3.y}, ms[4] = {an0.z, an1.z, an2.z, an3.z};
+        uint4 an[4] = {make_uint4(0, 0, 0, 0), make_uint4(0, 0, 0, 0), make_uint4(0, 0, 0, 0), make_uint4(0, 0, 0, 0)};
+        if (t0 < len) anc.load4(x0, an);
+        const uint32_t qs[4] = {an[0].x, an[1].x, an[2].x, an[3].x}, rs[4] = {an[0].y, an[1].y, an[2].y, an[3].y}, ms[4] = {an[0].z, an[1].z, an[2].z, an[3].z};
         uint32_t nq = 0, nu = 0, nm = 0xFFFFFFFFu; int32_t nf = -1;
         int32_t far_top = -1;
         {
@@ -456,16 +475,18 @@
     if (j == 0 && slot < A.n_rows && real) {
         if (mine && !ovf) {
             uint32_t nc = 0, last = 0;
+            const uint32_t q0 = PK ? A.row_q0[slot].x : 0u;
             for (uint32_t c = 0; c < S; c++) {
                 uint32_t pick = 0xFFFFFFFFu; unsigned long long k = 0; uint32_t q1 = 0, rb = 0;
 #pragma unroll
                 for (int i = 0; i < LANE_TREES; i++)
                     if (sroot[i] != 0xFFFFFFFFu && (c == 0 || sroot[i] > last) && sroot[i] < pick) { pick = sroot[i]; k = bk[i]; q1 = bq[i]; rb = br[i]; }
                 last = pick;
-                const uint32_t xr = s + pick, ra = A.anc[xr].y, o = s + nc;
-                A.c_score[o] = (int32_t)(uint32_t)(k >> 28); A.c_q0[o] = A.anc[xr].x; A.c_q1[o] = q1;
+                const uint4 ar = anc[s + pick];
+                const uint32_t ra = ar.y, o = s + nc;
+                A.c_score[o] = (int32_t)(uint32_t)(k >> 28); A.c_q0[o] = ar.x + q0; A.c_q1[o] = q1 + q0;
                 A.c_r0[o] = ra < rb ? ra : rb; A.c_r1[o] = ra < rb ? rb : ra;
-                A.c_n[o] = (uint32_t)(k & 16383u); A.c_rc[o] = A.anc[xr].z >> 1;
+                A.c_n[o] = (uint32_t)(k & 16383u); A.c_rc[o] = ar.z >> 1;
                 nc++;
             }
             ChunkOut o{};
@@ -496,9 +517,12 @@
 };
 static_assert(sizeof(uint32_t) * 7 * 64 <= sizeof(uint32_t) * 6 * RING, "candidate staging fits the ring");
 
-__device__ void chain_row_candidates(const ChainArgs& A, uint32_t s, uint32_t e, ChunkOut* op, ChainWaveLds& L, int lane, uint32_t R, bool fast);
-
+template <bool PK>
+__device__ void chain_row_candidates(const ChainArgs& A, uint32_t slot, uint32_t s, uint32_t e, ChunkOut* op, ChainWaveLds& L, int lane, uint32_t R, bool fast);
+
+template <bool PK>
 __device__ void chain_chunk_row(const ChainArgs& A, uint32_t slot, ChainWaveLds& L, int lane) {
+    const AncRd<PK> anc{A.anc};
     const uint2 se = A.chunks[slot];
     const uint32_t s = se.x, e = se.y, n = e - s;
     ChunkOut* op = &A.out[slot];
@@ -510,7 +534,7 @@
         for (uint32_t base = s; base < e && fast; base += 64) {
             const uint32_t idx = base + lane;
             const bool have = idx < e;
-            const uint4 my_a = have ? A.anc[idx] : make_uint4(0, 0, 0, 0);
+            const uint4 my_a = have ? anc[idx] : make_uint4(0, 0, 0, 0);
             const uint32_t my_qp = my_a.x, my_rp = my_a.y, my_rm = my_a.z;
             const uint32_t cnt = e - base < 64 ? e - base : 64;
             for (uint32_t j = 0; j < cnt; j++) {
@@ -559,11 +583,14 @@
             }
         }
     }
-    chain_row_candidates(A, s, e, op, L, lane, R, fast);
-}
-
-__device__ void chain_row_candidates(const ChainArgs& A, uint32_t s, uint32_t e, ChunkOut* op, ChainWaveLds& L, int lane, uint32_t R, bool fast) {
+    chain_row_candidates<PK>(A, slot, s, e, op, L, lane, R, fast);
+}
+
+template <bool PK>
+__device__ void chain_row_candidates(const ChainArgs& A, uint32_t slot, uint32_t s, uint32_t e, ChunkOut* op, ChainWaveLds& L, int lane, uint32_t R, bool fast) {
     unsigned long long* s_best_w = L.best; uint32_t (*s_cand_w)[64] = L.cand;
+    const AncRd<PK> anc{A.anc};
+    const uint32_t q0 = PK ? A.row_q0[slot].x : 0u;
     uint32_t C = 0;
     if (fast) {
         for (uint32_t r0 = 0; r0 < R && fast; r0 += 64) {
@@ -580,17 +607,17 @@
             C += __popcll(bal);
             if (C > 64) { fast = false; break; }
             if (qual) {
-                uint32_t xr = s + rootx, xb = s + lx;
-                uint32_t ra = A.anc[xr].y, rb = A.anc[xb].y;
-                s_cand_w[0][ci] = f; s_cand_w[1][ci] = A.anc[xr].x; s_cand_w[2][ci] = A.anc[xb].x;
+                const uint4 ar = anc[s + rootx], ab = anc[s + lx];
+                uint32_t ra = ar.y, rb = ab.y;
+                s_cand_w[0][ci] = f; s_cand_w[1][ci] = ar.x + q0; s_cand_w[2][ci] = ab.x + q0;
                 s_cand_w[3][ci] = ra < rb ? ra : rb; s_cand_w[4][ci] = ra < rb ? rb : ra; s_cand_w[5][ci] = dep;
-                s_cand_w[6][ci] = A.anc[xr].z >> 1;
+                s_cand_w[6][ci] = ar.z >> 1;
             }
         }
     }
     if (!fast) {
         if (lane == 0) {
-            C = chain_chunk_serial(A, s, e);
+            C = chain_chunk_serial<PK>(A, s, e, q0);
             atomicAdd(&A.stats[1], 1u);
         }
     } else {
@@ -608,6 +635,7 @@
     }
 }
 
+template <bool PK>
 __global__ __launch_bounds__(64 * CHAIN_WAVES) void chain_chunk_kernel(ChainArgs A) {
     __shared__ ChainWaveLds s_lds[CHAIN_WAVES];
     const int wave = threadIdx.x >> 6, lane = threadIdx.x & 63;
@@ -615,15 +643,16 @@
     const uint32_t pair = A.row_pair[slot < A.n_rows ? slot : A.n_rows - 1];
     if (slot >= A.n_rows) return;
     if (slot - A.cbase[pair] >= A.n_chunks[pair]) return;
-    chain_chunk_row(A, slot, s_lds[wave], lane);
-}
-
+    chain_chunk_row<PK>(A, slot, s_lds[wave], lane);
+}
+
+template <bool PK>
 __global__ __launch_bounds__(64 * CHAIN_WAVES) void chain_chunk_list_kernel(ChainArgs A) {
     __shared__ ChainWaveLds s_lds[CHAIN_WAVES];
     const int wave = threadIdx.x >> 6, lane = threadIdx.x & 63;
     const uint32_t n_list = *A.ovf_count, n_waves = gridDim.x * CHAIN_WAVES;
     for (uint32_t k = blockIdx.x * CHAIN_WAVES + wave; k < n_list; k += n_waves) {
-        chain_chunk_row(A, A.ovf_list[k], s_lds[wave], lane);
+        chain_chunk_row<PK>(A, A.ovf_list[k], s_lds[wave], lane);
         lds_wave_sync();
     }
 }
@@ -657,13 +686,13 @@
     return __builtin_amdgcn_readlane(v, 63);
 }
 
-template <int S, int T>
+template <int S, int T, bool PK>
 __device__ __forceinline__ void chain_reg_block(const ChainArgs& A, ChainWaveLds& L, uint32_t* s_root, const int lane, const uint32_t s, const uint32_t e, const uint32_t base,
                                                 const uint32_t band, RegWin& w0, RegWin& w1, uint32_t& R, bool& over) {
     constexpr uint32_t WMASK = 64u * S - 1u;
     RegWin& wt = T ? w1 : w0;
     const uint32_t idx = base + lane;
-    const uint4 my_a = idx < e ? A.anc[idx] : make_uint4(0, 0, 0, 0);
+    const uint4 my_a = idx < e ? AncRd<PK>{A.anc}[idx] : make_uint4(0, 0, 0, 0);
     const uint32_t cnt = e - base < 64 ? e - base : 64;
     for (uint32_t j = 0; j < cnt; j++) {
         const uint32_t qx = __builtin_amdgcn_readlane(my_a.x, j), rx = __builtin_amdgcn_readlane(my_a.y, j), mx = __builtin_amdgcn_readlane(my_a.z, j);
@@ -701,7 +730,7 @@
         atomicMax(&L.best[wt.id], ((unsigned long long)(uint32_t)(wt.f1 + 1) << 28) | ((unsigned long long)(16383u - (base - s + (uint32_t)lane)) << 14) | wt.dp);
 }
 
-template <int S>
+template <int S, bool PK>
 __device__ void chain_chunk_row_reg(const ChainArgs& A, uint32_t slot, ChainWaveLds& L, int lane) {
     static_assert(S == 1 || S == 2, "one or two window slots per lane");
     const uint2 se = A.chunks[slot];
@@ -719,8 +748,8 @@
         lds_wave_sync();
         bool over = false;
         for (uint32_t base = s; base < e && !over; base += 64u * S) {
-            chain_reg_block<S, 0>(A, L, s_root, lane, s, e, base, band, w0, w1, R, over);
-            if (S > 1 && base + 64u < e && !over) chain_reg_block<S, 1>(A, L, s_root, lane, s, e, base + 64u, band, w0, w1, R, over);
+            chain_reg_block<S, 0, PK>(A, L, s_root, lane, s, e, base, band, w0, w1, R, over);
+            if (S > 1 && base + 64u < e && !over) chain_reg_block<S, 1, PK>(A, L, s_root, lane, s, e, base + 64u, band, w0, w1, R, over);
         }
         fast = !over;
     }
@@ -730,10 +759,10 @@
         for (int u = 0; u < RMAX / 64; u++) if ((uint32_t)lane + 64u * u < R) L.best[lane + 64 * u] |= (unsigned long long)s_root[lane + 64 * u] << 49;
         lds_wave_sync();
     }
-    chain_row_candidates(A, s, e, op, L, lane, R, fast);
-}
-
-template <int S>
+    chain_row_candidates<PK>(A, slot, s, e, op, L, lane, R, fast);
+}
+
+template <int S, bool PK>
 __global__ __launch_bounds__(64 * CHAIN_WAVES) void chain_wave_reg_kernel(ChainArgs A) {
     __shared__ ChainWaveLds s_lds[CHAIN_WAVES];
     const int wave = __builtin_amdgcn_readfirstlane(threadIdx.x >> 6), lane = threadIdx.x & 63;
@@ -741,9 +770,16 @@
     const uint32_t pair = A.row_pair[slot < A.n_rows ? slot : A.n_rows - 1];
     if (slot >= A.n_rows) return;
     if (slot - A.cbase[pair] >= A.n_chunks[pair]) return;
-    chain_chunk_row_reg<S>(A, slot, s_lds[wave], lane);
-}
-
-
-template __global__ void chain_wave_reg_kernel<1>(ChainArgs A);
-template __global__ void chain_wave_reg_kernel<2>(ChainArgs A);
+    chain_chunk_row_reg<S, PK>(A, slot, s_lds[wave], lane);
+}
+
+
+#define PSK_DP_FORMS(PK) \
+    template __global__ void chain_lane20_kernel<PK>(ChainArgs, uint32_t); template __global__ void chain_lane20x_kernel<PK>(ChainArgs, uint32_t); \
+    template __global__ void chain_lane_kernel<PK>(ChainArgs, uint32_t); template __global__ void chain_quad_kernel<PK>(ChainArgs); \
+    template __global__ void chain_quad_deep_kernel<PK>(ChainArgs); template __global__ void chain_chunk_kernel<PK>(ChainArgs); \
+    template __global__ void chain_chunk_list_kernel<PK>(ChainArgs); \
+    template __global__ void chain_wave_reg_kernel<1, PK>(ChainArgs); template __global__ void chain_wave_reg_kernel<2, PK>(ChainArgs);
+PSK_DP_FORMS(false)
+PSK_DP_FORMS(true)
+#undef PSK_DP_FORMS
diff --git a/pyskani_amd/csrc/query_parts.h b/pyskani_amd/csrc/query_parts.h
--- a/pyskani_amd/csrc/query_parts.h
+++ b/pyskani_amd/csrc/query_parts.h
@@ -71,6 +71,7 @@
 constexpr size_t CHAIN_ANCHOR_WORDS = 14;
 struct ChainBufs {
     PairDesc* pairs; uint32_t *sbase, *cbase, *pstart; uint2* lbcnt; uint32_t* aoff; uint32_t* nch; uint2* chunks; ChunkOut* cout;
+    uint2* row_q0;
     psk_hit* hits; psk_hit* hits_sel; uint32_t* misc; uint32_t* ovf; unsigned long long* bsum; uint2* pair_qr; BatchQ* bq;
     uint32_t *blk_pair, *row_pair, *live, *big_list, *huge_list;
     uint32_t gi, gi_sum;
diff --git a/pyskani_amd/csrc/seed_index.hip b/pyskani_amd/csrc/seed_index.hip
--- a/pyskani_amd/csrc/seed_index.hip
+++ b/pyskani_amd/csrc/seed_index.hip
@@ -32,7 +32,7 @@
     uint64_t N = 0; uint32_t maxn = 0;
     for (uint32_t i = 0; i < n; i++) {
         const psk_sketch* r = db->refs[i];
-        if (!r->has_seeds || r->contig_len.size() > 32768u || r->params.k != db->params.k || r->params.c != db->params.c) return PSK_OK;
+        if (!r->has_seeds || r->contig_len.size() > (1u << GSI_CONTIG_BITS) || r->params.k != db->params.k || r->params.c != db->params.c) return PSK_OK;
         const uint32_t ns = r->store ? (uint32_t)r->n_seeds : 0u;
         segs[i] = GsiSeg{ns ? r->store->seed_kmer + r->seed_off : nullptr, ns ? r->store->seed_pm + r->seed_off : nullptr, ns, (uint32_t)N};
         N += ns; maxn = std::max(maxn, ns);
@@ -97,7 +97,7 @@
         uint64_t in_block = 0;
         for (uint32_t i = r0; i < r1; i++) {
             const psk_sketch* r = db->refs[i];
-            if (!r->has_seeds || r->contig_len.size() > 32768u || r->params.k != db->params.k || r->params.c != db->params.c) return PSK_OK;
+            if (!r->has_seeds || r->contig_len.size() > (1u << GSI_CONTIG_BITS) || r->params.k != db->params.k || r->params.c != db->params.c) return PSK_OK;
             const uint32_t ns = r->store ? (uint32_t)r->n_seeds : 0u;
             if (in_block + ns >= 0x7FFFFF00ull) return PSK_OK;
             segs[i] = GsiSeg{ns ? r->store->seed_kmer + r->seed_off : nullptr, ns ? r->store->seed_pm + r->seed_off : nullptr, ns, (uint32_t)in_block};
diff --git a/pyskani_amd/csrc/select.hip b/pyskani_amd/csrc/select.hip
--- a/pyskani_amd/csrc/select.hip
+++ b/pyskani_amd/csrc/select.hip
@@ -595,6 +595,6 @@
     const uint2 ch0 = A.chunks[row];
     if (ch0.x > ch0.y || ch0.y > A.cap) return;
     const uint32_t nc = A.pairs[pair].q_nc;
-    const uint32_t qc = nc == 1u ? 0u : A.anc[ch0.x].w;
+    const uint32_t qc = nc == 1u ? 0u : A.row_q0 ? A.row_q0[row].y : A.anc[ch0.x].w;
     if (qc < nc) o->seeds = seeds_between(A.pairs[pair], qc, o->left, o->right);
 }
diff --git a/pyskani_amd/csrc/slice_join.h b/pyskani_amd/csrc/slice_join.h
--- a/pyskani_amd/csrc/slice_join.h
+++ b/pyskani_amd/csrc/slice_join.h
@@ -24,9 +24,10 @@
     uint4* rec;
     uint32_t* bm;
     uint32_t* pair_cnt;
-    const uint32_t* pstart; uint4* anc; uint32_t cap; uint32_t* err;
+    const uint32_t* pstart; uint2* anc; uint32_t cap; uint32_t* err;
     uint32_t p_cap;
     uint2* chunks; uint32_t* n_chunks;
+    uint2* row_q0;
 };
 
 void gsl_make_tab(const BatchQ* bq, size_t n_entries, const uint32_t* q_seeds , std::vector<uint2>& tab, std::vector<uint2>& ebase, uint64_t* n_records, uint64_t* n_slices);
diff --git a/pyskani_amd/csrc/slice_join.hip b/pyskani_amd/csrc/slice_join.hip
--- a/pyskani_amd/csrc/slice_join.hip
+++ b/pyskani_amd/csrc/slice_join.hip
@@ -24,7 +24,7 @@
 static size_t gsl_walk_lds(const GslArgs& A, bool emit) {
     const size_t nw = (A.n_refs + 63) / 64;
     (void)nw;
-    return (emit ? (16 * GSL_LW + 8 + 8) * (size_t)A.p_cap + 8 * 64 : 0) + 64 + 4 * (size_t)A.p_cap + (emit ? 0 : 4 * (size_t)GSL_WORDS * (A.p_cap + 1));
+    return (emit ? (8 * GSL_LW + 8 + 8) * (size_t)A.p_cap + 8 * 64 : 0) + 64 + 4 * (size_t)A.p_cap + (emit ? 0 : 4 * (size_t)GSL_WORDS * (A.p_cap + 1));
 }
 
 template <bool EMIT>
@@ -42,8 +42,8 @@
     const uint32_t P = B.rank_hi - B.rank_lo, pc = A.p_cap;
     const uint2 eb = A.ebase[te.x];
     const uint32_t rec0 = eb.x + te.y * P;
-    uint4* s_line = s_gsl;
-    unsigned long long* s_lim = (unsigned long long*)(s_gsl + (EMIT ? GSL_LW * pc : 0u));
+    uint2* s_line = (uint2*)s_gsl;
+    unsigned long long* s_lim = (unsigned long long*)(s_line + (EMIT ? GSL_LW * pc : 0u));
     uint2* s_cs = (uint2*)(s_lim + (EMIT ? pc : 0u));
     uint2* s_fl = s_cs + (EMIT ? pc : 0u);
     uint2* s_bp = s_fl + (EMIT ? 64u : 0u);
@@ -140,27 +140,31 @@
                     continue;
                 }
                 const uint32_t sqp = (uint32_t)__builtin_amdgcn_readlane((int)qp, (int)s), sqm = (uint32_t)__builtin_amdgcn_readlane((int)qm, (int)s);
-                const uint32_t rmeta = (uint32_t)((((v >> 33) & 0x7FFFull) << 1) | (v & 1ull));
-                const uint4 av = make_uint4(sqp, (uint32_t)(v >> 1), (rmeta & ~1u) | ((rmeta ^ sqm) & 1u), sqm >> 1);
+                const uint32_t rmeta = (uint32_t)((((v >> 33) & ((1ull << GSI_CONTIG_BITS) - 1ull)) << 1) | (v & 1ull));
                 const uint32_t prev = (uint32_t)__builtin_amdgcn_update_dpp(-1, (int)slot, 0x138 , 0xf, 0xf, false);
                 const bool same = valid && prev == slot;
                 const bool dup = __ballot(same) != 0;
                 const uint2 cs = s_cs[valid ? slot : 0u];
+                const unsigned long long lim = s_lim[valid ? slot : 0u];
                 const uint32_t base = cs.x;
+                bool opens = false;
                 if (((uint32_t)__builtin_amdgcn_readlane((int)unw, (int)(jl >> 5)) >> (jl & 31u)) & 1u) {
-                    if (valid && !same) {
-                        const unsigned long long key1 = (((unsigned long long)(sqm >> 1) << 32) | sqp) + 1ull;
-                        if (key1 > s_lim[slot]) {
-                            const uint32_t row = s_rows[slot], idxc = base < A.cap ? base : A.cap;
-                            if (row < Q.rows) {
-                                uint2* r = A.chunks + ((size_t)B.row_off + (size_t)slot * Q.rows + row);
-                                r->x = idxc;
-                                if (row > 0) r[-1].y = idxc;
-                            } else atomicOr(A.err, 1u);
-                            s_rows[slot] = row + 1u; s_lim[slot] = key1 + FRAGMENT_LENGTH;
-                        }
+                    const unsigned long long key1 = (((unsigned long long)(sqm >> 1) << 32) | sqp) + 1ull;
+                    opens = valid && key1 > lim;
+                    if (opens && !same) {
+                        const uint32_t row = s_rows[slot], idxc = base < A.cap ? base : A.cap;
+                        if (row < Q.rows) {
+                            const size_t ri = (size_t)B.row_off + (size_t)slot * Q.rows + row;
+                            uint2* r = A.chunks + ri;
+                            r->x = idxc;
+                            if (row > 0) r[-1].y = idxc;
+                            A.row_q0[ri] = make_uint2(sqp, sqm >> 1);
+                        } else atomicOr(A.err, 1u);
+                        s_rows[slot] = row + 1u; s_lim[slot] = key1 + FRAGMENT_LENGTH;
                     }
                 }
+                const uint32_t q_rel = opens ? 0u : sqp - (uint32_t)(lim - 1ull - FRAGMENT_LENGTH);
+                const uint2 av = pk_anchor(q_rel, (uint32_t)(v >> 1), (rmeta & ~1u) | ((rmeta ^ sqm) & 1u));
                 if (!dup) {
                     const uint32_t t3 = base & GSL_LM;
                     if (valid) { s_cs[slot].x = base + 1u; s_line[t3 * pc + slot] = av; }
```
